# MadrMan/gpgpuraytrace

Hardware: AMD Instinct MI355X
Metric: Mray/s + ms/frame at 1920×1080, 1/2/4/8 MI355X; % HBM roofline (higher is better)
Workload: dtype f32

## Files before the change

gpgpuraytrace_amd/_native.py:

```python
import ctypes as C
import os

HERE = os.path.dirname(os.path.abspath(__file__))
LIB_PATH = os.path.join(HERE, "_build", "librt_hip.so")
ROOT = os.path.dirname(HERE)
HEADER = os.path.join(ROOT, "include", "frosttrace.h")

RT_OK = 0
RT_DEVICE_FLOAT_OUTPUT = 1
RT_DEVICE_STATS = 2
RT_DEVICE_GRAPH = 4
RT_DEVICE_DEBUG_SMALL_RINGS = 32
RT_DEVICE_DEBUG_WITHHOLD_FUSE = 64
RT_DEVICE_GATED = 128
RT_DEVICE_DEBUG_GATE_STRESS = 512
RT_DEVICE_DEFERRED = 1024
RT_DEVICE_DEBUG_DEFER_SMALL = 2048
ABI_VERSION = 9
RT_READBACK_RGBA8 = 0
RT_READBACK_BGRX = 1
RT_TEXTURE_2D = 1
RT_FORMAT_R8G8B8A8_UINT = 3


class RtStats(C.Structure):
    _fields_ = [("primary_steps", C.c_ulonglong), ("shadow_steps", C.c_ulonglong),
                ("prepass_steps", C.c_ulonglong), ("hits", C.c_ulonglong), ("noise_calls", C.c_ulonglong),
                ("ao_steps", C.c_ulonglong), ("noise_wave_iters", C.c_ulonglong)]


RT_RAYS_EYE = 1
RT_RAYS_FORCE_SEGMENTS = 2
RT_RAYS_FORCE_LANES = 4
RT_MAX_RAYS = 1 << 26


class RtRayOptions(C.Structure):
    _fields_ = [("size", C.c_uint32), ("flags", C.c_uint32), ("eye", C.c_float * 3), ("max_blocks", C.c_uint32)]


RT_SURFACE_PARAMS = 8
RT_SURFACE_RAY_RANGE = 16


class RtSurfaceOptions(C.Structure):
    _fields_ = [("size", C.c_uint32), ("flags", C.c_uint32), ("eye", C.c_float * 3), ("max_blocks", C.c_uint32),
                ("t_min", C.c_float), ("t_max", C.c_float), ("stepmod", C.c_float), ("max_steps", C.c_uint32)]


RT_POINT_MAX_AO = 16


class RtPointOptions(C.Structure):
    _fields_ = [("size", C.c_uint32), ("flags", C.c_uint32), ("eye", C.c_float * 3), ("max_blocks", C.c_uint32),
                ("ao_samples", C.c_uint32), ("seed", C.c_uint32)]


RT_FIELD_NORMAL = 32
RT_MAX_LATTICE_DIM = 4096


class RtFieldOptions(C.Structure):
    _fields_ = [("size", C.c_uint32), ("flags", C.c_uint32), ("eye", C.c_float * 3), ("max_blocks", C.c_uint32)]


class RtLattice(C.Structure):
    _fields_ = [("origin", C.c_float * 3), ("spacing", C.c_float * 3), ("dims", C.c_uint32 * 3)]


RT_DIST_FAR = 0xFFFFFFFF


class RtDistanceOptions(C.Structure):
    _fields_ = [("size", C.c_uint32), ("flags", C.c_uint32), ("eye", C.c_float * 3), ("max_blocks", C.c_uint32),
                ("max_cells", C.c_uint32)]


class NativeError(RuntimeError):
    pass


_lib = None

_vp, _i, _u, _sz, _cp = C.c_void_p, C.c_int, C.c_uint, C.c_size_t, C.c_char_p
SIGNATURES = {
    "rt_last_error": (_cp, []),
    "rt_abi_version": (_i, []),
    "rt_vfs_add_path": (_i, [_cp]),
    "rt_vfs_clear": (_i, []),
    "rt_device_create": (_i, [_i, _i, _i, _u, C.POINTER(_vp)]),
    "rt_device_destroy": (None, [_vp]),
    "rt_device_present": (_i, [_vp]),
    "rt_device_flush": (_i, [_vp]),
    "rt_device_synchronize": (_i, [_vp]),
    "rt_device_readback": (_i, [_vp, _vp, _sz]),
    "rt_device_readback_float": (_i, [_vp, _vp]),
    "rt_device_readback_bgrx": (_i, [_vp, _vp, _sz]),
    "rt_device_size": (_i, [_vp, C.POINTER(_i), C.POINTER(_i)]),
    "rt_device_framebuffer": (_vp, [_vp]),
    "rt_device_stream": (_vp, [_vp]),
    "rt_device_set_stream": (_i, [_vp, _vp]),
    "rt_device_stats": (_i, [_vp, C.POINTER(RtStats), _i]),
    "rt_device_stats_sized": (_i, [_vp, C.POINTER(RtStats), _sz, _i]),
    "rt_stream_refs": (_i, [_vp]),
    "rt_device_set_profiling": (_i, [_vp, _i]),
    "rt_device_kernel_time": (_i, [_vp, C.POINTER(C.c_double), C.POINTER(_i)]),
    "rt_device_graph_info": (_i, [_vp, C.POINTER(C.c_ulonglong), C.POINTER(C.c_ulonglong)]),
    "rt_device_info": (_i, [_vp, _i, C.POINTER(C.c_ulonglong)]),
    "rt_device_reserve_cus": (_i, [_vp, _i]),
    "rt_device_defer_batch": (_i, [_vp, _i]),
    "rt_debug_spin": (_i, [_vp, _vp, C.c_ulonglong, C.c_ulonglong, _vp]),
    "rt_debug_defer_slot": (_i, [_vp, _i, _vp, _vp, _vp]),
    "rt_device_wait_event": (_i, [_vp, _vp]),
    "rt_device_record_event": (_i, [_vp, _vp]),
    "rt_device_check": (_i, [_vp]),
    "rt_texture_create": (_i, [_vp, C.POINTER(_vp)]),
    "rt_texture_init": (_i, [_vp, _i, _i, _i, _i, _vp, _i, _i]),
    "rt_texture_destroy": (None, [_vp]),
    "rt_compute_create": (_i, [_vp, C.POINTER(_vp)]),
    "rt_compute_destroy": (None, [_vp]),
    "rt_compute_load": (_i, [_vp, _cp, _cp, _cp, _i, _i, _i, C.POINTER(_cp), C.POINTER(_cp), _i]),
    "rt_compute_swap": (_i, [_vp]),
    "rt_compute_run": (_i, [_vp, _u, _u, _u]),
    "rt_compute_set_texture": (_i, [_vp, _i, _vp]),
    "rt_compute_thread_size": (_i, [_vp, C.POINTER(_i), C.POINTER(_i), C.POINTER(_i)]),
    "rt_compute_get_variable": (_vp, [_vp, _cp]),
    "rt_compute_get_array": (_vp, [_vp, _cp]),
    "rt_compute_get_buffer": (_vp, [_vp, _cp]),
    "rt_variable_write": (_i, [_vp, _vp]),
    "rt_variable_size": (_sz, [_vp]),
    "rt_variable_name": (_cp, [_vp]),
    "rt_array_create": (_i, [_vp, _u]),
    "rt_array_map": (_vp, [_vp]),
    "rt_array_unmap": (_i, [_vp]),
    "rt_array_write": (_i, [_vp, _vp]),
    "rt_array_stride": (_sz, [_vp]),
    "rt_array_device_pointer": (_vp, [_vp]),
    "rt_terrain_render": (_i, [_vp, _vp, _i, _i]),
    "rt_terrain_render_feed": (_i, [_vp, _vp, _i, _i]),
    "rt_terrain_render_batch": (_i, [C.POINTER(_vp), C.POINTER(_vp), _i, _i, _i]),
    "rt_terrain_render_batch_packed": (_i, [C.POINTER(_vp), C.POINTER(_vp), _i, _i, _i, _vp, _sz]),
    "rt_terrain_prepass_batch": (_i, [C.POINTER(_vp), C.POINTER(_vp), _i, _i, _i, _vp]),
    "rt_terrain_trace_batch": (_i, [C.POINTER(_vp), C.POINTER(_vp), _i, _i, _i, _vp]),
    "rt_terrain_prepass_ahead": (_i, [C.POINTER(_vp), C.POINTER(_vp), _i]),
    "rt_terrain_trace_ahead": (_i, [C.POINTER(_vp), C.POINTER(_vp), _i, _i, _i]),
    "rt_terrain_feed_wait": (_i, [_vp, _vp]),
    "rt_shard_bytes": (_sz, [_vp, _i, _i]),
    "rt_shard_pack": (_i, [_vp, _i, _i, _vp]),
    "rt_shard_unpack": (_i, [_vp, _i, _i, _vp]),
    "rt_shard_pack_batch": (_i, [C.POINTER(_vp), C.POINTER(_i), _i, C.POINTER(_vp), _i]),
    "rt_shard_unpack_batch": (_i, [C.POINTER(_vp), C.POINTER(_i), _i, C.POINTER(_vp), _i]),
    "rt_terrain_trace_rays": (_i, [_vp, _vp, _vp, _i, C.POINTER(RtRayOptions), _vp, _vp]),
    "rt_terrain_trace_rays_device": (_i, [_vp, _vp, _i, C.POINTER(RtRayOptions), _vp, _vp]),
    "rt_terrain_trace_surface": (_i, [_vp, _vp, _vp, _vp, _i, C.POINTER(RtSurfaceOptions), _vp, _vp]),
    "rt_terrain_trace_surface_device": (_i, [_vp, _vp, _i, C.POINTER(RtSurfaceOptions), _vp, _vp]),
    "rt_terrain_shade_rays": (_i, [_vp, _vp, _vp, _vp, _i, C.POINTER(RtSurfaceOptions), _vp, _vp, _vp]),
    "rt_terrain_shade_rays_device": (_i, [_vp, _vp, _i, C.POINTER(RtSurfaceOptions), _vp, _vp, _vp]),
    "rt_terrain_shade_points": (_i, [_vp, _vp, _vp, _i, C.POINTER(RtPointOptions), _vp, _vp, _vp]),
    "rt_terrain_shade_points_device": (_i, [_vp, _vp, _vp, _i, C.POINTER(RtPointOptions), _vp, _vp, _vp]),
    "rt_terrain_sample_field": (_i, [_vp, _vp, _i, C.POINTER(RtFieldOptions), _vp]),
    "rt_terrain_sample_field_device": (_i, [_vp, _vp, _i, C.POINTER(RtFieldOptions), _vp]),
    "rt_terrain_sample_lattice": (_i, [_vp, C.POINTER(RtLattice), C.POINTER(RtFieldOptions), _vp, _vp]),
    "rt_terrain_sample_lattice_device": (_i, [_vp, C.POINTER(RtLattice), C.POINTER(RtFieldOptions), _vp, _vp]),
    "rt_terrain_mesh_scratch_bytes": (_sz, [C.POINTER(RtLattice)]),
    "rt_terrain_extract_mesh": (_i, [_vp, C.POINTER(RtLattice), C.POINTER(RtFieldOptions), _vp, _vp, C.c_uint32, _vp,
                                     C.c_uint32, _vp]),
    "rt_terrain_extract_mesh_device": (_i, [_vp, C.POINTER(RtLattice), C.POINTER(RtFieldOptions), _vp, _sz, _vp, _vp,
                                            C.c_uint32, _vp, C.c_uint32, _vp]),
    "rt_terrain_distance_scratch_bytes": (_sz, [C.POINTER(RtLattice)]),
    "rt_terrain_distance_field": (_i, [_vp, C.POINTER(RtLattice), C.POINTER(RtDistanceOptions), _vp, _vp, _vp]),
    "rt_terrain_distance_field_device": (_i, [_vp, C.POINTER(RtLattice), C.POINTER(RtDistanceOptions), _vp, _vp, _sz,
                                              _vp, _vp]),
    "rt_noise_generate": (_i, [C.c_uint32, _i, _vp, _vp]),
    "rt_terrain_set_target_depths": (_i, [_vp, _vp]),
    "rt_recorder_create": (_i, [_vp, _i, _i, _cp, C.POINTER(_vp)]),
    "rt_recorder_start": (_i, [_vp]),
    "rt_recorder_stop": (_i, [_vp]),
    "rt_recorder_is_recording": (_i, [_vp]),
    "rt_recorder_set_frame_time": (_i, [_vp, C.c_float]),
    "rt_recorder_write": (_i, [_vp, _vp, _i]),
    "rt_recorder_info": (_i, [_vp, C.POINTER(C.c_ulonglong), C.POINTER(C.c_ulonglong), C.POINTER(C.c_ulonglong)]),
    "rt_recorder_destroy": (None, [_vp]),
    "rt_recorder_set_async": (_i, [_vp, _i]),
    "rt_readback_create": (_i, [_vp, _i, _i, C.POINTER(_vp)]),
    "rt_readback_submit": (_i, [_vp, C.POINTER(C.c_ulonglong)]),
    "rt_readback_ready": (_i, [_vp, C.c_ulonglong]),
    "rt_readback_wait": (_i, [_vp, C.c_ulonglong, C.POINTER(_vp)]),
    "rt_readback_release": (_i, [_vp, C.c_ulonglong]),
    "rt_readback_destroy": (None, [_vp]),
    "rt_varmgr_start": (_i, [_i, _cp]),
    "rt_varmgr_stop": (_i, []),
    "rt_varmgr_count": (_i, []),
    "rt_varmgr_register_compute": (_i, [_vp]),
    "rt_debug_math": (_i, [_vp, _i, _vp, _vp, _vp, _i]),
    "rt_debug_sky_ceiling": (_i, [_vp, _i, C.c_float, _vp, _i, C.POINTER(C.c_double)]),
    "rt_debug_noise": (_i, [_vp, _vp, _vp, _i, _i]),
    "rt_debug_sky": (_i, [_vp, _vp, _vp, _i]),
}


def lib():
    global _lib
    if _lib is None:
        if not os.path.exists(LIB_PATH):
            raise ImportError(
                f"gpgpuraytrace_amd: native library missing at {LIB_PATH}; build it with "
                "`python -c 'import __graft_entry__ as g; g.build()'` (make -C gpgpuraytrace_amd/csrc)")
        L = C.CDLL(LIB_PATH)
        L.rt_abi_version.restype, L.rt_abi_version.argtypes = _i, []
        if L.rt_abi_version() < ABI_VERSION:
            raise ImportError(f"gpgpuraytrace_amd: {LIB_PATH} has ABI {L.rt_abi_version()}, this binding "
                              f"needs >= {ABI_VERSION}; rebuild it (make -C gpgpuraytrace_amd/csrc)")
        for name, (res, args) in SIGNATURES.items():
            try:
                f = getattr(L, name)
            except AttributeError:
                raise ImportError(f"gpgpuraytrace_amd: {LIB_PATH} does not export {name}; rebuild it "
                                  "(make -C gpgpuraytrace_amd/csrc)") from None
            f.restype = res
            f.argtypes = args
        _lib = L
    return _lib


def check(rc, what=""):
    if rc != RT_OK:
        msg = lib().rt_last_error().decode(errors="replace")
        raise NativeError(f"{what}: rc={rc}: {msg}")
    return rc
```

gpgpuraytrace_amd/csrc/rt_kernels.hip:

```cpp
#include <hip/hip_runtime.h>

#include <cstdio>
#include <cstdlib>
#include <type_traits>

#include "rt_kernels.h"
#include "rt_rayquery.h"
#include "rt_shader.h"
#include "rt_variants.h"

using namespace rts;
using rtm::f3;

namespace {

constexpr int kPermWords = 128 * 128;
constexpr int kNpOct = RT_NP_OCTAVES + 3;
constexpr int kOctWords = kNpOct * 4;
constexpr int kOctBase = (int)kLdsGz / 4 + (int)(kLdsGz - kLdsGxy) / 4;
constexpr int kNoiseLdsWords = kOctBase + kOctWords;
static_assert(kNoiseLdsWords % 4 == 0, "LDS carved after the noise image stays 16-byte aligned");
static_assert(kLdsGxy == (uint32_t)kPermWords * 4u, "gxy follows the perm2D texels");

__device__ __forceinline__ void load_noise_lds(uint32_t* lds, const uint32_t* __restrict__ perm2d,
                                               const float4* __restrict__ grad, const RtConsts* __restrict__ k)
{
    {
        float4* oct = reinterpret_cast<float4*>(lds + kOctBase);
        const int i = threadIdx.x;
        if (i < kNpOct) {
            const int n = i <= RT_NP_OCTAVES ? i : RT_NP_OCTAVES;
            oct[i] = make_float4(k->np_scale[n], k->np_scale_y[n], k->np_rcp[n], 0.0f);
        }
    }
    float4* gxy = reinterpret_cast<float4*>(lds + kLdsGxy / 4);
    float4* gz = reinterpret_cast<float4*>(lds + kLdsGz / 4);
    for (int i = threadIdx.x; i < 128 * 16; i += blockDim.x) {
        int e = i >> 4;
        float4 g0 = grad[e], g1 = grad[(e + 1) & 127];
        gxy[i] = make_float4(g0.x, g1.x, g0.y, g1.y);
        gz[i] = make_float4(g0.z, g1.z, 0.0f, 0.0f);
    }
    uint4* p = reinterpret_cast<uint4*>(lds);
    const uint4* src = reinterpret_cast<const uint4*>(perm2d);
    for (int i = threadIdx.x; i < kPermWords / 4; i += blockDim.x) p[i] = src[i];
    __syncthreads();
}

template <class T>
__device__ __forceinline__ T __attribute__((address_space(1)))* gptr(T* p)
{
    return (T __attribute__((address_space(1)))*)p;
}
__device__ __forceinline__ void gstore(float4* p, float4 v)
{
    typedef float v4f __attribute__((ext_vector_type(4)));
    *(v4f __attribute__((address_space(1)))*)p = v4f{v.x, v.y, v.z, v.w};
}

__device__ __forceinline__ Ctx make_ctx(const RtConsts* k, const uint32_t* lds)
{
    Ctx c;
    c.nz.img = reinterpret_cast<const char*>(lds);
    c.nz.oct = reinterpret_cast<const float4*>(lds + kOctBase);
    c.nz.so16 = kLdsGxy | ((threadIdx.x & (RT_LDS_SLOTS - 1u)) * 16u);
    c.nz.calls = 0;
    c.nz.lds_calls = nullptr;
    c.nz.phase = RT_PHASE_OTHER;
    c.k = k;
    c.kf = (KPtr)k;
    c.eye = rtm::mk(k->eye[0], k->eye[1], k->eye[2]);
    c.sun = rtm::mk(k->sun[0], k->sun[1], k->sun[2]);
    return c;
}

struct QueryEye {
    float x, y, z;
};
__device__ __forceinline__ Ctx make_ctx(const RtConsts* k, const uint32_t* lds, QueryEye e)
{
    Ctx c = make_ctx(k, lds);
    c.eye = rtm::mk(e.x, e.y, e.z);
    return c;
}

__device__ __forceinline__ void stats_noise(RtStats* stats, uint64_t calls)
{
    atomicAdd(&stats->noise_calls, (unsigned long long)(calls & 0xffffffffull));
    if (calls >> 32) atomicAdd(&stats->noise_waves, (unsigned long long)(calls >> 32));
}

__device__ __forceinline__ float uniform_f(float x)
{
    return __int_as_float(__builtin_amdgcn_readfirstlane(__float_as_int(x)));
}

__device__ __forceinline__ Ctx frame_ctx_cam(const Ctx& c, const FrameTable* __restrict__ ft, uint32_t f)
{
    Ctx cf = c;
    cf.kf = (KPtr)ft->kcam[f];
    cf.eye = rtm::mk(uniform_f(cf.kf->eye[0]), uniform_f(cf.kf->eye[1]), uniform_f(cf.kf->eye[2]));
    cf.sun = rtm::mk(uniform_f(cf.kf->sun[0]), uniform_f(cf.kf->sun[1]), uniform_f(cf.kf->sun[2]));
    return cf;
}

template <int L, bool STATS>
__global__ void __launch_bounds__(64) k_camerarays(const RtConsts* __restrict__ k, const uint32_t* __restrict__ perm2d,
                                                   const float4* __restrict__ grad, float4* __restrict__ out,
                                                   RtStats* stats, const FrameTable* __restrict__ ft)
{
    if (ft) out = ft->cam[blockIdx.y];
    __shared__ __attribute__((aligned(16))) uint32_t lds[kNoiseLdsWords];
    load_noise_lds(lds, perm2d, grad, k);
    int i = blockIdx.x * blockDim.x + threadIdx.x;
    if (i >= RT_CAMERA_RES * RT_CAMERA_RES) return;
    Ctx c = make_ctx(k, lds);
    if (ft) c = frame_ctx_cam(c, ft, blockIdx.y);
    int tx = i % RT_CAMERA_RES, ty = i / RT_CAMERA_RES;
    const float r31 = rtm::rcp(31.0f);
    uint32_t pxs = (uint32_t)(((float)tx * r31) * k->screen[0]);
    uint32_t pys = (uint32_t)(((float)ty * r31) * k->screen[1]);
    f3 p, dir;
    get_pixel_ray(c, (float)pxs, (float)pys, &p, &dir);
    RayResult rr = trace_ray<L, false, true>(c, p, RT_CAMERA_NEAR, RT_CAMERA_FAR, 2.0f, dir, 0);
    if (rr.density < 0.0f) rr.pd.w = RT_CAMERA_FAR;
    out[i] = make_float4(rr.pd.x, rr.pd.y, rr.pd.z, rr.pd.w);
    if constexpr (STATS) {
        atomicAdd(&stats->prepass_steps, (unsigned long long)rr.steps);
        stats_noise(stats, c.nz.calls);
    }
}

template <bool STATS, int BS, int LPR>
__global__ void __launch_bounds__(BS) k_camerarays_group(const RtConsts* __restrict__ k,
                                                          const uint32_t* __restrict__ perm2d,
                                                          const float4* __restrict__ grad, float4* __restrict__ out,
                                                          RtStats* stats, const FrameTable* __restrict__ ft)
{
    constexpr int L = RT_NOMADPLAINS;
    if (ft) out = ft->cam[blockIdx.y];
    __shared__ __attribute__((aligned(16))) uint32_t lds[kNoiseLdsWords];
    load_noise_lds(lds, perm2d, grad, k);
    const int i = blockIdx.x * (BS / LPR) + (int)(threadIdx.x / LPR);
    if (i >= RT_CAMERA_RES * RT_CAMERA_RES) return;
    Ctx c = make_ctx(k, lds);
    if (ft) c = frame_ctx_cam(c, ft, blockIdx.y);
    const uint32_t j = threadIdx.x & (LPR - 1u), base = threadIdx.x & 63u & ~(LPR - 1u);
    const SegOctaves<LPR> g = seg_octaves<LPR>(c, j);
    int tx = i % RT_CAMERA_RES, ty = i / RT_CAMERA_RES;
    const float r31 = rtm::rcp(31.0f);
    uint32_t pxs = (uint32_t)(((float)tx * r31) * k->screen[0]);
    uint32_t pys = (uint32_t)(((float)ty * r31) * k->screen[1]);
    f3 p, dir;
    get_pixel_ray(c, (float)pxs, (float)pys, &p, &dir);
    March<L, false> st;
    march_begin(c, st, p, RT_CAMERA_NEAR, 2.0f, dir);
    uint32_t noise = 0;
    while (march_live<L, false, true>(c, st, RT_CAMERA_FAR, 0)) {
        auto dens = [&](f3 q) {
            uint32_t used;
            float d = density_nomadplains_seg<LPR>(c, g, q, j, base, &used);
            noise += used + 1u;
            return d;
        };
        march_step_with<L, false, true>(c, st, dens);
    }
    RayResult rr = march_result(st);
    if (rr.density < 0.0f) rr.pd.w = RT_CAMERA_FAR;
    if (j == 0) {
        out[i] = make_float4(rr.pd.x, rr.pd.y, rr.pd.z, rr.pd.w);
        if constexpr (STATS) {
            atomicAdd(&stats->prepass_steps, (unsigned long long)rr.steps);
            atomicAdd(&stats->noise_calls, (unsigned long long)noise);
        }
    }
}

template <class Depth>
__device__ __forceinline__ float cd_get_depth(Depth depth, int x, int y)
{
    x = x < 0 ? 0 : (x >= RT_CAMERA_RES ? RT_CAMERA_RES - 1 : x);
    y = y < 0 ? 0 : (y >= RT_CAMERA_RES ? RT_CAMERA_RES - 1 : y);
    return depth(x, y);
}
template <class Depth>
__device__ __forceinline__ float cd_interp(Depth d, int x, int y)
{
    if (x < 0) {
        float m = cd_get_depth(d, x + 1, y);
        float dd = cd_get_depth(d, x + 2, y) - m;
        return m - dd;
    }
    if (x >= RT_CAMERA_RES) {
        float m = cd_get_depth(d, x - 1, y);
        float dd = cd_get_depth(d, x - 2, y) - m;
        return m - dd;
    }
    if (y < 0) {
        float m = cd_get_depth(d, x, y + 1);
        float dd = cd_get_depth(d, x, y + 2) - m;
        return m - dd;
    }
    if (y >= RT_CAMERA_RES) {
        float m = cd_get_depth(d, x, y - 1);
        float dd = cd_get_depth(d, x, y - 2) - m;
        return m - dd;
    }
    return cd_get_depth(d, x, y);
}

template <class Depth>
__device__ __forceinline__ float2 cell_bracket(Depth depth, int xpos, int ypos)
{
    float dmin = cd_interp(depth, xpos, ypos);
    float dmax = dmin;
    for (int xp = -2; xp <= 2; ++xp) {
        for (int yp = -2; yp <= 2; ++yp) {
            float d = cd_interp(depth, xpos + xp, ypos + yp);
            dmin = (dmin < d) ? dmin : d;
            dmax = (d < dmax) ? dmax : d;
        }
    }
    dmin = dmin * 0.96f - 0.01f;
    dmax = dmax * 1.22f + 0.4f;
    dmin = (RT_CAMERA_NEAR < dmin) ? dmin : RT_CAMERA_NEAR;
    dmax = (dmax < RT_CAMERA_FAR) ? dmax : RT_CAMERA_FAR;
    return make_float2(dmin, dmax);
}

__device__ __forceinline__ float cam_depth_sc1(const float4* cam, int x, int y)
{
    typedef const float __attribute__((address_space(1))) gfloat;
    return __hip_atomic_load((gfloat*)(reinterpret_cast<const float*>(cam + y * RT_CAMERA_RES + x) + 3),
                             __ATOMIC_RELAXED, __HIP_MEMORY_SCOPE_AGENT);
}

__device__ __forceinline__ void cell_depths_frame(const float4* __restrict__ cam, float2* __restrict__ cells,
                                                  float* s_d)
{
    const int i = threadIdx.x;
    __syncthreads();
    s_d[i] = cam_depth_sc1(cam, i % RT_CAMERA_RES, i / RT_CAMERA_RES);
    __syncthreads();
    cells[i] = cell_bracket([&](int x, int y) { return s_d[y * RT_CAMERA_RES + x]; }, i % RT_CAMERA_RES,
                            i / RT_CAMERA_RES);
}

struct UnitMap {
    uint32_t off_x, off_y, ext_x, ext_y, tiles32_x, tile_first, tile_stride, n_units;
    uint32_t n_frames, frame_samples;
    uint32_t frame_rot;
    uint32_t order_batch;
    uint32_t cells_from_cam;
    uint32_t fit;
    uint32_t fitm;
    uint32_t packed;
};

__device__ __forceinline__ uint32_t out_index(const UnitMap& m, uint32_t u, uint32_t lane, uint32_t px, uint32_t py,
                                              uint32_t W)
{
    if (m.packed)
        return (u >> 4) * 1024u + ((u & 15u) >> 2) * 256u + (lane >> 3) * 32u + (u & 3u) * 8u + (lane & 7u);
    return py * W + px;
}
__device__ __forceinline__ uint32_t packed_index(uint32_t tl)
{
    return (tl & ~0xf8u) | ((tl >> 3) & 0x18u) | ((tl << 2) & 0xe0u);
}

__device__ __forceinline__ bool unit_pixel(const UnitMap& m, uint32_t f, uint32_t u, uint32_t lane, uint32_t W,
                                           uint32_t H, uint32_t* px, uint32_t* py)
{
    const uint32_t first = m.frame_rot ? (m.tile_first + f) % m.tile_stride : m.tile_first;
    uint32_t T = (u >> 4) * m.tile_stride + first, sub = u & 15u;
    uint32_t gx = (T % m.tiles32_x) * 32u + (sub & 3u) * 8u + (lane & 7u);
    uint32_t gy = (T / m.tiles32_x) * 32u + (sub >> 2) * 8u + (lane >> 3);
    *px = gx + m.off_x;
    *py = gy + m.off_y;
    return gx < m.ext_x && gy < m.ext_y && *px < W && *py < H;
}

__device__ __forceinline__ bool sample_pixel(const UnitMap& m, uint32_t f, uint32_t t, uint32_t aa, uint32_t W,
                                             uint32_t H, uint32_t* px, uint32_t* py, uint32_t* a)
{
    uint32_t pix = t / aa;
    *a = t - pix * aa;
    return unit_pixel(m, f, pix >> 6, pix & 63u, W, H, px, py);
}

__device__ __forceinline__ uint32_t wave_fetch(uint32_t* counter, uint32_t lane, uint32_t n = 1u)
{
    uint32_t u = 0;
    if (lane == 0) u = atomicAdd(counter, n);
    return __builtin_amdgcn_readfirstlane(u);
}

__device__ __forceinline__ uint32_t lane_rank(uint64_t mask)
{
    return __builtin_amdgcn_mbcnt_hi((uint32_t)(mask >> 32), __builtin_amdgcn_mbcnt_lo((uint32_t)mask, 0u));
}

__device__ __forceinline__ uint32_t first_unit_index(uint32_t* __restrict__ counters, uint32_t lane)
{
    const uint32_t w = (uint32_t)__builtin_amdgcn_readfirstlane((int)(threadIdx.x >> 6));
    return w * gridDim.x + wave_fetch(&counters[RT_CTR_FIRST + w], lane);
}

template <int L>
struct HitRec {
    static constexpr uint32_t N = FogLive<L>::value ? 3u : (RT_DIAG_HITPAD ? 2u : 1u);
};
template <int L>
__device__ __forceinline__ void hit_store(float4* __restrict__ r, uint32_t t, const RayResult& rr)
{
    if constexpr (FogLive<L>::value) {
        r[0] = make_float4(rr.pd.x, rr.pd.y, rr.pd.z, rr.pd.w);
        r[1] = make_float4(rr.fc.x, rr.fc.y, rr.fc.z, rr.fc.w);
        r[2] = make_float4(rr.density, rr.steps, 0.0f, __uint_as_float(t));
    } else {
        r[0] = make_float4(rr.sd, rr.pd.w, rr.density, __uint_as_float(t));
        if constexpr (RT_DIAG_HITPAD) r[1] = make_float4(0.0f, 0.0f, 0.0f, 0.0f);
    }
}

constexpr uint32_t kOrderLdsBuckets = 144u * 1024u;
constexpr uint32_t kOrderBatchUnitsPerWave = 4u;
__global__ void __launch_bounds__(1024) k_order(const FrameTable* __restrict__ ft, UnitMap m,
                                                uint32_t* __restrict__ order, uint32_t* __restrict__ counters,
                                                const uint32_t* wait_ctl, uint32_t wait_total, uint32_t* zero_ctl,
                                                uint32_t* host_flag, uint32_t* gate, uint32_t* claims)
{
    __shared__ float s_key[RT_CAMERA_RES * RT_CAMERA_RES];
    __shared__ uint32_t s_hist[64];
    __shared__ uint8_t s_b[kOrderLdsBuckets];
    if (blockIdx.x == 0 && threadIdx.x < RT_CTR_BYTES / 4) counters[threadIdx.x] = 0u;
    if (zero_ctl && blockIdx.x == 0 && threadIdx.x < 2) zero_ctl[threadIdx.x] = 0u;
    if (gate) {
        const uint32_t g0 = m.order_batch ? 0u : blockIdx.x, g1 = m.order_batch ? m.n_frames : blockIdx.x + 1u;
        for (uint32_t i = g0 * RT_GATE_WORDS + threadIdx.x; i < g1 * RT_GATE_WORDS; i += blockDim.x) gate[i] = 0u;
        const uint32_t nt = m.n_units >> 4;
        for (uint32_t i = g0 * nt + threadIdx.x; i < g1 * nt; i += blockDim.x) claims[i] = 0u;
    }
    if (wait_ctl) {
        if (threadIdx.x == 0) {
            const uint64_t t0 = __builtin_amdgcn_s_memrealtime();
            while (__hip_atomic_load(wait_ctl + 1, __ATOMIC_RELAXED, __HIP_MEMORY_SCOPE_AGENT) < wait_total) {
                __builtin_amdgcn_s_sleep(8);
                if (__builtin_amdgcn_s_memrealtime() - t0 > 50000000ull) {
                    atomicOr(counters + RT_CTR_BYTES / 4, RT_FLAG_PREPASS_TIMEOUT);
                    if (host_flag) __hip_atomic_store(host_flag, RT_FLAG_PREPASS_TIMEOUT, __ATOMIC_RELAXED,
                                                      __HIP_MEMORY_SCOPE_SYSTEM);
                    break;
                }
            }
        }
        __syncthreads();
    }
    if (m.cells_from_cam) {
        const uint32_t c0 = m.order_batch ? 0u : blockIdx.x, c1 = m.order_batch ? m.n_frames : blockIdx.x + 1u;
        for (uint32_t f = c0; f < c1; ++f) cell_depths_frame(ft->cam[f], ft->cells[f], s_key);
        __syncthreads();
    }
    if (threadIdx.x < 64) s_hist[threadIdx.x] = 0;
    const uint32_t n_tiles = m.n_units >> 4;
    const bool cached = n_tiles * m.n_frames <= kOrderLdsBuckets;
    uint32_t f = 0;
    auto load_keys = [&]() {
        __syncthreads();
        const float2* cells = ft->cells[f];
        for (int i = threadIdx.x; i < RT_CAMERA_RES * RT_CAMERA_RES; i += blockDim.x) {
            float2 cd = cells[i];
            s_key[i] = __log2f(cd.y / cd.x);
        }
        __syncthreads();
    };
    auto bucket = [&](uint32_t tile) -> uint32_t {
        const RtConsts* k = ft->k[f];
        const uint32_t W = (uint32_t)k->width, H = (uint32_t)k->height;
        float key = 0.0f;
        for (uint32_t corner = 0; corner < 4; ++corner) {
            uint32_t px, py;
            uint32_t u = tile * 16u + (corner & 1u) * 3u + (corner >> 1) * 12u;
            uint32_t lane = (corner & 1u) * 7u + (corner >> 1) * 56u;
            if (!unit_pixel(m, f, u, lane, W, H, &px, &py)) {
                if (!unit_pixel(m, f, tile * 16u, 0u, W, H, &px, &py)) continue;
                px = px + (corner & 1u) * 31u < W ? px + (corner & 1u) * 31u : W - 1u;
                py = py + (corner >> 1) * 31u < H ? py + (corner >> 1) * 31u : H - 1u;
            }
            float spx = (float)px * k->rcp_w, spy = (float)py * k->rcp_h;
            uint32_t cell = (uint32_t)rtm::fma(rtm::floor(spy * 32.0f), 32.0f, rtm::floor(spx * 32.0f));
            key = fmaxf(key, s_key[cell]);
        }
        int b = (int)(key * 3.3f);
        return (uint32_t)(b < 0 ? 0 : (b > 63 ? 63 : b));
    };
    {
        const uint32_t g0 = m.order_batch ? 0u : blockIdx.x, g1 = m.order_batch ? m.n_frames : blockIdx.x + 1u;
        for (f = g0; f < g1; ++f) {
            load_keys();
            for (uint32_t t = threadIdx.x; t < n_tiles; t += blockDim.x) {
                const uint32_t b = bucket(t);
                if (cached) s_b[f * n_tiles + t] = (uint8_t)b;
                atomicAdd(&s_hist[b], 1u);
            }
        }
        __syncthreads();
        if (threadIdx.x == 0) {
            uint32_t run = g0 * n_tiles;
            for (int b = 63; b >= 0; --b) {
                uint32_t c = s_hist[b];
                s_hist[b] = run;
                run += c;
            }
        }
        for (f = g0; f < g1; ++f) {
            if (cached) __syncthreads();
            else load_keys();
            for (uint32_t t = threadIdx.x; t < n_tiles; t += blockDim.x) {
                const uint32_t b = cached ? (uint32_t)s_b[f * n_tiles + t] : bucket(t);
                order[atomicAdd(&s_hist[b], 1u)] = (f << 24) | t;
            }
        }
    }
}

constexpr uint32_t kShadowRec = 3;

constexpr uint32_t kRefillIdle = RT_REFILL_IDLE;

__device__ __forceinline__ float4 shade_finish(const RtConsts* k, float4 cb, float4 fog, float4 ray,
                                               float shadow_density, float shadow_fog_w)
{
    float b = cb.w;
    if (shadow_density > 0.0f) b = b * 0.1f;
    else b = rtm::sat(b - shadow_fog_w);
    f3 col = rtm::mk(cb.x * fma(b, k->one_minus_shadow[0], k->shadow_color[0]),
                     cb.y * fma(b, k->one_minus_shadow[1], k->shadow_color[1]),
                     cb.z * fma(b, k->one_minus_shadow[2], k->shadow_color[2]));
    col = rtm::mk(rtm::lerp(col.x, fog.x, fog.w), rtm::lerp(col.y, fog.y, fog.w), rtm::lerp(col.z, fog.z, fog.w));
    col = rtm::mk(rtm::lerp(col.x, ray.x, ray.w), rtm::lerp(col.y, ray.y, ray.w), rtm::lerp(col.z, ray.z, ray.w));
    return make_float4(rtm::sat(col.x), rtm::sat(col.y), rtm::sat(col.z), 1.0f);
}

__device__ __forceinline__ float4 miss_sample(const Ctx& c, float px, float py, float dist, f4 fog)
{
    f3 p, dir;
    get_pixel_ray(c, px, py, &p, &dir);
    f3 pdn = rtm::normalize(dir);
    float skyAmount = dist * 0.0005f;
    skyAmount = rtm::sat(skyAmount * skyAmount);
    SkyColor scat = get_rayleigh_mie(c, pdn);
    float space = get_space_color(c, pdn);
    f3 sky = rtm::mk((scat.mie.x + scat.rayleigh.x) + space, (scat.mie.y + scat.rayleigh.y) + space,
                     (scat.mie.z + scat.rayleigh.z) + space);
    f3 col = rtm::mk(rtm::lerp(sky.x, fog.x, fog.w), rtm::lerp(sky.y, fog.y, fog.w), rtm::lerp(sky.z, fog.z, fog.w));
    col = rtm::mk(rtm::lerp(col.x, sky.x, skyAmount), rtm::lerp(col.y, sky.y, skyAmount),
                  rtm::lerp(col.z, sky.z, skyAmount));
    return make_float4(rtm::sat(col.x), rtm::sat(col.y), rtm::sat(col.z), 0.0f);
}

typedef float v4f_t __attribute__((ext_vector_type(4)));
__device__ __forceinline__ float4 ld_rec(const float4* base, uint32_t i)
{
    const __amdgpu_buffer_rsrc_t r =
        __builtin_amdgcn_make_buffer_rsrc(const_cast<float4*>(base), (short)0, 0x7fffffff, 0x00020000);
    const v4f_t v = __builtin_amdgcn_raw_buffer_load_b128(r, (int)(i * 16u), 0, 16 );
    return make_float4(v.x, v.y, v.z, v.w);
}
__device__ __forceinline__ uint32_t ld_u32(const uint32_t* base, uint32_t i, bool sc1 = true)
{
    const __amdgpu_buffer_rsrc_t r =
        __builtin_amdgcn_make_buffer_rsrc(const_cast<uint32_t*>(base), (short)0, 0x7fffffff, 0x00020000);
    return sc1 ? __builtin_amdgcn_raw_buffer_load_b32(r, (int)(i * 4u), 0, 16 )
               : __builtin_amdgcn_raw_buffer_load_b32(r, (int)(i * 4u), 0, 0);
}
__device__ __forceinline__ float4 ld_fresh(const float4* p)
{
    v4f_t v;
    asm volatile("global_load_dwordx4 %0, %1, off sc1\n\ts_waitcnt vmcnt(0)" : "=v"(v) : "v"(p) : "memory");
    return make_float4(v.x, v.y, v.z, v.w);
}

__device__ __forceinline__ uint32_t late(uint32_t x)
{
    asm volatile("" : "+v"(x));
    return x;
}

__device__ __forceinline__ void sample_store(const RtConsts* k, float4* __restrict__ samples, uint32_t t, float4 v)
{
    t = late(t);
    if (k->aa_samples == 1) {
        float* c = reinterpret_cast<float*>(samples) + 3u * t;
        c[0] = v.x;
        c[1] = v.y;
        c[2] = v.z;
    } else {
        samples[t] = v;
    }
}

__device__ __forceinline__ void ao_count(uint32_t* __restrict__ aocc, uint32_t t)
{
    atomicAdd(&aocc[t >> 2], 1u << ((t & 3u) * 8u));
}
constexpr uint32_t kFinFlag = 0x80u;
__device__ __forceinline__ uint32_t ao_occluded(const uint32_t* __restrict__ aocc, uint32_t t)
{
    return (aocc[t >> 2] >> ((t & 3u) * 8u)) & 0x7fu;
}

struct ShadeHit {
    float4 cb, fog, ray;
    bool more;
    f3 hp, n;
    float prec;
    uint32_t px, py, a;
};


__device__ __forceinline__ Ctx frame_ctx(const Ctx& c, const FrameTable* __restrict__ ft, uint32_t f)
{
    Ctx cf = c;
    cf.kf = (KPtr)ft->k[f];
    cf.eye = rtm::mk(uniform_f(cf.kf->eye[0]), uniform_f(cf.kf->eye[1]), uniform_f(cf.kf->eye[2]));
    cf.sun = rtm::mk(uniform_f(cf.kf->sun[0]), uniform_f(cf.kf->sun[1]), uniform_f(cf.kf->sun[2]));
    return cf;
}

__device__ __forceinline__ uint32_t frame_of(const UnitMap& m, uint32_t t)
{
    return m.n_frames == 1u ? 0u : t / m.frame_samples;
}

template <class Body>
__device__ __forceinline__ void per_frame(bool valid, uint32_t f_lane, Body body)
{
    uint64_t pend = __ballot(valid);
    while (pend) {
        const uint32_t f = (uint32_t)__builtin_amdgcn_readlane((int)f_lane, (int)__builtin_ctzll(pend));
        const bool mine = valid && f_lane == f;
        pend &= ~__ballot(mine);
        if (mine) body(f);
    }
}

struct FrameRays {
    float v[RT_MAX_BATCH][6];
    uint32_t* out8[RT_MAX_BATCH];
};
__device__ __forceinline__ void frame_rays_load(FrameRays& s, const FrameTable* __restrict__ ft, uint32_t n_frames)
{
    if (threadIdx.x < n_frames) {
        const RtConsts* k = ft->k[threadIdx.x];
        const f3 sun = rtm::mk(k->sun[0], k->sun[1], k->sun[2]);
        const f3 sd = rtm::scale(sun, rtm::rcp(rtm::length(sun)));
        s.v[threadIdx.x][0] = k->eye[0];
        s.v[threadIdx.x][1] = k->eye[1];
        s.v[threadIdx.x][2] = k->eye[2];
        s.v[threadIdx.x][3] = sd.x;
        s.v[threadIdx.x][4] = sd.y;
        s.v[threadIdx.x][5] = sd.z;
        s.out8[threadIdx.x] = ft->out8[threadIdx.x];
    }
}

template <int L>
__device__ __forceinline__ ShadeHit shade_hit(const Ctx& c, const UnitMap& m, float4 r0, float4 r1, float4 r2,
                                              uint32_t t, uint32_t tl, March<L, true>& st)
{
    const RtConsts* k = c.k;
    const uint32_t W = (uint32_t)k->width, H = (uint32_t)k->height, aa = (uint32_t)k->aa_samples;
    ShadeHit h;
    float4 pdw, dn;
    if constexpr (FogLive<L>::value) {
        pdw = r0;
        h.fog = r1;
        dn = r2;
    } else {
        (void)r1;
        (void)r2;
        pdw = make_float4(r0.x, 0.0f, 0.0f, r0.y);
        dn = make_float4(r0.z, 0.0f, 0.0f, 0.0f);
        h.fog = make_float4(0.0f, 0.0f, 0.0f, 0.0f);
    }
    uint32_t px, py, a;
    sample_pixel(m, m.frame_rot ? (t - tl) / m.frame_samples : 0u, tl, aa, W, H, &px, &py, &a);
    h.px = px;
    h.py = py;
    h.a = a;
    f3 p, dir;
    get_pixel_ray(c, (float)px + k->aa_off[a][0], (float)py + k->aa_off[a][1], &p, &dir);
    if constexpr (!FogLive<L>::value) {
        const f3 md = rtm::scale(dir, rtm::rcp(rtm::length(dir)));
        const float sd = pdw.x;
        pdw = make_float4(fma(md.x, sd, p.x), fma(md.y, sd, p.y), fma(md.z, sd, p.z), pdw.w);
    }
    f3 hp = rtm::mk(pdw.x, pdw.y, pdw.z);
    h.hp = hp;
    h.prec = shade_precision(pdw.w);
    march_begin(c, st, hp, 0.4f, h.prec, c.sun);
    if (march_live<L, true, true>(c, st, 100.0f, 0)) march_step<L, true, true>(c, st);
    h.more = march_live<L, true, true>(c, st, 100.0f, 0);
    f3 pdn = rtm::normalize(dir);
    float skyAmount = pdw.w * 0.0005f;
    skyAmount = rtm::sat(skyAmount * skyAmount);
    f4 pd = {pdw.x, pdw.y, pdw.z, dn.x};
    f3 n = get_normal<L>(c, pd);
    h.n = n;
    ShadePre sp = shade_pre<L>(c, hp, n, pdn, pdw.w);
    float specular = rtm::sat(rtm::pow_nonneg(rtm::max(sp.spec_dot, 0.0f), 40.0f)) * sp.spec_k;
    SkyColor scat = get_rayleigh_mie(c, pdn);
    h.cb = make_float4(sp.col[0] + specular, sp.col[1] + specular, sp.col[2] + specular, sp.brightness);
    h.ray = make_float4(scat.rayleigh.x, scat.rayleigh.y, scat.rayleigh.z, skyAmount);
    return h;
}

constexpr uint32_t kAuxAO = 0xffffffffu, kAuxAOCand = 0x80000000u, kAuxFinT = 0x7ffffffeu;
__device__ __forceinline__ bool aux_ao(uint32_t aux) { return (int32_t)aux < 0; }
constexpr uint32_t kAuxAOSlot = 0xc0000000u, kAuxSlotFree = 0x60000000u;
__device__ __forceinline__ bool aux_ao_slot(uint32_t aux) { return (aux & 0xff000000u) == kAuxAOSlot; }
__device__ __forceinline__ bool aux_slot_free(uint32_t aux) { return (aux & 0xff000000u) == kAuxSlotFree; }

template <int L>
__device__ __forceinline__ void long_pack(const March<L, true>& st, uint32_t t, uint32_t aux, float4* r)
{
    r[0] = make_float4(st.p.x, st.p.y, st.p.z, st.dist);
    r[1] = make_float4(st.step, __uint_as_float(aux), __uint_as_float((uint32_t)st.iters), __uint_as_float(t));
    if (aux_ao(aux)) r[2] = make_float4(st.dir.x, st.dir.y, st.dir.z, 0.0f);
    else if constexpr (March<L, true>::FOG) r[2] = make_float4(st.f.x, st.f.y, st.f.z, st.f.w);
}

template <int L>
__device__ __forceinline__ uint32_t long_unpack(const float4 r0, const float4 r1, const float4 r2, f3 sun_dir,
                                                March<L, true>& st, uint32_t* aux)
{
    *aux = __float_as_uint(r1.y);
    st.p = rtm::mk(r0.x, r0.y, r0.z);
    st.dist = r0.w;
    st.step = r1.x;
    st.lastStep = 0.0f;
    st.d = 0.0f;
    st.iters = (int)__float_as_uint(r1.z);
    if (aux_ao(*aux)) {
        st.dir = rtm::mk(r2.x, r2.y, r2.z);
        st.f = {0.0f, 0.0f, 0.0f, 0.0f};
        st.fog = false;
    } else {
        st.dir = sun_dir;
        if constexpr (March<L, true>::FOG) st.f = {r2.x, r2.y, r2.z, r2.w};
        else st.f = {0.0f, 0.0f, 0.0f, 0.0f};
        st.fog = true;
    }
    return __float_as_uint(r1.w);
}

template <int L>
__device__ __forceinline__ void ao_begin(const Ctx& c, const ShadeHit& h, uint32_t kk, March<L, true>& st)
{
    march_begin(c, st, h.hp, 0.4f, h.prec, ao_dir(h.n, h.px, h.py, h.a, kk), false);
}

template <int L>
struct FinRec {
    static constexpr uint32_t N = FogLive<L>::value ? 3u : 2u;
};
template <int L>
__device__ __forceinline__ void fin_store(float4* __restrict__ f, const ShadeHit& h)
{
    if constexpr (FogLive<L>::value) {
        f[0] = h.cb;
        f[1] = h.fog;
        f[2] = h.ray;
    } else {
        f[0] = h.cb;
        f[1] = h.ray;
    }
}

__device__ __forceinline__ uint32_t fit_pixel(float4 v, float ao)
{
    const float ia = rtm::rcp(1.0f);
    return unorm8((0.0f + v.x * ao) * ia) | (unorm8((0.0f + v.y * ao) * ia) << 8) |
           (unorm8((0.0f + v.z * ao) * ia) << 16) | 0xff000000u;
}

__device__ __forceinline__ void fit_store(const RtConsts* k, const UnitMap& m, const FrameRays& fr, uint32_t t,
                                          uint32_t px8)
{
    const uint32_t f = frame_of(m, t), W = (uint32_t)k->width;
    const uint32_t tl = t - f * m.frame_samples;
    if (m.packed) {
        gptr(fr.out8[f])[late(packed_index(tl))] = px8;
        return;
    }
    uint32_t px, py;
    unit_pixel(m, f, tl >> 6, t & 63u, W, (uint32_t)k->height, &px, &py);
    gptr(fr.out8[f])[(size_t)late(py) * W + px] = px8;
}

template <int L>
__device__ __forceinline__ void long_finish(const RtConsts* k, const UnitMap& m, const FrameRays& fr,
                                            const float4* __restrict__ fin, const float4* __restrict__ finp,
                                            float4* __restrict__ samples, uint32_t* __restrict__ aocc, uint32_t t,
                                            uint32_t aux, const March<L, true>& st)
{
    if (aux_ao(aux)) {
        if (st.d > 0.0f) {
            if (aux == kAuxAO) {
                if (m.fit) reinterpret_cast<uint8_t*>(aocc)[late(t)] = (uint8_t)(kFinFlag | 1u);
                else if (k->ao_samples == 1) reinterpret_cast<uint8_t*>(aocc)[late(t)] = 1u;
                else if (!(RT_DIAG_SKIP & 8)) ao_count(aocc, t);
            } else if (!(RT_DIAG_SKIP & 2)) {
                fit_store(k, m, fr, t, aux | 0xff000000u);
            }
        }
    } else {
        constexpr uint32_t FR = FinRec<L>::N;
        float4 f0, f1, fog = make_float4(0.0f, 0.0f, 0.0f, 0.0f);
        if (aux == kAuxFinT) {
            const float4* f = fin + (size_t)FR * t;
            f0 = ld_fresh(f);
            if constexpr (FogLive<L>::value) fog = ld_fresh(f + 1);
            f1 = ld_fresh(f + FR - 1u);
        } else {
            f0 = ld_rec(finp, FR * aux);
            if constexpr (FogLive<L>::value) fog = ld_rec(finp, FR * aux + 1u);
            f1 = ld_rec(finp, FR * aux + FR - 1u);
        }
        const float4 v = shade_finish(k, f0, fog, f1, st.d, st.f.w);
        if (m.fit && k->ao_samples == 0) {
            if (!(RT_DIAG_SKIP & 2)) fit_store(k, m, fr, t, fit_pixel(v, 1.0f));
        } else if (!(RT_DIAG_SKIP & 4)) {
            sample_store(k, samples, t, v);
        }
    }
}

constexpr uint32_t kLongRing = 570;
constexpr uint32_t kFinSlots = RT_FIN_SLOTS;
constexpr uint32_t kAoSlots = RT_AO_SLOTS;
static_assert(kAoSlots % 2u == 0u && kAoSlots <= 256u && kAoSlots <= RT_AO_POOL_SLOTS,
              "AO slots: pairs of u16 counters, u8 indices, a colour each in the pool");
constexpr uint32_t kLongBatch = RT_LONG_BATCH;
constexpr uint32_t kCompactLive = RT_COMPACT_LIVE;
constexpr uint32_t kSegLanes = RT_SEG_LANES, kSegHandBack = RT_SEG_HANDBACK, kSegQueue = RT_SEG_QUEUE;
constexpr uint32_t kPrepassSplit = RT_FUSE_RAYS_PER_TASK / (64u / RT_PREPASS_LPR);
static_assert(kPrepassSplit >= 1u && RT_PREPASS_LPR >= RT_FUSE_RAYS_PER_TASK && RT_PREPASS_LPR <= 32, "prepass lanes per ray");
constexpr uint32_t kPrimarySeg = RT_PRIMARY_SEG;
static_assert(kPrimarySeg == 0u || kPrimarySeg == 4u || kPrimarySeg == 8u || kPrimarySeg == 16u, "lanes per ray");
constexpr bool kStatsPrimarySeg = RT_STATS_PRIMARY_SEG != 0;

struct BlockStats {
    enum { PRIMARY = 0, SHADOW = 1, AO = 2, HITS = 3, NOISE = 4, NOISE_WAVES = 5 };
    unsigned long long v[6];
    uint32_t done, pad;
};

struct TraceQueues {
    uint32_t lock;
    uint32_t h_top, pad0;
    uint32_t l_head, l_tail;
    uint32_t active;
    uint32_t drained;
    uint32_t pad;
    uint32_t ls_top;
    uint32_t pad1;
    uint32_t f_top;
    uint32_t overflow;
    uint32_t gscan, gate_all, gate_cells;
    uint32_t near_end;

    float4 longs[kLongRing * kShadowRec];
    uint16_t fin_free[kFinSlots];
    uint32_t ao_ctr[kAoSlots / 2];
    uint8_t ao_free[kAoSlots];
    uint32_t ao_top;
};

template <class T>
__device__ __forceinline__ T vload(const T& x)
{
    return __hip_atomic_load(&x, __ATOMIC_RELAXED, __HIP_MEMORY_SCOPE_WORKGROUP);
}

__device__ __forceinline__ void q_lock(uint32_t* lock, uint32_t lane)
{
    if (lane == 0) {
        while (atomicCAS(lock, 0u, 1u) != 0u) __builtin_amdgcn_s_sleep(1);
    }
    __builtin_amdgcn_wave_barrier();
    __builtin_amdgcn_fence(__ATOMIC_ACQUIRE, "workgroup");
}

__device__ __forceinline__ void q_unlock(uint32_t* lock, uint32_t lane)
{
    __builtin_amdgcn_fence(__ATOMIC_RELEASE, "workgroup");
    __builtin_amdgcn_wave_barrier();
    if (lane == 0) atomicExch(lock, 0u);
}

RT_DIAG_LIVE_HIST(__device__ unsigned long long g_live_hist[65];)
WT(__device__ unsigned long long g_wave_trace[RT_WT_MAX_WAVES * RT_WT_FIELDS];)

template <int L>
struct TraceThreads {
    static constexpr uint32_t value = 64u * ((L == RT_GREENROCKS || L == RT_SIMPLE) ? RT_TRACE_WAVES_WIDE : RT_TRACE_WAVES_FAST);
};
static_assert(RT_CTR_FIRST + RT_TRACE_WAVES_FAST <= RT_CTR_BYTES / 4 && RT_CTR_FIRST + RT_TRACE_WAVES_WIDE <= RT_CTR_BYTES / 4,
              "a first-unit counter per wave slot inside the zeroed work counters");

template <int L, bool STATS, bool GATED = false>
__global__ void __launch_bounds__(TraceThreads<L>::value) k_trace(const RtConsts* __restrict__ k, const FrameTable* __restrict__ ft,
                                                const uint32_t* __restrict__ perm2d,
                                                const float4* __restrict__ grad,
                                                UnitMap m, const uint32_t* __restrict__ order,
                                                uint64_t* __restrict__ hitmask, float4* __restrict__ samples,
                                                float4* __restrict__ fin, float4* __restrict__ finpool,
                                                float4* __restrict__ cpool,
                                                float4* __restrict__ hitq,
                                                float4* __restrict__ spill_long, uint32_t hit_cap,
                                                uint32_t long_spill_cap,
                                                uint32_t* __restrict__ aocc, uint32_t* __restrict__ counters,
                                                RtStats* stats, uint32_t long_batch, uint32_t refill_idle,
                                                uint32_t compact_live, uint32_t long_ring_cap, uint32_t fin_slots,
                                                FusedPrepass np, GatedPrepass gp)
{
    __shared__ __attribute__((aligned(16))) uint32_t
        lds[kNoiseLdsWords + (sizeof(FrameRays) + sizeof(TraceQueues) + sizeof(BlockStats)) / 4];
    FrameRays& s_fr = *reinterpret_cast<FrameRays*>(lds + kNoiseLdsWords);
    TraceQueues& q = *reinterpret_cast<TraceQueues*>(lds + kNoiseLdsWords + sizeof(FrameRays) / 4);
    BlockStats& s_st =
        *reinterpret_cast<BlockStats*>(lds + kNoiseLdsWords + (sizeof(FrameRays) + sizeof(TraceQueues)) / 4);
    frame_rays_load(s_fr, ft, m.n_frames);
    if (threadIdx.x == 0) {
        q.lock = 0;
        q.h_top = 0;
        q.l_head = q.l_tail = 0;
        q.active = 0;
        q.drained = 0;
        q.ls_top = 0;
        q.f_top = fin_slots;
        q.overflow = 0;
        q.gscan = q.gate_all = q.gate_cells = 0;
        q.near_end = 0;
        if constexpr (STATS) s_st = BlockStats{};
    }
    for (uint32_t i = threadIdx.x; i < fin_slots; i += blockDim.x) q.fin_free[i] = (uint16_t)i;
    for (uint32_t i = threadIdx.x; i < kAoSlots; i += blockDim.x) {
        q.ao_free[i] = (uint8_t)i;
        if (i < kAoSlots / 2u) q.ao_ctr[i] = 0u;
    }
    if (threadIdx.x == 0) q.ao_top = kAoSlots;
    load_noise_lds(lds, perm2d, grad, k);
    const uint32_t lane = __lane_id();
    Ctx c = make_ctx(k, lds);
    if constexpr (STATS) c.nz.lds_calls = (__attribute__((address_space(3))) unsigned long long*)&s_st.v[BlockStats::NOISE];
    const uint32_t W = (uint32_t)k->width, H = (uint32_t)k->height, aa = (uint32_t)k->aa_samples;
    const int max_steps = k->max_steps;
    constexpr bool kSky = RT_SKY_EXIT && L == RT_NOMADPLAINS && (!STATS || RT_SKY_EXIT_STATS);
    const uint32_t n_total = (uint32_t)__builtin_amdgcn_readfirstlane(m.n_units * m.n_frames);
    constexpr uint32_t HR = HitRec<L>::N;
    float4* const hq = hitq + (size_t)blockIdx.x * hit_cap * HR;
    float4* const finp = finpool + (size_t)blockIdx.x * kFinSlots * FinRec<L>::N;
    float4* const cpl = cpool + (size_t)blockIdx.x * RT_AO_POOL_SLOTS;
    float4* const lspill = spill_long + (size_t)blockIdx.x * long_spill_cap * kShadowRec;
    auto queued_long = [&]() { return vload(q.l_tail) - vload(q.l_head) + vload(q.ls_top); };
    auto queued_hits = [&]() { return vload(q.h_top); };
    auto stat = [&](int i, uint32_t v) {
        if constexpr (STATS) atomicAdd(&s_st.v[i], (unsigned long long)v);
    };

    WT(unsigned long long wt[RT_WT_FIELDS] = {}; wt[10] = __builtin_amdgcn_s_getreg((31 << 11) | 4);
       wt[11] = __builtin_amdgcn_s_getreg((31 << 11) | 20); uint32_t wl_rays = 0, wl_maxit = 0, wp_maxit = 0;)
    auto push_recs = [&](bool want, auto pack) {
        const uint64_t lb = __ballot(want);
        if (!lb) return;
        const uint32_t n = (uint32_t)__popcll(lb), rank = lane_rank(lb);
        q_lock(&q.lock, lane);
        const uint32_t lh = vload(q.l_head), lt = vload(q.l_tail);
        if (lt - lh + n <= long_ring_cap) {
            if (want) pack(&q.longs[((lt + rank) % kLongRing) * kShadowRec]);
            if (lane == 0) q.l_tail = lt + n;
        } else {
            const uint32_t stl = (uint32_t)__builtin_amdgcn_readfirstlane(vload(q.ls_top));
            const bool fits = stl + n <= long_spill_cap;
            if (want && fits) pack(lspill + (size_t)(stl + rank) * kShadowRec);
            __builtin_amdgcn_s_waitcnt(0);
            if (lane == 0) {
                q.ls_top = fits ? stl + n : stl;
                q.overflow |= fits ? 0u : RT_FLAG_SPILL_OVERFLOW;
            }
        }
        q_unlock(&q.lock, lane);
    };
    auto push_long = [&](bool want, const March<L, true>& st, uint32_t t, uint32_t aux) {
        push_recs(want, [&](float4* r) { long_pack(st, t, aux, r); });
    };

    auto free_fin_locked = [&](bool live, uint32_t& aux) {
        const bool pend = !live && aux < kFinSlots;
        const uint64_t pb = __ballot(pend);
        if (pb) {
            const uint32_t top = vload(q.f_top);
            if (pend) {
                q.fin_free[top + lane_rank(pb)] = (uint16_t)aux;
                aux = kAuxAO;
            }
            if (lane == 0) q.f_top = top + (uint32_t)__popcll(pb);
        }
        if constexpr (kAoSlots > 0u) {
            const bool pa = !live && aux_slot_free(aux);
            const uint64_t ab = __ballot(pa);
            if (ab) {
                const uint32_t top = vload(q.ao_top);
                if (pa) {
                    q.ao_free[top + lane_rank(ab)] = (uint8_t)(aux & 255u);
                    aux = kAuxAO;
                }
                if (lane == 0) q.ao_top = top + (uint32_t)__popcll(ab);
            }
        }
    };
    auto ao_slot_finish = [&](const March<L, true>& st, uint32_t t, uint32_t& aux) {
        const uint32_t sl = aux & 255u, sh = (sl & 1u) * 16u;
        const uint32_t occ1 = st.d > 0.0f ? 1u : 0u;
        const uint32_t old = atomicAdd(&q.ao_ctr[sl >> 1], (1u | (occ1 << 5)) << sh) >> sh;
        if ((old & 31u) + 1u == (uint32_t)k->ao_samples) {
            const uint32_t occ = ((old >> 5) & 31u) + occ1;
            if (m.fitm && !(old & (1u << 10))) {
                const float4 v = ld_rec(cpl, sl);
                const uint32_t at = __float_as_uint(v.w);
                if (!(RT_DIAG_SKIP & 2)) gptr(s_fr.out8[at >> 23])[at & 0x7fffffu] = fit_pixel(v, ao_factor(occ, k->ao_samples));
            } else if (occ != 0u) {
                reinterpret_cast<uint8_t*>(aocc)[late(t)] = (uint8_t)((m.fitm ? kFinFlag : 0u) | occ);
            }
            atomicAnd(&q.ao_ctr[sl >> 1], ~(0xffffu << sh));
            aux = kAuxSlotFree | sl;
        } else {
            aux = kAuxAO;
        }
    };

    auto do_shadow = [&]() {
        March<L, true> st;
        st.d = 0.0f;
        st.iters = 0;
        bool live = false;
        uint32_t t = 0, aux = kAuxAO;
        Ctx cl = c;
        cl.nz.phase = RT_PHASE_LONG;
        for (;;) {
            if (live && !march_live<L, true, true>(cl, st, aux_ao(aux) ? RT_AO_END : 100.0f, 0)) {
                WT(wl_rays++; wl_maxit = max(wl_maxit, (uint32_t)st.iters);)
                stat(aux_ao(aux) ? BlockStats::AO : BlockStats::SHADOW, (uint32_t)st.iters);
                if (kAoSlots > 0u && aux_ao_slot(aux)) ao_slot_finish(st, t, aux);
                else long_finish<L>(k, m, s_fr, fin, finp, samples, aocc, t, aux, st);
                live = false;
            }
            const uint64_t idle = __ballot(!live);
            const uint32_t nidle = (uint32_t)__popcll(idle);
            if (nidle >= refill_idle && queued_long() != 0u) {
                q_lock(&q.lock, lane);
                free_fin_locked(live, aux);
                const uint32_t head = vload(q.l_head), tail = vload(q.l_tail);
                const uint32_t take = (tail - head) < nidle ? (tail - head) : nidle;
                const uint32_t sl = vload(q.ls_top);
                const uint32_t more = sl < nidle - take ? sl : nidle - take;
                const uint32_t rank = lane_rank(idle);
                const bool mine = ((idle >> lane) & 1ull) && rank < take + more;
                auto take_ray = [&](float4 r0, float4 r1, float4 r2) {
                    t = long_unpack(r0, r1, r2, rtm::mk(0.0f, 0.0f, 0.0f), st, &aux);
                    const float* fr = s_fr.v[frame_of(m, t)];
                    cl.eye = rtm::mk(fr[0], fr[1], fr[2]);
                    if (!aux_ao(aux)) st.dir = rtm::mk(fr[3], fr[4], fr[5]);
                    live = true;
                };
                if (mine && rank < take) {
                    const float4* r = &q.longs[((head + rank) % kLongRing) * kShadowRec];
                    take_ray(r[0], r[1], r[2]);
                } else if (mine) {
                    const uint32_t ri = (sl - more + rank - take) * kShadowRec;
                    take_ray(ld_rec(lspill, ri), ld_rec(lspill, ri + 1u), ld_rec(lspill, ri + 2u));
                }
                if (more) __builtin_amdgcn_s_waitcnt(0);
                if (lane == 0) {
                    q.l_head = head + take;
                    q.ls_top = sl - more;
                }
                q_unlock(&q.lock, lane);
            }
            const uint64_t lv = __ballot(live);
            const bool drained_now = vload(q.drained) != 0u;
            bool hand_back = lv != 0ull && (uint32_t)__popcll(lv) < compact_live && queued_long() == 0u && !drained_now;
            if constexpr (L == RT_NOMADPLAINS && kSegLanes > 0u)
                hand_back = hand_back || (drained_now && lv != 0ull && (uint32_t)__popcll(lv) <= kSegHandBack &&
                                          queued_long() == 0u);
            if (lv == 0ull || hand_back) {
                if (__ballot(!live && (aux < kFinSlots || aux_slot_free(aux)))) {
                    q_lock(&q.lock, lane);
                    free_fin_locked(live, aux);
                    q_unlock(&q.lock, lane);
                }
                if (hand_back) push_long(live, st, t, aux);
                c.nz.calls = cl.nz.calls;
                return;
            }
            RT_DIAG_LONG_STEPS(if (live && (RT_COUNT_LONG_STEPS == 1 || (RT_COUNT_LONG_STEPS == 2) == (vload(q.drained) != 0u))) {
                cl.nz.phase = RT_COUNT_PHASE;
                count_noise(cl.nz);
                cl.nz.phase = RT_PHASE_LONG;
            })
            WT(wt[26]++;)
            if (live) march_step<L, true, true>(cl, st);
        }
    };

    auto do_shadow_seg = [&]() {
        if constexpr (L == RT_NOMADPLAINS && kSegLanes > 0u) {
            constexpr uint32_t LPR = kSegLanes ? kSegLanes : 8u, RPW = 64u / LPR;
            March<L, true> st;
            st.d = 0.0f;
            st.iters = 0;
            uint32_t t = 0, aux = kAuxAO;
            bool live = false;
            Ctx cl = c;
            cl.nz.phase = RT_PHASE_LONG;
            q_lock(&q.lock, lane);
            const uint32_t head = vload(q.l_head), tail = vload(q.l_tail);
            const uint32_t take = (tail - head) < RPW ? (tail - head) : RPW;
            const uint32_t sl = vload(q.ls_top);
            const uint32_t more = sl < RPW - take ? sl : RPW - take;
            if (const uint32_t grp = late(lane) / LPR; grp < take + more) {
                float4 r0, r1, r2;
                if (grp < take) {
                    const float4* r = &q.longs[((head + grp) % kLongRing) * kShadowRec];
                    r0 = r[0];
                    r1 = r[1];
                    r2 = r[2];
                } else {
                    const uint32_t ri = (sl - more + grp - take) * kShadowRec;
                    r0 = ld_rec(lspill, ri);
                    r1 = ld_rec(lspill, ri + 1u);
                    r2 = ld_rec(lspill, ri + 2u);
                }
                t = long_unpack(r0, r1, r2, rtm::mk(0.0f, 0.0f, 0.0f), st, &aux);
                const float* fr = s_fr.v[frame_of(m, t)];
                cl.eye = rtm::mk(fr[0], fr[1], fr[2]);
                if (!aux_ao(aux)) st.dir = rtm::mk(fr[3], fr[4], fr[5]);
                live = true;
            }
            __builtin_amdgcn_s_waitcnt(0);
            if (lane == 0) {
                q.l_head = head + take;
                q.ls_top = sl - more;
            }
            q_unlock(&q.lock, lane);
            const uint32_t lid = late(lane);
            const uint32_t j = lid & (LPR - 1u), base = lid & ~(LPR - 1u);
            const SegOctaves<LPR> g = seg_octaves<LPR>(c, j);
            for (;;) {
                if (live && !march_live<L, true, true>(cl, st, aux_ao(aux) ? RT_AO_END : 100.0f, 0)) {
                    if (j == 0u) {
                        stat(aux_ao(aux) ? BlockStats::AO : BlockStats::SHADOW, (uint32_t)st.iters);
                        if (kAoSlots > 0u && aux_ao_slot(aux)) ao_slot_finish(st, t, aux);
                        else long_finish<L>(k, m, s_fr, fin, finp, samples, aocc, t, aux, st);
                    }
                    live = false;
                }
                if (!__ballot(live)) break;
                WT(wt[25]++;)
                if (live) {
                    auto dens = [&](f3 q0) {
                        uint32_t used;
                        const float d = density_nomadplains_seg<LPR>(cl, g, q0, j, base, &used);
                        if constexpr (STATS) {
                            if (j == 0u) atomicAdd(&s_st.v[BlockStats::NOISE], (unsigned long long)(used + 1u));
                            if (lane == (uint32_t)__builtin_ctzll(__ballot(1)))
                                atomicAdd(&s_st.v[BlockStats::NOISE_WAVES], (unsigned long long)SegOctaves<LPR>::R);
                        }
                        return d;
                    };
                    march_step_with<L, true, true>(cl, st, dens);
                }
            }
            uint32_t fa = j == 0u ? aux : kAuxAO;
            if (__ballot(fa < kFinSlots || aux_slot_free(fa))) {
                q_lock(&q.lock, lane);
                free_fin_locked(false, fa);
                q_unlock(&q.lock, lane);
            }
        }
    };

    auto primary_seg = [&](const Ctx& cf, March<L, true>& st, bool lv, uint64_t lb, float spx, float spy, bool sky) {
        if constexpr (L == RT_NOMADPLAINS && kPrimarySeg > 0u && (!STATS || kStatsPrimarySeg)) {
            constexpr uint32_t LPR = 64u / (kPrimarySeg ? kPrimarySeg : 8u);
            const uint32_t lid = late(lane);
            const uint32_t j = lid & (LPR - 1u), grp = lid / LPR, base = lid & ~(LPR - 1u);
            const uint32_t n = (uint32_t)__popcll(lb);
            uint32_t src = lid;
            uint64_t rem = lb;
            for (uint32_t r = 0; r < n; ++r) {
                const uint32_t sl = (uint32_t)__builtin_ctzll(rem);
                rem &= rem - 1ull;
                src = grp == r ? sl : src;
            }
            March<L, true> sg;
            sg.p = rtm::mk(__shfl(st.p.x, (int)src), __shfl(st.p.y, (int)src), __shfl(st.p.z, (int)src));
            sg.dir = rtm::mk(__shfl(st.dir.x, (int)src), __shfl(st.dir.y, (int)src), __shfl(st.dir.z, (int)src));
            sg.sd = __shfl(st.sd, (int)src);
            sg.dist = __shfl(st.dist, (int)src);
            sg.step = __shfl(st.step, (int)src);
            sg.lastStep = __shfl(st.lastStep, (int)src);
            sg.d = __shfl(st.d, (int)src);
            sg.iters = __shfl(st.iters, (int)src);
            sg.f = {0.0f, 0.0f, 0.0f, 0.0f};
            sg.fog = false;
            bool live = grp < n;
            const SegOctaves<LPR> g = seg_octaves<LPR>(cf, j);
            for (;;) {
                if (live && !march_live<L, true, false>(cf, sg, RT_CAMERA_FAR, max_steps)) live = false;
                if constexpr (kSky) {
                    if (live && sky && sky_exit(sg.p.y, sg.dir.y, sg.dist)) live = false;
                }
                if (!__ballot(live)) break;
                if (live) {
                    auto dens = [&](f3 q0) {
                        uint32_t used;
                        const float d = density_nomadplains_seg<LPR, true>(cf, g, q0, j, base, &used);
                        if constexpr (STATS) {
                            if (j == 0u) atomicAdd(&s_st.v[BlockStats::NOISE], (unsigned long long)(used + 1u));
                            if (lane == (uint32_t)__builtin_ctzll(__ballot(1)))
                                atomicAdd(&s_st.v[BlockStats::NOISE_WAVES], (unsigned long long)SegOctaves<LPR>::R);
                        }
                        return d;
                    };
                    march_step_with<L, true, false>(cf, sg, dens);
                }
            }
            const int back = (int)(lane_rank(lb) * LPR);
            const float sd = __shfl(sg.sd, back), dist = __shfl(sg.dist, back), step = __shfl(sg.step, back);
            const float last = __shfl(sg.lastStep, back), d = __shfl(sg.d, back);
            const int iters = __shfl(sg.iters, back);
            if (lv) {
                st.sd = sd;
                st.dist = dist;
                st.step = step;
                st.lastStep = last;
                st.d = d;
                st.iters = iters;
            }
            f3 p, dir;
            get_pixel_ray(cf, spx, spy, &p, &dir);
            st.p = p;
            st.dir = rtm::scale(dir, rtm::rcp(rtm::length(dir)));
        }
    };

    auto do_shade = [&]() {
        q_lock(&q.lock, lane);
        const uint32_t top = vload(q.h_top);
        const uint32_t take = top < 64u ? top : 64u;
        float4 r0 = make_float4(0.0f, 0.0f, 0.0f, 0.0f), r1 = r0, r2 = r0;
        if (lane < take) {
            const uint32_t ri = (top - take + lane) * HR;
            r0 = ld_rec(hq, ri);
            if constexpr (HR == 3u) {
                r1 = ld_rec(hq, ri + 1u);
                r2 = ld_rec(hq, ri + 2u);
            }
        }
        __builtin_amdgcn_s_waitcnt(0);
        if (lane == 0) q.h_top = top - take;
        q_unlock(&q.lock, lane);
        const uint32_t t = __float_as_uint(HR == 3u ? r2.w : r0.w);
        March<L, true> st;
        bool more = false;
        uint32_t aux = kAuxAO;
        uint32_t ao_aux = kAuxAO;
        const bool valid = lane < take;
        if (kAoSlots > 0u && k->ao_samples >= 2) {
            const uint64_t vb = __ballot(valid);
            if (vb) {
                q_lock(&q.lock, lane);
                const uint32_t top = vload(q.ao_top), n = (uint32_t)__popcll(vb), rank = lane_rank(vb);
                const uint32_t got = n < top ? n : top;
                if (valid && rank < got) ao_aux = kAuxAOSlot | (uint32_t)q.ao_free[top - 1u - rank];
                if (lane == 0) q.ao_top = top - got;
                q_unlock(&q.lock, lane);
            }
        }
        ShadeHit h;
        per_frame(valid, valid ? frame_of(m, t) : 0u, [&](uint32_t f) {
            Ctx cf = frame_ctx(c, ft, f);
            cf.nz.phase = RT_PHASE_SHADE;
            h = shade_hit<L>(cf, m, r0, r1, r2, t, t - f * m.frame_samples, st);
            c.nz.calls = cf.nz.calls;
            more = h.more;
            if (!more) {
                const float4 v = shade_finish(k, h.cb, h.fog, h.ray, st.d, st.f.w);
                if (m.fit) {
                    if (!(RT_DIAG_SKIP & 2)) {
                        const uint32_t tl = t - f * m.frame_samples;
                        gptr(ft->out8[f])[m.packed ? late(packed_index(tl)) : late(h.py) * W + h.px] = fit_pixel(v, 1.0f);
                    }
                    if (k->ao_samples) ao_aux = kAuxAOCand | (fit_pixel(v, ao_factor(1u, 1)) & 0xffffffu);
                } else if (m.fitm && aux_ao_slot(ao_aux)) {
                    const uint32_t tl = t - f * m.frame_samples;
                    cpl[late(ao_aux & 255u)] =
                        make_float4(v.x, v.y, v.z, __uint_as_float((f << 23) | (m.packed ? packed_index(tl) : h.py * W + h.px)));
                } else if (!(RT_DIAG_SKIP & 4)) {
                    sample_store(k, samples, t, v);
                }
                stat(BlockStats::SHADOW, (uint32_t)st.iters);
            }
            const uint64_t mb = __ballot(more);
            if (mb) {
                const uint32_t lead = (uint32_t)__builtin_ctzll(__ballot(1));
                q_lock(&q.lock, lane - lead);
                const uint32_t top = vload(q.f_top), n = (uint32_t)__popcll(mb), rank = lane_rank(mb);
                const uint32_t got = n < top ? n : top;
                if (more) aux = rank < got ? (uint32_t)q.fin_free[top - 1u - rank] : kAuxFinT;
                if (lane == lead) q.f_top = top - got;
                q_unlock(&q.lock, lane - lead);
                if (more && !(RT_DIAG_SKIP & 16)) fin_store<L>(aux == kAuxFinT ? fin + (size_t)FinRec<L>::N * t : finp + (size_t)FinRec<L>::N * aux, h);
            }
        });
        const bool kfin = valid && ((m.fit && k->ao_samples && more) || (m.fitm && (more || !aux_ao_slot(ao_aux))));
        if (kfin) {
            reinterpret_cast<uint8_t*>(aocc)[late(t)] = (uint8_t)kFinFlag;
            hitmask[t >> 6] = 1ull;
        }
        if (m.fitm && more && aux_ao_slot(ao_aux))
            atomicOr(&q.ao_ctr[(ao_aux & 255u) >> 1], (1u << 10) << ((ao_aux & 1u) * 16u));
        if (__ballot(more)) {
            __builtin_amdgcn_s_waitcnt(0);
            push_long(more, st, t, aux);
        }
        if (m.fit || m.fitm) __builtin_amdgcn_s_waitcnt(0);
        for (int kk = 0; kk < k->ao_samples; ++kk) {
            March<L, true> ao;
            if (valid) ao_begin(c, h, (uint32_t)kk, ao);
            push_long(valid, ao, t, ao_aux);
        }
    };

    auto do_prepass = [&](const FrameTable* __restrict__ pft, uint32_t qt, bool own) {
        if constexpr (L == RT_NOMADPLAINS) {
            constexpr uint32_t LPR = RT_PREPASS_LPR, RPW = 64u / LPR;
            constexpr uint32_t WPF = RT_CAMERA_RES * RT_CAMERA_RES / RPW;
            const uint32_t f = qt / WPF;
            const uint32_t ray0 = (qt - f * WPF) * RPW;
            const uint32_t ray = ray0 + late(lane) / LPR;
            const uint32_t lid = late(lane);
            const uint32_t j = lid & (LPR - 1u), base = lid & ~(LPR - 1u);
            Ctx cp = c;
            cp.k = pft->kcam[0];
            cp.kf = (KPtr)pft->kcam[f];
            cp.eye = rtm::mk(uniform_f(cp.kf->eye[0]), uniform_f(cp.kf->eye[1]), uniform_f(cp.kf->eye[2]));
            cp.sun = rtm::mk(uniform_f(cp.kf->sun[0]), uniform_f(cp.kf->sun[1]), uniform_f(cp.kf->sun[2]));
            const uint32_t tx = ray % RT_CAMERA_RES, ty = ray / RT_CAMERA_RES;
            const float r31 = rtm::rcp(31.0f);
            const uint32_t pxs = (uint32_t)(((float)tx * r31) * cp.k->screen[0]);
            const uint32_t pys = (uint32_t)(((float)ty * r31) * cp.k->screen[1]);
            f3 p, dir;
            get_pixel_ray(cp, (float)pxs, (float)pys, &p, &dir);
            March<L, false> st;
            march_begin(cp, st, p, RT_CAMERA_NEAR, 2.0f, dir);
            const SegOctaves<LPR> g = seg_octaves<LPR>(cp, j);
            __builtin_amdgcn_s_setprio(RT_FUSE_PRIO);
            while (march_live<L, false, true>(cp, st, RT_CAMERA_FAR, 0)) {
                auto dens = [&](f3 q0) {
                    uint32_t used;
                    return density_nomadplains_seg<LPR, false>(cp, g, q0, j, base, &used);
                };
                march_step_with<L, false, true>(cp, st, dens);
            }
            __builtin_amdgcn_s_setprio(0);
            RayResult rr = march_result(st);
            if (rr.density < 0.0f) rr.pd.w = RT_CAMERA_FAR;
            if (j == 0u) {
                typedef float v4f __attribute__((ext_vector_type(4)));
                const v4f v = {rr.pd.x, rr.pd.y, rr.pd.z, rr.pd.w};
                float4* dst = pft->cam[f] + ray;
                asm volatile("global_store_dwordx4 %0, %1, off sc1" : : "v"(dst), "v"(v) : "memory");
            }
            asm volatile("s_waitcnt vmcnt(0)" : : : "memory");
            if (!own) {
                if (lane == 0) __hip_atomic_fetch_add(np.ctl + 1, RPW, __ATOMIC_RELAXED, __HIP_MEMORY_SCOPE_AGENT);
                return;
            }
            typedef uint32_t __attribute__((address_space(1))) guint;
            guint* gf = (guint*)(gp.gate + f * RT_GATE_WORDS);
            uint32_t old = 0;
            if (lane == 0) {
                const uint32_t task = ray0 / RT_FUSE_RAYS_PER_TASK;
                bool whole = true;
                if constexpr (RPW < RT_FUSE_RAYS_PER_TASK)
                    whole = __hip_atomic_fetch_add(gf + RT_GATE_TASKS + task, RPW, __ATOMIC_RELAXED,
                                                   __HIP_MEMORY_SCOPE_AGENT) == RT_FUSE_RAYS_PER_TASK - RPW;
                if (whole) {
                    __hip_atomic_fetch_or(gf + (task >> 5), 1u << (task & 31u), __ATOMIC_RELAXED, __HIP_MEMORY_SCOPE_AGENT);
                    old = __hip_atomic_fetch_add(gf + RT_GATE_CTR, (uint32_t)RT_FUSE_RAYS_PER_TASK, __ATOMIC_RELAXED,
                                                 __HIP_MEMORY_SCOPE_AGENT);
                }
            }
            if ((uint32_t)__builtin_amdgcn_readfirstlane(old) == RT_CAMERA_RES * RT_CAMERA_RES - RT_FUSE_RAYS_PER_TASK) {
                if (gp.debug & 2u) {
                    const uint64_t t0 = __builtin_amdgcn_s_memrealtime();
                    while (__builtin_amdgcn_s_memrealtime() - t0 < 20000ull) __builtin_amdgcn_s_sleep(8);
                }
                const float4* cam = pft->cam[f];
                typedef unsigned long long __attribute__((address_space(1))) gu64;
                gu64* cells = (gu64*)pft->cells[f];
                for (uint32_t c = late(lane); c < RT_CAMERA_RES * RT_CAMERA_RES; c += 64u) {
                    const float2 b = cell_bracket([&](int x, int y) { return cam_depth_sc1(cam, x, y); },
                                                  (int)(c % RT_CAMERA_RES), (int)(c / RT_CAMERA_RES));
                    __hip_atomic_store(cells + c, (unsigned long long)__float_as_uint(b.x) |
                                                      ((unsigned long long)__float_as_uint(b.y) << 32),
                                       __ATOMIC_RELAXED, __HIP_MEMORY_SCOPE_AGENT);
                }
                asm volatile("s_waitcnt vmcnt(0)" : : : "memory");
                if (lane == 0) __hip_atomic_store(gf + RT_GATE_CTR + 1, 1u, __ATOMIC_RELAXED, __HIP_MEMORY_SCOPE_AGENT);
            }
        }
    };

    typedef const uint32_t __attribute__((address_space(1))) gcuint;
    auto ld_sc1 = [&](const uint32_t* p) {
        return __hip_atomic_load((gcuint*)p, __ATOMIC_RELAXED, __HIP_MEMORY_SCOPE_AGENT);
    };
    auto tile_ready = [&](uint32_t e, uint32_t w0, uint32_t w1, uint32_t w2, uint32_t w3) -> bool {
        const uint32_t f = e >> 24, first = m.frame_rot ? (m.tile_first + f) % m.tile_stride : m.tile_first;
        const uint32_t T = (e & 0xffffffu) * m.tile_stride + first;
        const uint32_t gx = (T % m.tiles32_x) * 32u, gy = (T / m.tiles32_x) * 32u;
        const uint32_t px0 = gx + m.off_x, py0 = gy + m.off_y;
        if (gx >= m.ext_x || gy >= m.ext_y || px0 >= W || py0 >= H) return true;
        const uint32_t xe = m.off_x + m.ext_x < W ? m.off_x + m.ext_x : W, ye = m.off_y + m.ext_y < H ? m.off_y + m.ext_y : H;
        const uint32_t px1 = px0 + 31u < xe ? px0 + 31u : xe - 1u, py1 = py0 + 31u < ye ? py0 + 31u : ye - 1u;
        auto cell_of = [&](uint32_t p, float r) { return (int)rtm::floor(((float)p * r) * 32.0f); };
        const int cx0 = cell_of(px0, k->rcp_w) - 2, cx1 = cell_of(px1, k->rcp_w) + 2;
        const int cy0 = cell_of(py0, k->rcp_h) - 2, cy1 = cell_of(py1, k->rcp_h) + 2;
        const int xlo = cx0 < 0 ? 0 : cx0, xhi = cx1 > RT_CAMERA_RES - 1 ? RT_CAMERA_RES - 1 : cx1;
        const int ylo = cy0 < 0 ? 0 : cy0, yhi = cy1 > RT_CAMERA_RES - 1 ? RT_CAMERA_RES - 1 : cy1;
        const uint32_t g = ((2u << (xhi / RT_FUSE_RAYS_PER_TASK)) - 1u) & ~((1u << (xlo / RT_FUSE_RAYS_PER_TASK)) - 1u);
        bool ok = true;
        for (int r = ylo; r <= yhi; ++r) {
            const uint32_t w = (r >> 3) == 0 ? w0 : (r >> 3) == 1 ? w1 : (r >> 3) == 2 ? w2 : w3;
            ok = ok && ((w >> ((r & 7) * 4)) & g) == g;
        }
        return ok;
    };
    auto gated_fetch = [&](uint32_t* pf, uint32_t* pu) -> int {
        const uint32_t nt = n_total >> 4;
        bool gate_all = vload(q.gate_all) != 0u;
        if (!gate_all) {
            const uint32_t gw = lane < m.n_frames ? ld_u32(gp.gate, late(lane * RT_GATE_WORDS + RT_GATE_CTR))
                                                  : (uint32_t)(RT_CAMERA_RES * RT_CAMERA_RES);
            gate_all = __ballot(gw < (uint32_t)(RT_CAMERA_RES * RT_CAMERA_RES)) == 0ull;
            if (gate_all && lane == 0) q.gate_all = 1u;
        }
        if (gate_all) {
            for (int tries = 0; tries < 16; ++tries) {
                const uint32_t qi = wave_fetch(&counters[RT_CTR_PRIMARY], lane);
                if (qi >= n_total) return -1;
                uint32_t old = 0u;
                if (lane == 0) old = atomicOr(gp.claims + late(qi >> 4), 1u << (qi & 15u));
                if (!((__builtin_amdgcn_readfirstlane(old) >> (qi & 15u)) & 1u)) {
                    const uint32_t e = __builtin_amdgcn_readfirstlane(order[qi >> 4]);
                    *pf = e >> 24;
                    *pu = (e & 0xffffffu) * 16u + (qi & 15u);
                    return 1;
                }
            }
            return 0;
        }
        const uint32_t h = (uint32_t)__builtin_amdgcn_readfirstlane(ld_sc1(counters + RT_CTR_SCAN));
        if (h >= nt) return -1;
        const uint32_t gs = vload(q.gscan);
        const uint32_t base = gs > h && gs < nt ? gs : h;
        const uint32_t i = late(base + lane);
        uint32_t e = 0u, c = 0xffffu;
        if (i < nt) {
            e = ld_u32(order, i, false);
            c = ld_u32(gp.claims, i);
        }
        const bool left = (c & 0xffffu) != 0xffffu;
        const uint64_t lb = __ballot(left);
        if (base == h) {
            const uint32_t nh = lb ? base + (uint32_t)__builtin_ctzll(lb) : base + 64u;
            if (nh > h && lane == 0) atomicMax(counters + RT_CTR_SCAN, nh);
        }
        if (lane == 0) q.gscan = base + 64u;
        bool ready = left;
        if (left) {
            const uint32_t gw = (e >> 24) * RT_GATE_WORDS;
            ready = tile_ready(e, ld_u32(gp.gate, gw), ld_u32(gp.gate, gw + 1u), ld_u32(gp.gate, gw + 2u),
                               ld_u32(gp.gate, gw + 3u));
        }
        const uint64_t rdy = __ballot(ready);
        const uint32_t hw = __builtin_amdgcn_s_getreg((31 << 11) | 4);
        const uint64_t from = rdy & (~0ull << ((hw ^ (hw >> 6) ^ (hw >> 12)) & 63u));
        for (uint64_t rb = from ? from : rdy; rb; rb &= rb - 1ull) {
            const uint32_t l = (uint32_t)__builtin_ctzll(rb);
            uint32_t cl = (uint32_t)__builtin_amdgcn_readlane((int)c, (int)l) | 0xffff0000u;
            while (cl != 0xffffffffu) {
                const uint32_t kk = (uint32_t)__builtin_ctz(~cl);
                uint32_t old = 0u;
                if (lane == 0) old = atomicOr(gp.claims + late(base + l), 1u << kk);
                old = (uint32_t)__builtin_amdgcn_readfirstlane(old);
                if (!((old >> kk) & 1u)) {
                    const uint32_t el = (uint32_t)__builtin_amdgcn_readlane((int)e, (int)l);
                    *pf = el >> 24;
                    *pu = (el & 0xffffffu) * 16u + kk;
                    if (lane == 0) q.gscan = base;
                    return 1;
                }
                cl |= old;
            }
        }
        return 0;
    };

    auto do_unit = [&](uint32_t f, uint32_t u) {
        bool cells_in = true;
        if constexpr (GATED) {
            cells_in = (vload(q.gate_cells) >> f) & 1u;
            if (!cells_in && ld_sc1(gp.gate + f * RT_GATE_WORDS + RT_GATE_CTR + 1) != 0u) {
                cells_in = true;
                if (lane == 0) atomicOr(&q.gate_cells, 1u << f);
            }
        }
        Ctx cf = frame_ctx(c, ft, f);
        cf.nz.phase = RT_PHASE_PRIMARY;
        uint32_t px, py;
        const bool valid = unit_pixel(m, f, u, lane, W, H, &px, &py);
        const float pxf = (float)px, pyf = (float)py;
        float plane_x = 0.0f;
        if (valid) {
            float spx = pxf * k->rcp_w, spy = pyf * k->rcp_h;
            const uint32_t cell = (uint32_t)rtm::fma(rtm::floor(spy * 32.0f), 32.0f, rtm::floor(spx * 32.0f));
            if (GATED && !cells_in) {
                const float4* cam = ft->cam[f];
                plane_x = cell_bracket([&](int x, int y) { return cam_depth_sc1(cam, x, y); }, (int)(cell % RT_CAMERA_RES),
                                       (int)(cell / RT_CAMERA_RES)).x;
            } else if (GATED) {
                typedef const float __attribute__((address_space(1))) gcfloat;
                plane_x = __hip_atomic_load((gcfloat*)(ft->cells[f] + cell), __ATOMIC_RELAXED, __HIP_MEMORY_SCOPE_AGENT);
            } else {
                plane_x = gptr(ft->cells[f])[cell].x;
            }
        }
        [[maybe_unused]] const bool sky = kSky && k->sky_exit != 0;
        for (uint32_t a = 0; a < aa; ++a) {
            const uint32_t t = f * m.frame_samples + (u * 64u + lane) * aa + a;
            March<L, true> st;
            st.d = 0.0f;
            bool lv = false;
            if (valid) {
                f3 p, dir;
                get_pixel_ray(cf, pxf + k->aa_off[a][0], pyf + k->aa_off[a][1], &p, &dir);
                march_begin(cf, st, p, plane_x, 1.0f, dir);
                lv = true;
            }
            __builtin_amdgcn_s_setprio(0);
            uint32_t it = 0;
            while (lv) {
                lv = march_live<L, true, false>(cf, st, RT_CAMERA_FAR, max_steps);
                if (!lv) break;
                if constexpr (kSky) {
                    if (sky && sky_exit(st.p.y, st.dir.y, st.dist)) {
                        lv = false;
                        break;
                    }
                }
                [[maybe_unused]] const uint64_t lb = __ballot(1);
                RT_DIAG_LIVE_HIST(if (lane == (uint32_t)__builtin_ctzll(lb)) atomicAdd(&g_live_hist[__popcll(lb)], 1ull);)
                RT_DIAG_PRIMARY_STEPS({
                    cf.nz.phase = RT_COUNT_PHASE;
                    count_noise(cf.nz);
                    cf.nz.phase = RT_PHASE_PRIMARY;
                })
                if constexpr (L == RT_NOMADPLAINS && kPrimarySeg > 0u && (!STATS || kStatsPrimarySeg)) {
                    if ((uint32_t)__popcll(lb) <= kPrimarySeg) break;
                }
                march_step<L, true, false>(cf, st);
                if (it == 96u) __builtin_amdgcn_s_setprio(1);
                else if (it == 224u) __builtin_amdgcn_s_setprio(2);
                else if (it == 384u) __builtin_amdgcn_s_setprio(3);
                ++it;
            }
            if constexpr (L == RT_NOMADPLAINS && kPrimarySeg > 0u && (!STATS || kStatsPrimarySeg)) {
                if (const uint64_t lb = __ballot(lv)) primary_seg(cf, st, lv, lb, pxf + k->aa_off[a][0], pyf + k->aa_off[a][1], sky);
            }
            __builtin_amdgcn_s_setprio(0);
            const bool hit = valid && st.d > 0.0f;
            WT(if (valid) wp_maxit = max(wp_maxit, (uint32_t)st.iters);)
            RayResult rr;
            if (valid) {
                rr = march_result(st);
                stat(BlockStats::PRIMARY, (uint32_t)st.iters);
                if (!hit) {
                    const float4 v = miss_sample(cf, pxf + k->aa_off[a][0], pyf + k->aa_off[a][1], rr.pd.w, rr.fc);
                    if (aa == 1u) {
                        const uint32_t px8 = unorm8(v.x) | (unorm8(v.y) << 8) | (unorm8(v.z) << 16) | 0xff000000u;
                        if (m.packed) {
                            if (!(RT_DIAG_SKIP & 1)) gptr(ft->out8[f])[packed_index(late(u * 64u + lane))] = px8;
                        } else {
                            const size_t o = (size_t)py * W + px;
                            if (!(RT_DIAG_SKIP & 1)) gptr(ft->out8[f])[o] = px8;
                            if (float4* o32 = ft->out32[f]) gstore(o32 + o, make_float4(v.x, v.y, v.z, 1.0f));
                        }
                    } else {
                        samples[t] = v;
                    }
                }
            }
            const uint64_t hb = __ballot(hit);
            if (lane == 0) hitmask[(f * m.n_units + u) * aa + a] = (m.fit || m.fitm) ? 0ull : hb;
            if (hb) {
                const uint32_t n = (uint32_t)__popcll(hb), rank = lane_rank(hb);
                if (hit) stat(BlockStats::HITS, 1u);
                q_lock(&q.lock, lane);
                const uint32_t top = vload(q.h_top);
                const bool fits = (uint32_t)__builtin_amdgcn_readfirstlane(top) + n <= hit_cap;
                if (hit && fits) hit_store<L>(hq + (size_t)(top + rank) * HR, t, rr);
                __builtin_amdgcn_s_waitcnt(0);
                if (lane == 0) {
                    if (fits) q.h_top = top + n;
                    else q.overflow |= RT_FLAG_HIT_OVERFLOW;
                }
                q_unlock(&q.lock, lane);
            }
        }
        c.nz.calls = cf.nz.calls;
    };

    const uint32_t n_static = gridDim.x * (blockDim.x >> 6);
    const uint32_t first_qi = first_unit_index(counters, lane);
    bool first_unit = true;
    bool np_open = np.tasks != 0u;
    bool gp_open = GATED && gp.tasks != 0u;
    if constexpr (GATED) {
        if (gp.debug & 1u) {
            float acc = 0.0f;
            for (uint32_t f = 0; f < m.n_frames; ++f)
                for (uint32_t i = lane; i < RT_CAMERA_RES * RT_CAMERA_RES; i += 64u) acc += ft->cells[f][i].x;
            asm volatile("" : : "v"(acc));
        }
    }
    WT(wt[0] = __builtin_amdgcn_s_memrealtime();)
    for (;;) {
        if constexpr (L == RT_NOMADPLAINS) {
            if (GATED && gp_open) {
                const uint32_t qt = wave_fetch(&counters[RT_CTR_GATE], lane);
                if (qt < gp.tasks * kPrepassSplit) {
                    WT(const unsigned long long tp = __builtin_amdgcn_s_memrealtime();)
                    do_prepass(ft, qt, true);
                    WT(const unsigned long long tq = __builtin_amdgcn_s_memrealtime(); wt[21] += tq - tp; wt[22] = tq;)
                    continue;
                }
                gp_open = false;
            }
            if (np_open && !first_unit) {
                const uint32_t qt = wave_fetch(np.ctl, lane);
                if (qt < np.tasks * kPrepassSplit) {
                    do_prepass(np.ft, qt, false);
                    continue;
                }
                np_open = false;
            }
        }
        const uint32_t lp = queued_long();
        const uint32_t hp = queued_hits();
        const bool drained = vload(q.drained) != 0u;
        WT(const unsigned long long t0 = __builtin_amdgcn_s_memrealtime(); wt[12]++;
           wt[15] = t0; if (drained && wt[18] == 0) { wt[18] = t0; wt[19] = lp; wt[20] = hp; })
        const uint32_t lb_now = (RT_NEAR_UNITS > 0 && vload(q.near_end) != 0u) ? (uint32_t)RT_NEAR_LONG_BATCH : long_batch;
        if (lp >= lb_now || (drained && lp > 0u)) {
            if constexpr (L == RT_NOMADPLAINS && kSegLanes > 0u) {
                if (drained && lp <= kSegQueue) {
                    do_shadow_seg();
                    WT(const unsigned long long ds = __builtin_amdgcn_s_memrealtime() - t0; wt[4] += ds; wt[7]++;
                       wt[23] += ds; wt[24]++;)
                    continue;
                }
            }
            do_shadow();
            WT(const unsigned long long dl = __builtin_amdgcn_s_memrealtime() - t0; wt[4] += dl; wt[7]++; wt[27] += dl;)
            continue;
        }
        if (hp >= 64u || (drained && hp > 0u)) {
            if (lane == 0) atomicAdd(&q.active, 1u);
            do_shade();
            if (lane == 0) atomicSub(&q.active, 1u);
            WT(wt[3] += __builtin_amdgcn_s_memrealtime() - t0; wt[6]++;)
            continue;
        }
        if (GATED ? !drained : (!drained || first_unit)) {
            if (lane == 0) atomicAdd(&q.active, 1u);
            bool run = false;
            uint32_t f = 0, u = 0;
            if constexpr (GATED) {
                const int got = __builtin_amdgcn_readfirstlane(gated_fetch(&f, &u));
                run = got > 0;
                if (got < 0) {
                    if (lane == 0) q.drained = 1u;
                }
            } else {
                const uint32_t qi = first_unit ? first_qi : n_static + wave_fetch(&counters[RT_CTR_PRIMARY], lane);
                first_unit = false;
                if (RT_NEAR_UNITS > 0 && qi + (uint32_t)RT_NEAR_UNITS * n_static >= n_total && lane == 0) q.near_end = 1u;
                if (qi < n_total) {
                    const uint32_t e = __builtin_amdgcn_readfirstlane(order[qi >> 4]);
                    f = e >> 24;
                    u = (e & 0xffffffu) * 16u + (qi & 15u);
                    run = true;
                } else if (lane == 0) {
                    q.drained = 1u;
                }
            }
            WT(if (!run) wt[9] += __builtin_amdgcn_s_memrealtime() - t0;)
            if (run) {
                do_unit((uint32_t)__builtin_amdgcn_readfirstlane(f), (uint32_t)__builtin_amdgcn_readfirstlane(u));
                WT(const unsigned long long t1 = __builtin_amdgcn_s_memrealtime(); wt[2] += t1 - t0; wt[5]++; wt[8] = t1;)
            }
            if (lane == 0) atomicSub(&q.active, 1u);
            continue;
        }
        if (vload(q.active) == 0u && queued_long() == 0u && queued_hits() == 0u) break;
        __builtin_amdgcn_s_sleep(2);
        WT(wt[9] += __builtin_amdgcn_s_memrealtime() - t0;)
    }
    if (lane == 0) {
        const uint32_t ov = vload(q.overflow);
        if (ov) atomicOr(counters + RT_CTR_BYTES / 4, ov);
    }
    WT(wt[1] = __builtin_amdgcn_s_memrealtime();
       for (int o = 32; o >= 1; o >>= 1) {
           wl_rays += __shfl_xor(wl_rays, o, 64);
           wl_maxit = max(wl_maxit, (uint32_t)__shfl_xor(wl_maxit, o, 64));
           wp_maxit = max(wp_maxit, (uint32_t)__shfl_xor(wp_maxit, o, 64));
       }
       wt[13] = wl_rays; wt[14] = wl_maxit; wt[16] = wp_maxit;
       const uint32_t slot = blockIdx.x * (blockDim.x >> 6) + (threadIdx.x >> 6);
       if (lane < RT_WT_FIELDS && slot < RT_WT_MAX_WAVES) {
           unsigned long long v = 0;
           for (int f = 0; f < RT_WT_FIELDS; ++f) v = (lane == (uint32_t)f) ? wt[f] : v;
           g_wave_trace[slot * RT_WT_FIELDS + lane] = v;
       })
    if constexpr (STATS) {
        uint32_t done = 0;
        if (lane == 0) done = atomicAdd(&s_st.done, 1u);
        if (__builtin_amdgcn_readfirstlane(done) == (blockDim.x >> 6) - 1u && lane == 0) {
            atomicAdd(&stats->primary_steps, vload(s_st.v[BlockStats::PRIMARY]));
            atomicAdd(&stats->shadow_steps, vload(s_st.v[BlockStats::SHADOW]));
            atomicAdd(&stats->ao_steps, vload(s_st.v[BlockStats::AO]));
            atomicAdd(&stats->hits, vload(s_st.v[BlockStats::HITS]));
            atomicAdd(&stats->noise_calls, vload(s_st.v[BlockStats::NOISE]));
            atomicAdd(&stats->noise_waves, vload(s_st.v[BlockStats::NOISE_WAVES]));
        }
    }
}

__global__ void __launch_bounds__(1024) k_finish(const RtConsts* __restrict__ k, const FrameTable* __restrict__ ft,
                                                 UnitMap m, const uint64_t* __restrict__ hitmask,
                                                 const float4* __restrict__ samples, uint32_t* __restrict__ aocc)
{
    const uint32_t lane = threadIdx.x & 63u;
    const uint32_t W = (uint32_t)k->width, H = (uint32_t)k->height, aa = (uint32_t)k->aa_samples;
    const uint32_t n_waves = gridDim.x * (blockDim.x >> 6);
    const uint32_t total = m.n_units * m.n_frames;
    for (uint32_t g = blockIdx.x * (blockDim.x >> 6) + (threadIdx.x >> 6); g < total; g += n_waves) {
        const uint32_t f = __builtin_amdgcn_readfirstlane(g / m.n_units), u = g - f * m.n_units;
        auto* out8 = gptr(ft->out8[f]);
        float4* out32 = ft->out32[f];
        uint32_t px, py;
        if (!unit_pixel(m, f, u, lane, W, H, &px, &py)) continue;
        if (m.fit || m.fitm) {
            if (hitmask[f * m.n_units + u] == 0ull) continue;
            const uint32_t t = f * m.frame_samples + u * 64u + lane;
            if (!((aocc[t >> 2] >> ((t & 3u) * 8u)) & kFinFlag)) continue;
        } else if (aa == 1u && !((hitmask[f * m.n_units + u] >> lane) & 1ull)) {
            continue;
        }
        float c0 = 0.0f, c1 = 0.0f, c2 = 0.0f;
        for (uint32_t a = 0; a < aa; ++a) {
            const uint32_t t = f * m.frame_samples + (u * 64u + lane) * aa + a;
            float4 v;
            if (aa == 1u) {
                const float* c = reinterpret_cast<const float*>(samples) + 3u * t;
                v = make_float4(c[0], c[1], c[2], 1.0f);
            } else {
                v = samples[t];
            }
            if (v.w > 0.0f && k->ao_samples > 0) {
                const float ao = ao_factor(ao_occluded(aocc, t), k->ao_samples);
                v = make_float4(v.x * ao, v.y * ao, v.z * ao, v.w);
            }

            c0 = c0 + v.x;
            c1 = c1 + v.y;
            c2 = c2 + v.z;
        }
        if (k->ao_samples > 0) {
            const uint32_t t0 = f * m.frame_samples + (u * 64u + lane) * aa;
            for (uint32_t w = t0 >> 2; w <= (t0 + aa - 1u) >> 2; ++w) aocc[w] = 0u;
        }
        float ia = rtm::rcp((float)aa);
        c0 = c0 * ia;
        c1 = c1 * ia;
        c2 = c2 * ia;
        size_t o = out_index(m, u, lane, px, py, (uint32_t)k->width);
        if (!(RT_DIAG_SKIP & 64)) out8[o] = unorm8(c0) | (unorm8(c1) << 8) | (unorm8(c2) << 16) | 0xff000000u;
        if (out32) gstore(out32 + o, make_float4(c0, c1, c2, 1.0f));
    }
}

__global__ void __launch_bounds__(256) k_bgrx(const uint32_t* __restrict__ fb, uint32_t* __restrict__ dst, int w,
                                              int h, int pitch_words)
{
    const int quads = (w + 3) >> 2;
    const int y = blockIdx.y;
    for (int qx = blockIdx.x * blockDim.x + threadIdx.x; qx < quads; qx += gridDim.x * blockDim.x) {
        const int x = qx << 2;
        const uint32_t* src = fb + (size_t)y * w + x;
        uint32_t* out = dst + (size_t)y * pitch_words + x;
        constexpr uint32_t sel = 0x0c000102u;
        if (x + 4 <= w && ((w & 3) == 0) && ((pitch_words & 3) == 0)) {
            const uint4 v = *reinterpret_cast<const uint4*>(src);
            uint4 o;
            o.x = __builtin_amdgcn_perm(0u, v.x, sel);
            o.y = __builtin_amdgcn_perm(0u, v.y, sel);
            o.z = __builtin_amdgcn_perm(0u, v.z, sel);
            o.w = __builtin_amdgcn_perm(0u, v.w, sel);
            *reinterpret_cast<uint4*>(out) = o;
        } else {
            for (int i = 0; i < 4 && x + i < w; ++i) out[i] = __builtin_amdgcn_perm(0u, src[i], sel);
        }
    }
}

template <bool BGRX>
__global__ void __launch_bounds__(256) k_snapshot(const uint32_t* __restrict__ fb, uint32_t* __restrict__ dst,
                                                  uint32_t words)
{
    constexpr uint32_t sel = 0x0c000102u;
    const uint32_t quads = words >> 2;
    const uint32_t q = blockIdx.x * 256u + threadIdx.x;
    if (q < quads) {
        uint4 v = reinterpret_cast<const uint4*>(fb)[q];
        if (BGRX) {
            v.x = __builtin_amdgcn_perm(0u, v.x, sel);
            v.y = __builtin_amdgcn_perm(0u, v.y, sel);
            v.z = __builtin_amdgcn_perm(0u, v.z, sel);
            v.w = __builtin_amdgcn_perm(0u, v.w, sel);
        }
        reinterpret_cast<uint4*>(dst)[q] = v;
    } else if (q == quads) {
        for (uint32_t i = quads << 2; i < words; ++i) dst[i] = BGRX ? __builtin_amdgcn_perm(0u, fb[i], sel) : fb[i];
    }
}

__global__ void __launch_bounds__(256) k_shard_copy(ShardJobs jobs, int w, int h, int count, int pack)
{
    const int job = blockIdx.y;
    const int tiles_x = (w + 31) / 32, total = tiles_x * ((h + 31) / 32);
    const int tile = (int)blockIdx.x * count + jobs.shard[job];
    if (tile >= total) return;
    const int r = (int)threadIdx.x >> 3, c = ((int)threadIdx.x & 7) * 4;
    const int x = (tile % tiles_x) * 32 + c, y = (tile / tiles_x) * 32 + r;
    if (y >= h || x >= w) return;
    uint32_t* fb = jobs.fb[job] + (size_t)y * w + x;
    uint32_t* pk = jobs.packed[job] + (size_t)blockIdx.x * 1024 + r * 32 + c;
    if (x + 3 < w && (((uintptr_t)fb | (uintptr_t)pk) & 15u) == 0) {
        if (pack) *reinterpret_cast<uint4*>(pk) = *reinterpret_cast<const uint4*>(fb);
        else *reinterpret_cast<uint4*>(fb) = *reinterpret_cast<const uint4*>(pk);
    } else {
        for (int i = 0; i < 4 && x + i < w; ++i) {
            if (pack) pk[i] = fb[i];
            else fb[i] = pk[i];
        }
    }
}

template <int L>
void launch_camerarays_l(const RtLaunch& a, float4* out, const FrameTable* ft, uint32_t n)
{
    if constexpr (L == RT_NOMADPLAINS) {
        auto go = [&](auto bs_tag, auto lpr_tag) {
            constexpr int BS = decltype(bs_tag)::value, LPR = decltype(lpr_tag)::value;
            dim3 grid(RT_CAMERA_RES * RT_CAMERA_RES / (BS / LPR), n), block(BS);
            if (a.stats)
                hipLaunchKernelGGL((k_camerarays_group<true, BS, LPR>), grid, block, 0, a.stream, a.consts, a.perm2d,
                                   a.grad, out, a.stats, ft);
            else
                hipLaunchKernelGGL((k_camerarays_group<false, BS, LPR>), grid, block, 0, a.stream, a.consts,
                                   a.perm2d, a.grad, out, a.stats, ft);
        };
        using C512 = std::integral_constant<int, 512>;
        using L32 = std::integral_constant<int, 32>;
        if (n <= 2) go(std::integral_constant<int, RT_PREPASS_BS1>{}, std::integral_constant<int, RT_PREPASS_LPR1>{});
        else if (n <= 4) go(C512{}, L32{});
        else if (n <= 16) go(C512{}, std::integral_constant<int, 8>{});
        else go(C512{}, std::integral_constant<int, 4>{});
        return;
    }
    dim3 grid(RT_CAMERA_RES * RT_CAMERA_RES / 64, n), block(64);
    if (a.stats)
        hipLaunchKernelGGL((k_camerarays<L, true>), grid, block, 0, a.stream, a.consts, a.perm2d, a.grad, out, a.stats,
                           ft);
    else
        hipLaunchKernelGGL((k_camerarays<L, false>), grid, block, 0, a.stream, a.consts, a.perm2d, a.grad, out, a.stats,
                           ft);
}

template <int L>
void launch_split_l(const RtLaunch& a, uint32_t ox, uint32_t oy, uint32_t ex, uint32_t ey, uint32_t first,
                    uint32_t stride)
{
    UnitMap m;
    uint32_t tiles_x = (ex + 31) / 32, tiles_y = (ey + 31) / 32, total = tiles_x * tiles_y;
    const uint32_t rot = a.n_frames > 1u && stride > 1u ? 1u : 0u;
    if (!rot && first >= total) return;
    m.off_x = ox;
    m.off_y = oy;
    m.ext_x = ex;
    m.ext_y = ey;
    m.tiles32_x = tiles_x;
    m.tile_first = first;
    m.tile_stride = stride;
    m.n_units = ((total - (rot ? 0u : first) + stride - 1) / stride) * 16u;
    m.frame_rot = rot;
    m.n_frames = a.n_frames;
    m.frame_samples = m.n_units * 64u * (uint32_t)a.aa;
    uint32_t blocks = (uint32_t)(a.num_cus > 0 ? a.num_cus : 256);
    uint32_t need = (m.n_units * m.n_frames + 15u) / 16u;
    uint32_t pblocks = need < blocks ? need : blocks;
    m.order_batch = RT_ORDER_BATCH >= 0 ? (uint32_t)RT_ORDER_BATCH
                                        : (uint32_t)(m.n_frames > 1u && m.n_units < kOrderBatchUnitsPerWave * pblocks * 16u);
    uint32_t fblocks = need < 2u * blocks ? need : 2u * blocks;
    dim3 blk(1024);
    m.cells_from_cam = (uint32_t)a.cells_from_cam;
    m.fit = (uint32_t)a.fit;
    m.fitm = kAoSlots > 0u ? (uint32_t)a.fitm : 0u;
    m.packed = (uint32_t)a.packed;
    hipLaunchKernelGGL(k_order, dim3(m.order_batch ? 1u : m.n_frames), blk, 0, a.stream, a.frames, m, a.order, a.queue,
                       a.wait_ctl, a.wait_total, a.fuse_next.ctl, a.host_flag, a.gated.tasks ? a.gated.gate : nullptr,
                       a.gated.claims);
    if (a.after_order) (void)hipEventRecord(a.after_order, a.stream);
    if (a.after_order_fuse) (void)hipEventRecord(a.after_order_fuse, a.stream);
    auto primary = [&](auto stats_tag) {
        constexpr bool S = decltype(stats_tag)::value;
        const RtConsts* k0 = a.frames_host.k[0];
        constexpr bool kCanGate = L == RT_NOMADPLAINS && !S;
        auto* kern = (kCanGate && a.gated.tasks) ? k_trace<L, S, kCanGate> : k_trace<L, S, false>;
        hipLaunchKernelGGL(kern, dim3(pblocks), dim3(TraceThreads<L>::value), 0, a.stream, k0, a.frames,
                           a.perm2d, a.grad, m,
                           a.order, a.hitmask, a.samples, a.fin, a.finpool, a.cpool, a.hitq, a.spill_long, a.hit_cap,
                           a.long_spill_cap, a.aocc, a.queue, a.stats, kLongBatch, kRefillIdle, kCompactLive,
                           a.small_rings ? 64u : kLongRing, a.small_rings ? 8u : kFinSlots, a.fuse_next, a.gated);
        if (!(m.fit && a.ao_samples == 0))
            hipLaunchKernelGGL(k_finish, dim3(fblocks), blk, 0, a.stream, k0, a.frames, m, a.hitmask, a.samples, a.aocc);
    };
    if (a.stats) primary(std::true_type{});
    else primary(std::false_type{});
}

}

void rt_launch_camerarays(const RtLaunch& a, float4* out)
{
    switch (a.landscape) {
    case RT_TESTING: launch_camerarays_l<RT_TESTING>(a, out, nullptr, 1u); break;
    case RT_SIMPLE: launch_camerarays_l<RT_SIMPLE>(a, out, nullptr, 1u); break;
    case RT_GREENROCKS: launch_camerarays_l<RT_GREENROCKS>(a, out, nullptr, 1u); break;
    default: launch_camerarays_l<RT_NOMADPLAINS>(a, out, nullptr, 1u); break;
    }
}

void rt_launch_camerarays_batch(const RtLaunch& a)
{
    switch (a.landscape) {
    case RT_TESTING: launch_camerarays_l<RT_TESTING>(a, nullptr, a.frames, a.n_frames); break;
    case RT_SIMPLE: launch_camerarays_l<RT_SIMPLE>(a, nullptr, a.frames, a.n_frames); break;
    case RT_GREENROCKS: launch_camerarays_l<RT_GREENROCKS>(a, nullptr, a.frames, a.n_frames); break;
    default: launch_camerarays_l<RT_NOMADPLAINS>(a, nullptr, a.frames, a.n_frames); break;
    }
}

void rt_launch_tracescreen(const RtLaunch& a, uint32_t ox, uint32_t oy, uint32_t ex, uint32_t ey, uint32_t first,
                           uint32_t stride)
{
    if (ex == 0 || ey == 0 || stride == 0) return;
    switch (a.landscape) {
    case RT_TESTING: launch_split_l<RT_TESTING>(a, ox, oy, ex, ey, first, stride); break;
    case RT_SIMPLE: launch_split_l<RT_SIMPLE>(a, ox, oy, ex, ey, first, stride); break;
    case RT_GREENROCKS: launch_split_l<RT_GREENROCKS>(a, ox, oy, ex, ey, first, stride); break;
    default: launch_split_l<RT_NOMADPLAINS>(a, ox, oy, ex, ey, first, stride); break;
    }
}

void rt_launch_bgrx(hipStream_t s, const uint32_t* fb, uint32_t* dst, int w, int h, int pitch_words)
{
    const int quads = (w + 3) / 4;
    const int bx = (quads + 255) / 256;
    hipLaunchKernelGGL(k_bgrx, dim3(bx, h), dim3(256), 0, s, fb, dst, w, h, pitch_words);
}

void rt_launch_snapshot(hipStream_t s, const uint32_t* fb, uint32_t* dst, size_t words, int bgrx)
{
    if (words == 0 || words > 0xffffffffull) return;
    const uint32_t n = (uint32_t)words;
    const uint32_t threads = (n >> 2) + ((n & 3u) ? 1u : 0u);
    const uint32_t blocks = (threads + 255u) / 256u;
    if (bgrx) hipLaunchKernelGGL(k_snapshot<true>, dim3(blocks), dim3(256), 0, s, fb, dst, n);
    else hipLaunchKernelGGL(k_snapshot<false>, dim3(blocks), dim3(256), 0, s, fb, dst, n);
}

void rt_launch_shard_copy(hipStream_t s, const ShardJobs& jobs, int n, int w, int h, int count, int pack)
{
    if (n <= 0 || n > RT_SHARD_JOBS) return;
    const size_t tiles = rt_shard_tiles(w, h, 0, count);
    if (tiles == 0) return;
    hipLaunchKernelGGL(k_shard_copy, dim3((unsigned)tiles, (unsigned)n), dim3(256), 0, s, jobs, w, h, count, pack);
}

namespace {

template <int V>
using Int = std::integral_constant<int, V>;

template <class F>
void with_landscape(const RtLaunch& a, F f)
{
    switch (a.landscape) {
    case RT_TESTING: f(Int<RT_TESTING>{}); break;
    case RT_SIMPLE: f(Int<RT_SIMPLE>{}); break;
    case RT_GREENROCKS: f(Int<RT_GREENROCKS>{}); break;
    default: f(Int<RT_NOMADPLAINS>{}); break;
    }
}

template <class F>
void with_bool(bool b, F f)
{
    if (b) f(std::true_type{});
    else f(std::false_type{});
}

template <class F>
bool with_segment(int bs, int lpr, F f)
{
    if (bs == RT_PREPASS_BS1 && lpr == RT_PREPASS_LPR1) f(Int<RT_PREPASS_BS1>{}, Int<RT_PREPASS_LPR1>{});
    else if (bs == 512 && lpr == 32) f(Int<512>{}, Int<32>{});
    else if (bs == 512 && lpr == 8) f(Int<512>{}, Int<8>{});
    else if (bs == 512 && lpr == 4) f(Int<512>{}, Int<4>{});
    else return false;
    return true;
}

}

namespace {

#ifdef RT_QUERY_UTIL
__device__ unsigned long long g_query_util[4];
#endif

struct QueryRay {
    f3 p, dir;
    float t0, endd;
};

struct RayArgs {
    QueryEye eye;
};
template <bool STEPS>
struct RayPolicy {
    using Args = RayArgs;
    static constexpr bool SKIPREFINE = true, NORMAL = false, kSteps = STEPS;
    static __device__ __forceinline__ QueryRay ray(const Args&, float4 o, float4 d)
    {
        return QueryRay{rtm::mk(o.x, o.y, o.z), rtm::mk(d.x, d.y, d.z), RT_CAMERA_NEAR, RT_CAMERA_FAR};
    }
    static __device__ __forceinline__ float t_max(const Args&) { return RT_CAMERA_FAR; }
    static __device__ __forceinline__ float stepmod(const Args&) { return 2.0f; }
    static __device__ __forceinline__ int max_steps(const Args&) { return 0; }
    template <class M, class Normal>
    static __device__ __forceinline__ void store(const M& st, float4* __restrict__ out, uint32_t* __restrict__ steps,
                                                 uint32_t i, Normal)
    {
        RayResult rr = march_result(st);
        if (rr.density < 0.0f) rr.pd.w = RT_CAMERA_FAR;
        gstore(out + i, make_float4(rr.pd.x, rr.pd.y, rr.pd.z, rr.pd.w));
        if constexpr (STEPS) steps[i] = (uint32_t)st.iters;
    }
};

struct SurfArgs {
    QueryEye eye;
    float t_min, t_max, stepmod;
    int max_steps;
};
template <bool STEPS, bool RANGE>
struct SurfPolicy {
    using Args = SurfArgs;
    static constexpr bool SKIPREFINE = false, NORMAL = true, kSteps = STEPS;
    static __device__ __forceinline__ QueryRay ray(const Args& a, float4 o, float4 d)
    {
        return QueryRay{rtm::mk(o.x, o.y, o.z), rtm::mk(d.x, d.y, d.z), RANGE ? o.w : a.t_min, RANGE ? d.w : a.t_max};
    }
    static __device__ __forceinline__ float t_max(const Args& a) { return a.t_max; }
    static __device__ __forceinline__ float stepmod(const Args& a) { return a.stepmod; }
    static __device__ __forceinline__ int max_steps(const Args& a) { return a.max_steps; }
    template <class M, class Normal>
    static __device__ __forceinline__ void store(const M& st, float4* __restrict__ out, uint32_t* __restrict__ steps,
                                                 uint32_t i, Normal normal)
    {
        const RayResult rr = march_result(st);
        f3 nrm = rtm::mk(0.0f, 0.0f, 0.0f);
        if (rr.density > 0.0f) nrm = normal(f4{rr.pd.x, rr.pd.y, rr.pd.z, rr.density});
        gstore(out + 2 * (size_t)i, make_float4(rr.pd.x, rr.pd.y, rr.pd.z, rr.pd.w));
        gstore(out + 2 * (size_t)i + 1, make_float4(nrm.x, nrm.y, nrm.z, rr.density));
        if constexpr (STEPS) steps[i] = (uint32_t)st.iters;
    }
};

template <class P, int BS, int LPR>
__global__ void __launch_bounds__(BS) k_query_seg(const RtConsts* __restrict__ k, const uint32_t* __restrict__ perm2d,
                                                  const float4* __restrict__ grad, const float4* __restrict__ rays,
                                                  float4* __restrict__ out, uint32_t* __restrict__ steps, uint32_t n,
                                                  typename P::Args a)
{
    constexpr int L = RT_NOMADPLAINS;
    __shared__ __attribute__((aligned(16))) uint32_t lds[kNoiseLdsWords];
    load_noise_lds(lds, perm2d, grad, k);
    const uint32_t i = blockIdx.x * (uint32_t)(BS / LPR) + threadIdx.x / (uint32_t)LPR;
    if (i >= n) return;
    Ctx c = make_ctx(k, lds, a.eye);
    const uint32_t j = threadIdx.x & (LPR - 1u), base = threadIdx.x & 63u & ~(LPR - 1u);
    const SegOctaves<LPR> g = seg_octaves<LPR>(c, j);
    const QueryRay r = P::ray(a, rays[2 * (size_t)i], rays[2 * (size_t)i + 1]);
    auto dens = [&](f3 q) {
        uint32_t used;
        return density_nomadplains_seg<LPR>(c, g, q, j, base, &used);
    };
    March<L, false> st;
    march_begin(c, st, r.p, r.t0, P::stepmod(a), r.dir);
    while (march_live<L, false, P::SKIPREFINE>(c, st, r.endd, P::max_steps(a)))
        march_step_with<L, false, P::SKIPREFINE>(c, st, dens);
    if constexpr (P::NORMAL) {
        const RayResult rr = march_result(st);
        f3 nrm = rtm::mk(0.0f, 0.0f, 0.0f);
        if (rr.density > 0.0f) nrm = get_normal_with(c, f4{rr.pd.x, rr.pd.y, rr.pd.z, rr.density}, dens);
        if (j == 0) {
            gstore(out + 2 * (size_t)i, make_float4(rr.pd.x, rr.pd.y, rr.pd.z, rr.pd.w));
            gstore(out + 2 * (size_t)i + 1, make_float4(nrm.x, nrm.y, nrm.z, rr.density));
            if constexpr (P::kSteps) steps[i] = (uint32_t)st.iters;
        }
    } else {
        if (j == 0) P::store(st, out, steps, i, 0);
    }
}

template <int L, class P>
__global__ void __launch_bounds__(1024) k_query_lanes(const RtConsts* __restrict__ k, const uint32_t* __restrict__ perm2d,
                                                      const float4* __restrict__ grad, const float4* __restrict__ rays,
                                                      float4* __restrict__ out, uint32_t* __restrict__ steps, uint32_t n,
                                                      typename P::Args a, uint32_t* __restrict__ counter,
                                                      uint32_t refill_live)
{
    RT_DIAG_QUERY_UTIL(uint32_t util_wave = 0, util_lane = 0, util_nwave = 0, util_nlane = 0;)
    __shared__ __attribute__((aligned(16))) uint32_t lds[kNoiseLdsWords];
    load_noise_lds(lds, perm2d, grad, k);
    Ctx c = make_ctx(k, lds, a.eye);
    const uint32_t lane = threadIdx.x & 63u;
    auto normal = [&](f4 pd) { return get_normal<L>(c, pd); };
    March<L, false> st{};
    float endd = P::t_max(a);
    uint32_t idx = 0;
    bool has = false, live = false;
    bool more = true;
    for (;;) {
        uint64_t lv = __ballot(live);
        if (more && (uint32_t)__popcll(lv) <= refill_live) {
            const uint32_t cnt = 64u - (uint32_t)__popcll(lv);
            const uint32_t first = wave_fetch(counter, lane, cnt);
            RT_DIAG_QUERY_UTIL(if (const uint64_t nm = __ballot(!live && has && st.d > 0.0f); P::NORMAL && nm) {
                ++util_nwave;
                util_nlane += (uint32_t)__popcll(nm);
            })
            if (!live) {
                if (has) P::store(st, out, steps, idx, normal);
                idx = first + lane_rank(~lv);
                has = idx < n;
                if (has) {
                    const QueryRay r = P::ray(a, rays[2 * (size_t)idx], rays[2 * (size_t)idx + 1]);
                    endd = r.endd;
                    march_begin(c, st, r.p, r.t0, P::stepmod(a), r.dir);
                    live = march_live<L, false, P::SKIPREFINE>(c, st, endd, P::max_steps(a));
                }
            }
            more = first + cnt < n;
            lv = __ballot(live);
        }
        if (!lv) {
            if (!more) break;
            continue;
        }
        RT_DIAG_QUERY_UTIL(++util_wave; util_lane += (uint32_t)__popcll(lv);)
        if (live) {
            march_step<L, false, P::SKIPREFINE>(c, st);
            live = march_live<L, false, P::SKIPREFINE>(c, st, endd, P::max_steps(a));
        }
    }
    RT_DIAG_QUERY_UTIL(if (const uint64_t nm = __ballot(has && st.d > 0.0f); P::NORMAL && nm) {
        ++util_nwave;
        util_nlane += (uint32_t)__popcll(nm);
    })
    if (has) P::store(st, out, steps, idx, normal);
    RT_DIAG_QUERY_UTIL(if (lane == 0) {
        atomicAdd(&g_query_util[0], (unsigned long long)util_wave);
        atomicAdd(&g_query_util[1], (unsigned long long)util_lane);
        atomicAdd(&g_query_util[2], (unsigned long long)util_nwave);
        atomicAdd(&g_query_util[3], (unsigned long long)util_nlane);
    })
}

SurfArgs surf_args(const float eye[3], const RtMarchParams& m)
{
    return SurfArgs{{eye[0], eye[1], eye[2]}, m.t_min, m.t_max, m.stepmod, m.max_steps};
}

template <class F>
void with_steps_range(bool steps, bool range, F f)
{
    with_bool(steps, [&](auto steps_tag) { with_bool(range, [&](auto range_tag) { f(steps_tag, range_tag); }); });
}

template <class F>
void with_policy(const RtTraceQuery& q, F f)
{
    with_steps_range(q.steps != nullptr, q.surface && q.march.ray_range, [&](auto steps_tag, auto range_tag) {
        constexpr bool STEPS = decltype(steps_tag)::value, RANGE = decltype(range_tag)::value;
        if (q.surface) f((SurfPolicy<STEPS, RANGE>*)nullptr, surf_args(q.eye, q.march));
        else if constexpr (!RANGE) f((RayPolicy<STEPS>*)nullptr, RayArgs{{q.eye[0], q.eye[1], q.eye[2]}});
    });
}

}

bool rt_launch_tracequery(const RtLaunch& a, const RtTraceQuery& q)
{
    if (q.n == 0 || q.blocks == 0) return true;
    if (q.lpr > 1 && a.landscape != RT_NOMADPLAINS) return false;
    constexpr uint32_t thr = RT_RAYQ_REFILL < 63 ? RT_RAYQ_REFILL : 63;
    bool found = true;
    with_policy(q, [&](auto* policy, auto args) {
        using P = std::remove_pointer_t<decltype(policy)>;
        if (q.lpr > 1) {
            found = with_segment(q.bs, q.lpr, [&](auto bs_tag, auto lpr_tag) {
                constexpr int BS = decltype(bs_tag)::value, LPR = decltype(lpr_tag)::value;
                hipLaunchKernelGGL((k_query_seg<P, BS, LPR>), dim3(q.blocks), dim3(BS), 0, a.stream, a.consts, a.perm2d,
// ... 878 lines not shown
```

gpgpuraytrace_amd/csrc/rt_runtime.cpp:

```cpp
#include <hip/hip_runtime.h>

#include <arpa/inet.h>
#include <netinet/in.h>
#include <sys/socket.h>
#include <unistd.h>

#include <algorithm>
#include <atomic>
#include <cmath>
#include <cstdarg>
#include <cstdio>
#include <cstring>
#include <deque>
#include <map>
#include <memory>
#include <mutex>
#include <string>
#include <thread>
#include <vector>

#include "../../include/frosttrace.h"
#include "rt_kernels.h"
#include "rt_math.h"
#include "rt_noise.h"
// ... 2128 lines not shown

int rt_terrain_render_batch_packed(const rt_compute* cams, const rt_compute* scrs, int n, int shard_rank,
                                   int shard_count, void* dst_device, size_t frame_stride)
{
    if (!dst_device || shard_count < 2) return fail(RT_ERR_INVALID, "packed output: a device buffer and shard_count >= 2");
    if (cams && scrs && n >= 1 && scrs[0] && scrs[0]->dev) {
        const rt_device d = scrs[0]->dev;
        size_t need = 0;
        for (int f = 0; f < n; ++f) {
            const int sh = n > 1 ? (shard_rank + f) % shard_count : shard_rank;
            need = std::max(need, rt_shard_tiles(d->width, d->height, sh, shard_count) * RT_TILE * RT_TILE * 4);
        }
        if (frame_stride < need || frame_stride % 16) return fail(RT_ERR_INVALID, "packed output: frame_stride %zu < %zu bytes "
                                                                   "or not 16-byte aligned", frame_stride, need);
    }
    TraceOpts o;
    o.prepass = true;
    o.packed_dst = (uint8_t*)dst_device;
    o.packed_stride = frame_stride;
    o.shard = Shard{shard_rank, shard_count};
    return batch_trace(Frames{cams, scrs, n}, o);
}

int rt_terrain_prepass_batch(const rt_compute* cams, const rt_compute* scrs, int n, int first, int count,
                             void* camera_out)
{
    PrepassOpts o;
    o.first = first;
    o.count = count;
    o.camera_out = (float4*)camera_out;
    return batch_prepass(Frames{cams, scrs, n}, o);
}

int rt_terrain_trace_batch(const rt_compute* cams, const rt_compute* scrs, int n, int shard_rank, int shard_count,
                           const void* camera_in)
{
    if (!camera_in) return fail(RT_ERR_INVALID, "camera_in: the batch's gathered CameraResults");
    TraceOpts o;
    o.camera_in = (const float4*)camera_in;
    o.shard = Shard{shard_rank, shard_count};
    return batch_trace(Frames{cams, scrs, n}, o);
}

int rt_terrain_prepass_ahead(const rt_compute* cams, const rt_compute* scrs, int n)
{
    if (!cams || !scrs || n < 1 || n > RT_MAX_BATCH) return fail(RT_ERR_INVALID, "a batch holds 1..%d frames", RT_MAX_BATCH);
    for (int f = 0; f < n; ++f)
        if (!cams[f] || !scrs[f] || cams[f]->dev != scrs[f]->dev) return fail(RT_ERR_INVALID, "computes must share a device");
    rt_device lead = scrs[0]->dev;
    const Frames fr{cams, scrs, n};
    if (int rc0 = devices_enter(fr)) return rc0;
    if (lead->flags & RT_DEVICE_GRAPH) return fail(RT_ERR_STATE, "the ahead prepass runs on a side stream: not with RT_DEVICE_GRAPH");
    if (lead->ahead_pending) return fail(RT_ERR_STATE, "a prepass is already ahead for this device's batch: trace it first");
    if (lead->fuse_state == rt_device_s::FUSE_FUSED && lead->ev_fuser_done) {
        HIP_TRY(hipStreamWaitEvent(lead->stream, lead->ev_fuser_done, 0));
    }
    fuse_forget(lead);
    lead->fuse_state = rt_device_s::FUSE_NONE;
    HIP_TRY(hipSetDevice(lead->ordinal));
    hipStream_t side = ahead_stream(lead->ordinal, true);
    if (!side) return fail(RT_ERR_HIP, "side stream");
    if (int rc = ensure_event(lead->ev_order)) return rc;
    if (int rc = ensure_event(lead->ev_ahead)) return rc;
    if (!lead->order_recorded) {
        HIP_TRY(hipEventRecord(lead->ev_order, lead->stream));
        lead->order_recorded = true;
    }
    HIP_TRY(hipStreamWaitEvent(side, lead->ev_order, 0));
    const Shader* s0 = scrs[0]->shader;
    const bool fuse = s0 && s0->landscape == RT_NOMADPLAINS && !(lead->flags & RT_DEVICE_STATS);
    rt_device devs[RT_MAX_BATCH];
    int n_devs = 0;
    for (int f = 0; f < n; ++f)
        if (std::find(devs, devs + n_devs, scrs[f]->dev) == devs + n_devs) devs[n_devs++] = scrs[f]->dev;
    int rc;
    {
        StreamRedirect on_side(devs, n_devs, side);
        rc = fuse ? batch_stage(fr) : batch_prepass(fr, PrepassOpts{});
    }
    if (rc) return rc;
    HIP_TRY(hipEventRecord(lead->ev_ahead, side));
    lead->ahead_pending = true;
    lead->ahead_cams.assign(cams, cams + n);
    lead->fuse_devs.clear();
    for (int i = 0; i < n_devs; ++i) {
        rt_device d = devs[i];
        if (int rc = ensure_event(d->ev_ahead_in)) return rc;
        HIP_TRY(hipEventRecord(d->ev_ahead_in, side));
        d->ahead_in_pending = true;
        lead->fuse_devs.push_back(d);
    }
    if (fuse) {
        lead->fuse_state = rt_device_s::FUSE_STAGED;
        lead->fuse_n = n;
        std::lock_guard<std::mutex> lk(g_stream_mu);
        g_fuse_staged[lead->ordinal].push_back(lead);
    }
    return RT_OK;
}

int rt_terrain_trace_ahead(const rt_compute* cams, const rt_compute* scrs, int n, int shard_rank, int shard_count)
{
    if (!cams || !scrs || n < 1 || n > RT_MAX_BATCH || !scrs[0] || !scrs[0]->shader) return fail(RT_ERR_INVALID, "a batch holds 1..%d frames", RT_MAX_BATCH);
    rt_device lead = scrs[0]->dev;
    const Frames fr{cams, scrs, n};
    if (int rc0 = devices_enter(fr)) return rc0;
    HIP_TRY(hipSetDevice(lead->ordinal));
    bool ahead = lead->ahead_pending && (size_t)n <= lead->ahead_cams.size();
    for (int f = 0; ahead && f < n; ++f)
        ahead = cams[f] == lead->ahead_cams[f] && cams[f]->shader && !cams[f]->shader->cb_dirty;
    TraceOpts o;
    TraceFuse& tf = o.fuse;
    o.prepass = true;
    o.shard = Shard{shard_rank, shard_count};
    const int state = lead->fuse_state;
    if (ahead && state == rt_device_s::FUSE_FUSED) {
        HIP_TRY(hipStreamWaitEvent(lead->stream, lead->ev_fuse_order, 0));
        tf.wait_ctl = lead->fctl;
        tf.wait_total = (uint32_t)lead->fuse_n * (uint32_t)(RT_CAMERA_RES * RT_CAMERA_RES);
        for (rt_device d : lead->fuse_devs) d->ahead_in_pending = false;
        o.prepass = false;
    } else if (ahead && state == rt_device_s::FUSE_NONE) {
        HIP_TRY(hipStreamWaitEvent(lead->stream, lead->ev_ahead, 0));
        o.prepass = false;
    }
    fuse_forget(lead);
    lead->fuse_state = rt_device_s::FUSE_NONE;
    lead->ahead_pending = false;
    rt_device z = nullptr;
    const Shader* s0 = scrs[0]->shader;
    const size_t frame_tiles = rt_shard_tiles(lead->width, lead->height, 0, 1);
    const bool runs_trace = (n > 1 && shard_count > 1) || (size_t)shard_rank < frame_tiles;
    if (runs_trace && s0->landscape == RT_NOMADPLAINS && !(lead->flags & (RT_DEVICE_STATS | RT_DEVICE_GRAPH))) {
        std::lock_guard<std::mutex> lk(g_stream_mu);
        auto& v = g_fuse_staged[lead->ordinal];
        for (auto it = v.begin(); it != v.end(); ++it) {
            rt_device c = *it;
            const rt_compute cz = c->ahead_cams.empty() ? nullptr : (rt_compute)c->ahead_cams[0];
            if (c == lead || c->width != lead->width || c->height != lead->height || !cz || !cz->shader ||
                cz->shader->landscape != RT_NOMADPLAINS || !same_tables(cz->shader, s0))
                continue;
            z = c;
            v.erase(it);
            break;
        }
    }
    if (z) {
        HIP_TRY(hipStreamWaitEvent(lead->stream, z->ev_ahead, 0));
        const uint32_t tasks = (lead->flags & RT_DEVICE_DEBUG_WITHHOLD_FUSE)
                                   ? 0u : (uint32_t)z->fuse_n * (uint32_t)RT_FUSE_TASKS_PER_FRAME;
        tf.next = FusedPrepass{z->fuse_table.d, z->fctl, tasks};
        if (int rc = ensure_event(z->ev_fuse_order)) return rc;
        tf.next_after_order = z->ev_fuse_order;
    }
    int rc = batch_trace(fr, o);
    if (z) {
        if (rc) {
            std::lock_guard<std::mutex> lk(g_stream_mu);
            g_fuse_staged[z->ordinal].insert(g_fuse_staged[z->ordinal].begin(), z);
            return rc;
        }
        if (int rc = ensure_event(z->ev_fuser_done)) return rc;
        HIP_TRY(hipEventRecord(z->ev_fuser_done, lead->stream));
        z->fuse_state = rt_device_s::FUSE_FUSED;
        for (rt_device d : z->fuse_devs) {
            HIP_TRY(hipEventRecord(d->ev_ahead_in, lead->stream));
            d->ahead_in_pending = true;
        }
    }
    return rc;
}

size_t rt_shard_bytes(rt_device d, int rank, int count)
{
    if (!d || count < 1 || rank < 0 || rank >= count) return 0;
    size_t tiles = rt_shard_tiles(d->width, d->height, rank, count);
    return tiles * RT_TILE * RT_TILE * 4;
}

static int shard_copy(const rt_device* devs, const int* shards, int count, void* const* bufs, int n, int pack)
{
    if (!devs || !shards || !bufs || n < 0 || count < 1) return fail(RT_ERR_INVALID, "bad arguments");
    if (n == 0) return RT_OK;
    rt_device d0 = devs[0];
    if (d0 && host_flag_check(d0)) return RT_ERR_STATE;
    for (int i = 0; i < n; ++i) {
        if (!devs[i] || !bufs[i] || shards[i] < 0 || shards[i] >= count) return fail(RT_ERR_INVALID, "bad arguments");
        if (int rc = defer_flush(devs[i])) return rc;
        if (devs[i]->width != d0->width || devs[i]->height != d0->height)
            return fail(RT_ERR_INVALID, "shard batch: devices differ in size");
    }
    auto order = [&](rt_device from, rt_device to) -> int {
        if (int rc = ensure_event(from->sync_ev)) return rc;
        HIP_TRY(hipEventRecord(from->sync_ev, from->stream));
        HIP_TRY(hipStreamWaitEvent(to->stream, from->sync_ev, 0));
        return RT_OK;
    };
    int rc;
    for (int i = 1; i < n; ++i)
        if (devs[i]->stream != d0->stream && (rc = order(devs[i], d0))) return rc;
    ShardJobs jobs;
    for (int b = 0; b < n; b += RT_SHARD_JOBS) {
        const int m = n - b < RT_SHARD_JOBS ? n - b : RT_SHARD_JOBS;
        for (int j = 0; j < m; ++j) {
            jobs.fb[j] = devs[b + j]->fb8;
            jobs.packed[j] = (uint32_t*)bufs[b + j];
            jobs.shard[j] = shards[b + j];
        }
        rt_launch_shard_copy(d0->stream, jobs, m, d0->width, d0->height, count, pack);
    }
    HIP_TRY(hipGetLastError());
    bool others = false;
    for (int i = 1; i < n; ++i) others |= devs[i]->stream != d0->stream;
    if (others) {
        if (int rc = ensure_event(d0->sync_ev)) return rc;
        HIP_TRY(hipEventRecord(d0->sync_ev, d0->stream));
        for (int i = 1; i < n; ++i)
            if (devs[i]->stream != d0->stream) HIP_TRY(hipStreamWaitEvent(devs[i]->stream, d0->sync_ev, 0));
    }
    return RT_OK;
}

int rt_shard_pack(rt_device d, int rank, int count, void* dst)
{
    return shard_copy(&d, &rank, count, &dst, 1, 1);
}

int rt_shard_unpack(rt_device d, int rank, int count, const void* src)
{
    void* p = const_cast<void*>(src);
    return shard_copy(&d, &rank, count, &p, 1, 0);
}

int rt_shard_pack_batch(const rt_device* devs, const int* shard_ranks, int shard_count, void* const* dst_device, int n)
{
    return shard_copy(devs, shard_ranks, shard_count, dst_device, n, 1);
}

int rt_shard_unpack_batch(const rt_device* devs, const int* shard_ranks, int shard_count,
                          const void* const* src_device, int n)
{
    return shard_copy(devs, shard_ranks, shard_count, const_cast<void* const*>(src_device), n, 0);
}

int rt_noise_generate(uint32_t seed, int rand_kind, uint8_t* perm2d, float* grad)
{
    if (!perm2d || !grad) return fail(RT_ERR_INVALID, "null output");
    if (rand_kind != 0 && rand_kind != 1) return fail(RT_ERR_INVALID, "rand_kind must be 0 (MSVC) or 1 (glibc)");
    rt_noise::generate(seed, rand_kind, perm2d, grad);
    return RT_OK;
}

}

namespace {
float host_depth(const float* cr, int x, int y)
{
    if (x < 0) x = 0;
    if (x >= RT_CAMERA_RES) x = RT_CAMERA_RES - 1;
    if (y < 0) y = 0;
    if (y >= RT_CAMERA_RES) y = RT_CAMERA_RES - 1;
    return cr[(y * RT_CAMERA_RES + x) * 4 + 3];
}
float host_depth_interp(const float* cr, int x, int y)
{
    if (x < 0) { float m = host_depth(cr, x + 1, y); float d = host_depth(cr, x + 2, y) - m; return m - d; }
    if (x >= RT_CAMERA_RES) { float m = host_depth(cr, x - 1, y); float d = host_depth(cr, x - 2, y) - m; return m - d; }
    if (y < 0) { float m = host_depth(cr, x, y + 1); float d = host_depth(cr, x, y + 2) - m; return m - d; }
    if (y >= RT_CAMERA_RES) { float m = host_depth(cr, x, y - 1); float d = host_depth(cr, x, y - 2) - m; return m - d; }
    return host_depth(cr, x, y);
}
}

extern "C" int rt_terrain_set_target_depths(const float* cr, float* cells)
{
    if (!cr || !cells) return fail(RT_ERR_INVALID, "null arguments");
    for (int x = 0; x < RT_CAMERA_RES * RT_CAMERA_RES; ++x) {
        int xpos = x % RT_CAMERA_RES, ypos = x / RT_CAMERA_RES;
        float dmin = host_depth_interp(cr, xpos, ypos);
        float dmax = dmin;
        for (int xp = -2; xp <= 2; ++xp)
            for (int yp = -2; yp <= 2; ++yp) {
                float d = host_depth_interp(cr, xpos + xp, ypos + yp);
                dmin = std::min(d, dmin);
                dmax = std::max(d, dmax);
            }
        dmin = dmin * 0.96f - 0.01f;
        dmax = dmax * 1.22f + 0.4f;
        dmin = std::max(RT_CAMERA_NEAR, dmin);
        dmax = std::min(RT_CAMERA_FAR, dmax);
        cells[2 * x] = dmin;
        cells[2 * x + 1] = dmax;
    }
    return RT_OK;
}

extern "C" int rt_debug_sky_ceiling(const float* np_rcp, int n_oct, float expo, const float* grad, int n_grad,
                                    double* ceiling)
{
    if (!np_rcp || n_oct < 0 || (grad && n_grad < 0)) return fail(RT_ERR_INVALID, "bad arguments");
    return sky_ceiling(np_rcp, n_oct, expo, grad, n_grad, ceiling);
}

extern "C" int rt_debug_math(rt_device d, int op, const float* a, const float* b, float* y, int n)
{
    if (!d || !a || !y || n <= 0) return fail(RT_ERR_INVALID, "bad arguments");
    float *da = nullptr, *db = nullptr, *dy = nullptr;
    if (op == 12) {
        HIP_TRY(hipMalloc(&da, 4));
        HIP_TRY(hipMalloc(&dy, 12));
        HIP_TRY(hipMemcpy(da, a, 4, hipMemcpyHostToDevice));
        HIP_TRY(hipMemsetAsync(dy, 0, 12, d->stream));
        rt_launch_debug_math(d->stream, op, da, da, dy, n);
        HIP_TRY(hipGetLastError());
        HIP_TRY(hipStreamSynchronize(d->stream));
        HIP_TRY(hipMemcpy(y, dy, 12, hipMemcpyDeviceToHost));
        HIP_TRY(hipFree(da));
        HIP_TRY(hipFree(dy));
        return RT_OK;
    }
    if (op == 14) {
        const size_t in = (size_t)n * 12, out = (size_t)n * 4;
        HIP_TRY(hipMalloc(&da, in));
        HIP_TRY(hipMalloc(&dy, out));
        HIP_TRY(hipMemcpy(da, a, in, hipMemcpyHostToDevice));
        rt_launch_debug_math(d->stream, op, da, da, dy, n);
        HIP_TRY(hipGetLastError());
        HIP_TRY(hipStreamSynchronize(d->stream));
        HIP_TRY(hipMemcpy(y, dy, out, hipMemcpyDeviceToHost));
        HIP_TRY(hipFree(da));
        HIP_TRY(hipFree(dy));
        RtConsts k;
        consts_np_octaves(k);
        double C;
        sky_ceiling(k.np_rcp + 1, RT_NP_OCTAVES, k.np_expo, nullptr, 0, &C);
        y[n] = std::nextafter((float)C, INFINITY);
        return RT_OK;
    }
    size_t bytes = (size_t)n * 4;
    HIP_TRY(hipMalloc(&da, bytes));
    HIP_TRY(hipMalloc(&db, bytes));
    HIP_TRY(hipMalloc(&dy, bytes));
    HIP_TRY(hipMemcpy(da, a, bytes, hipMemcpyHostToDevice));
    HIP_TRY(hipMemcpy(db, b ? b : a, bytes, hipMemcpyHostToDevice));
    rt_launch_debug_math(d->stream, op, da, db, dy, n);
    HIP_TRY(hipGetLastError());
    HIP_TRY(hipStreamSynchronize(d->stream));
    HIP_TRY(hipMemcpy(y, dy, bytes, hipMemcpyDeviceToHost));
    HIP_TRY(hipFree(da));
    HIP_TRY(hipFree(db));
    HIP_TRY(hipFree(dy));
    return RT_OK;
}

extern "C" int rt_debug_noise(rt_compute c, const float* xyz, float* out, int n, int density)
{
    if (!c || !c->shader || !xyz || !out || n <= 0) return fail(RT_ERR_INVALID, "bad arguments");
    rt_device dev = c->dev;
    int rc;
    if ((rc = check_texture(c->shader)) || (rc = sync_shader(dev, c->shader))) return rc;
    float *dx = nullptr, *dy = nullptr;
    HIP_TRY(hipMalloc(&dx, (size_t)n * 12));
    HIP_TRY(hipMalloc(&dy, (size_t)n * 4));
    HIP_TRY(hipMemcpyAsync(dx, xyz, (size_t)n * 12, hipMemcpyHostToDevice, dev->stream));
    rt_launch_debug_noise(make_launch(dev, c->shader), dx, dy, n, density);
    HIP_TRY(hipGetLastError());
    HIP_TRY(hipMemcpyAsync(out, dy, (size_t)n * 4, hipMemcpyDeviceToHost, dev->stream));
    HIP_TRY(hipStreamSynchronize(dev->stream));
    HIP_TRY(hipFree(dx));
    HIP_TRY(hipFree(dy));
    return RT_OK;
}

extern "C" int rt_debug_sky(rt_compute c, const float* dirs, float* out, int n)
{
    if (!c || !c->shader || !dirs || !out || n <= 0) return fail(RT_ERR_INVALID, "bad arguments");
    rt_device dev = c->dev;
    int rc;
    if ((rc = check_texture(c->shader)) || (rc = sync_shader(dev, c->shader))) return rc;
    float *dx = nullptr, *dy = nullptr;
    HIP_TRY(hipMalloc(&dx, (size_t)n * 12));
    HIP_TRY(hipMalloc(&dy, (size_t)n * 28));
    HIP_TRY(hipMemcpyAsync(dx, dirs, (size_t)n * 12, hipMemcpyHostToDevice, dev->stream));
    rt_launch_debug_sky(make_launch(dev, c->shader), dx, dy, n);
    HIP_TRY(hipGetLastError());
    HIP_TRY(hipMemcpyAsync(out, dy, (size_t)n * 28, hipMemcpyDeviceToHost, dev->stream));
    HIP_TRY(hipStreamSynchronize(dev->stream));
    HIP_TRY(hipFree(dx));
    HIP_TRY(hipFree(dy));
    return RT_OK;
}

namespace {

int sync_query_consts(rt_device dev, Shader* s, float default_eye[3], const float* sky_eye = nullptr)
{
    Shader::QueryConsts& q = s->query;
    if (!q.d_consts) HIP_TRY(hipMalloc(&q.d_consts, sizeof(RtConsts)));
    if (!q.d_grad) HIP_TRY(hipMalloc(&q.d_grad, 128 * sizeof(float4)));
    RtConsts hk;
    std::vector<uint8_t> grad(128 * sizeof(float4), 0);
    {
        std::lock_guard<std::mutex> lk(g_cb_mu);
        build_consts(*s, *dev, hk);
        const auto& nz = s->cb[CB_NOISE];
        memcpy(grad.data(), nz.data(), std::min(grad.size(), nz.size()));
    }
    for (int i = 0; i < 3; ++i) default_eye[i] = hk.eye[i];
    if (sky_eye) {
        for (int i = 0; i < 3; ++i) hk.eye[i] = sky_eye[i];
        consts_sky_eye(hk);
    }
    if (q.valid && !memcmp(&hk, &q.last, sizeof(RtConsts)) && grad == q.grad_last) return RT_OK;
    q.valid = false;
    if (int rc = q.consts_staging.upload(dev->stream, q.d_consts, &hk, sizeof(RtConsts))) return rc;
    if (int rc = q.grad_staging.upload(dev->stream, q.d_grad, grad.data(), grad.size())) return rc;
    q.last = hk;
    q.grad_last = grad;
    q.valid = true;
    return RT_OK;
}

int query_prepare(rt_compute c, const rtq::Options& o, bool sky_eye, RtLaunch* a, float eye[3])
{
    const float* opt_eye = (o.flags & rtq::kEye) ? o.eye : nullptr;
    if (int rc = sync_query_consts(c->dev, c->shader, eye, sky_eye ? opt_eye : nullptr)) return rc;
    if (opt_eye) memcpy(eye, opt_eye, 3 * sizeof(float));
    *a = make_launch(c->dev, c->shader);
    a->consts = c->shader->query.d_consts;
    a->grad = c->shader->query.d_grad;
    return RT_OK;
}

int arm_counter(rt_device dev, uint32_t** counter)
{
    if (!dev->rq_counter) HIP_TRY(hipMalloc(&dev->rq_counter, 64));
    HIP_TRY(hipMemsetAsync(dev->rq_counter, 0, 4, dev->stream));
    *counter = dev->rq_counter;
    return RT_OK;
}

int query_launched(bool launched, const char* no_kernel)
{
    if (!launched) return fail(RT_ERR_UNSUPPORTED, "%s", no_kernel);
    HIP_TRY(hipGetLastError());
    return RT_OK;
}

int cus_of(rt_device dev) { return dev->num_cus - dev->reserve_cus; }

RtMarchParams march_params(const rtq::SurfOptions& o)
{
    return RtMarchParams{o.t_min, o.t_max, o.stepmod, rtq::surface_max_steps(o.max_steps),
                         (o.flags & rtq::kSurfRayRange) != 0};
}

template <class Opt>
struct QueryFamily {
    const char* name;
    const char* counted;
    int (*parse)(const void*, Opt*, const char**);
};

template <class Opt, class Clause, class Run>
int query_entry(rt_compute c, const QueryFamily<Opt>& f, int count, const void* opt, Clause clause, const char* missing,
                Run run)
{
    if (!c) return fail(RT_ERR_INVALID, "null compute");
    const char* why = "";
    if (f.counted && rtq::check_count(count, &why))
        return fail(RT_ERR_INVALID, "%s: the %s count must be 0..2^26", f.name, f.counted);
    Opt o;
    if (int rc = f.parse(opt, &o, &why)) return fail(rc, "%s: %s", f.name, why);
    if (!c->shader) return fail(RT_ERR_STATE, "no current shader");
    uint32_t n = (uint32_t)count;
    if (int rc = clause(o, &n)) return rc;
    if (n > 0 && missing) return fail(RT_ERR_INVALID, "%s", missing);
    if (int rc = check_texture(c->shader)) return rc;
    if (int rc = host_flag_check(c->dev)) return rc;
    if (n == 0) return RT_OK;
    HIP_TRY(hipSetDevice(c->dev->ordinal));
    return run(o, n);
}

template <class Opt>
auto segments_clause(rt_compute c, const char* name)
{
    return [=](const Opt& o, uint32_t*) -> int {
        if ((o.flags & rtq::kForceSegments) && c->shader->landscape != RT_NOMADPLAINS)
            return fail(RT_ERR_UNSUPPORTED, "%s: the segment shape exists for nomadplains only", name);
        return RT_OK;
    };
}

struct HostPart {
    size_t bytes;
    const void* src;
    void* dst;
};

template <int N, class Enqueue>
int host_form(rt_device dev, const HostPart (&parts)[N], Enqueue enqueue)
{
    static_assert(N <= rtq::kBlockParts, "a part more than the layout holds");
    size_t bytes[N];
    for (int i = 0; i < N; ++i) bytes[i] = parts[i].bytes;
    const rtq::BlockLayout lay = rtq::block_layout(bytes, N);
    char* d = nullptr;
    HIP_TRY(hipMalloc(&d, lay.total));
    char* at[N];
    for (int i = 0; i < N; ++i) at[i] = bytes[i] ? d + lay.offset[i] : nullptr;
    auto run = [&]() -> int {
        for (int i = 0; i < N; ++i)
            if (at[i] && parts[i].src)
                HIP_TRY(hipMemcpyAsync(at[i], parts[i].src, bytes[i], hipMemcpyHostToDevice, dev->stream));
        if (int rc = enqueue(at)) return rc;
        for (int i = 0; i < N; ++i)
            if (at[i] && parts[i].dst)
                HIP_TRY(hipMemcpyAsync(parts[i].dst, at[i], bytes[i], hipMemcpyDeviceToHost, dev->stream));
        HIP_TRY(hipStreamSynchronize(dev->stream));
        return RT_OK;
    };
    const int rc = run();
    if (rc) (void)hipStreamSynchronize(dev->stream);
    (void)hipFree(d);
    return rc;
}

std::vector<float> pack_surface_rays(const float* origins, const float* dirs, const float* ranges, uint32_t n,
                                     rtq::SurfOptions* o)
{
    if (ranges) o->flags |= rtq::kSurfRayRange;
    else o->flags &= ~rtq::kSurfRayRange;
    std::vector<float> packed((size_t)n * 8);
    rtq::pack(origins, dirs, (int)n, packed.data());
    if (ranges) rtq::pack_ranges(ranges, (int)n, packed.data());
    return packed;
}

int trace_rays_enqueue(rt_compute c, const void* rays_device, uint32_t n, const rtq::Options& o, void* results_device,
                       void* steps_device)
{
    rt_device dev = c->dev;
    RtLaunch a;
    RtTraceQuery q{};
    if (int rc = query_prepare(c, o, false, &a, q.eye)) return rc;
    rtq::Plan p;
    const char* why = "";
    if (int rc = rtq::plan((int)n, a.landscape == RT_NOMADPLAINS, o.flags, o.max_blocks, cus_of(dev), RT_PREPASS_BS1,
                           RT_PREPASS_LPR1, &p, &why))
        return fail(rc, "rt_terrain_trace_rays: %s", why);
    q.rays = (const float4*)rays_device;
    q.results = (float4*)results_device;
    q.steps = (uint32_t*)steps_device;
    q.n = n;
    q.bs = p.bs;
    q.lpr = p.lpr;
    q.blocks = p.blocks;
    if (p.shape == rtq::LANES)
        if (int rc = arm_counter(dev, &q.counter)) return rc;
    return query_launched(rt_launch_tracequery(a, q), "rt_terrain_trace_rays: no kernel for this shape");
}

const QueryFamily<rtq::Options> kRayFamily{"rt_terrain_trace_rays", "ray", rtq::parse_options};

}

extern "C" int rt_terrain_trace_rays_device(rt_compute c, const void* rays_device, int n, const rt_ray_options* opt,
                                            void* results_device, void* steps_device)
{
    return query_entry(
        c, kRayFamily, n, opt, segments_clause<rtq::Options>(c, kRayFamily.name),
        !rays_device || !results_device ? "rt_terrain_trace_rays_device: null rays or results" : nullptr,
        [&](const rtq::Options& o, uint32_t nr) {
            return trace_rays_enqueue(c, rays_device, nr, o, results_device, steps_device);
        });
}

extern "C" int rt_terrain_trace_rays(rt_compute c, const float* origins, const float* dirs, int n,
                                     const rt_ray_options* opt, float* results, uint32_t* steps)
{
    return query_entry(
        c, kRayFamily, n, opt, segments_clause<rtq::Options>(c, kRayFamily.name),
        !origins || !dirs || !results ? "rt_terrain_trace_rays: null origins, dirs or results" : nullptr,
        [&](const rtq::Options& o, uint32_t nr) {
            std::vector<float> packed((size_t)nr * 8);
            rtq::pack(origins, dirs, n, packed.data());
            const HostPart parts[] = {{nr * rtq::kRayBytes, packed.data(), nullptr},
                                      {nr * rtq::kRayResultBytes, nullptr, results},
                                      {steps ? nr * rtq::kStepsBytes : 0, nullptr, steps}};
            return host_form(c->dev, parts,
                             [&](char* const* at) { return trace_rays_enqueue(c, at[0], nr, o, at[1], at[2]); });
        });
}

namespace {

int trace_surface_enqueue(rt_compute c, const void* rays_device, uint32_t n, const rtq::SurfOptions& o,
                          void* results_device, void* steps_device)
{
    rt_device dev = c->dev;
    RtLaunch a;
    RtTraceQuery q{};
    if (int rc = query_prepare(c, o, false, &a, q.eye)) return rc;
    rtq::Plan p;
    const char* why = "";
// ... 1044 lines not shown
```

gpgpuraytrace_amd/csrc/rt_types.h:

```cpp
#pragma once

#include <stdint.h>

enum { RT_NOMADPLAINS = 0, RT_TESTING = 1, RT_SIMPLE = 2, RT_GREENROCKS = 3, RT_NUM_LANDSCAPES = 4 };

#define RT_CAMERA_RES 32
#define RT_CAMERA_NEAR 0.01f
#define RT_CAMERA_FAR 5000.0f
#define RT_NP_OCTAVES 17
#define RT_NOISE_BOUND 1.05f
#define RT_SKY_CEIL 256.0f
#define RT_COL_OCTAVES 20

struct RtConsts {
    float eye[4];
    float view_inverse[16];
    float screen[2];
    float proj11, proj22;
    float rcp_w, rcp_h;
    float sun[3];
    float step_factor, one_minus_step_factor, density_factor, min_limit;
    float np_scale[RT_NP_OCTAVES + 1];
    float np_scale_y[RT_NP_OCTAVES + 1];
    float np_rcp[RT_NP_OCTAVES + 1];
    float np_expo;
    float col_scale[RT_COL_OCTAVES + 1];
    float col_rcp[RT_COL_OCTAVES + 1];
    float albedo[4];
    float shadow_color[3], one_minus_shadow[3];
    float rcp200;
    float sky_dist_to_top, sky_start[3], sky_start_n[3], sky_depth0, sky_rcp_samples, sky_fscale, sky_sos;
    float sky_att[3], sky_mie_k[3], sky_km_esun, sky_mie_a, sky_two_g, sky_one_plus_g2;
    float aa_off[16][2];
    int32_t aa_samples;
    int32_t landscape;
    int32_t max_steps;
    int32_t ao_samples;
    int32_t width, height;
    int32_t sky_exit;
    int32_t pad[2];
};

struct RtStats {
    unsigned long long primary_steps;
    unsigned long long shadow_steps;
    unsigned long long prepass_steps;
    unsigned long long hits;
    unsigned long long noise_calls;
    unsigned long long ao_steps;
    unsigned long long noise_waves;
};
```

include/frosttrace.h:

```cpp
#ifndef FROSTTRACE_H
#define FROSTTRACE_H

#include <stddef.h>
#include <stdint.h>

#ifdef __cplusplus
extern "C" {
#endif

#define RT_ABI_VERSION 9

enum {
    RT_OK = 0,
    RT_ERR_INVALID = -1,
    RT_ERR_HIP = -2,
    RT_ERR_NOT_FOUND = -3,
    RT_ERR_UNSUPPORTED = -4,
    RT_ERR_STATE = -5
};

enum {
    RT_DEVICE_FLOAT_OUTPUT = 1u,
    RT_DEVICE_STATS = 2u,
    RT_DEVICE_GRAPH = 4u,
    RT_DEVICE_DEBUG_SMALL_RINGS = 32u,
    RT_DEVICE_DEBUG_WITHHOLD_FUSE = 64u,
    RT_DEVICE_GATED = 128u,
    RT_DEVICE_DEBUG_GATE_STRESS = 512u,
    RT_DEVICE_DEFERRED = 1024u,
    RT_DEVICE_DEBUG_DEFER_SMALL = 2048u
};

enum { RT_TEXTURE_1D = 0, RT_TEXTURE_2D = 1, RT_TEXTURE_3D = 2 };
enum { RT_FORMAT_UNKNOWN = 0, RT_FORMAT_R8G8B8A8_SNORM = 1, RT_FORMAT_R8G8B8A8_UNORM = 2, RT_FORMAT_R8G8B8A8_UINT = 3 };

typedef struct rt_device_s* rt_device;
typedef struct rt_compute_s* rt_compute;
typedef struct rt_texture_s* rt_texture;
typedef struct rt_variable_s* rt_variable;
typedef struct rt_array_s* rt_array;
typedef struct rt_recorder_s* rt_recorder;

typedef struct {
    unsigned long long primary_steps;
    unsigned long long shadow_steps;
    unsigned long long prepass_steps;
    unsigned long long hits;
    unsigned long long noise_calls;
    unsigned long long ao_steps;
    unsigned long long noise_wave_iters;
} rt_stats;

const char* rt_last_error(void);
int rt_abi_version(void);

int rt_vfs_add_path(const char* path);
int rt_vfs_clear(void);

int rt_device_create(int ordinal, int width, int height, unsigned flags, rt_device* out);
void rt_device_destroy(rt_device dev);
int rt_device_present(rt_device dev);
int rt_device_flush(rt_device dev);
int rt_device_synchronize(rt_device dev);
int rt_device_readback(rt_device dev, void* dst, size_t row_pitch);
int rt_device_readback_float(rt_device dev, float* dst);
int rt_device_readback_bgrx(rt_device dev, void* dst, size_t row_pitch);
int rt_device_size(rt_device dev, int* width, int* height);
void* rt_device_framebuffer(rt_device dev);
void* rt_device_stream(rt_device dev);
int rt_device_set_stream(rt_device dev, void* hip_stream);
int rt_stream_refs(void* hip_stream);
int rt_device_stats(rt_device dev, rt_stats* out, int reset);
int rt_device_stats_sized(rt_device dev, rt_stats* out, size_t size, int reset);
int rt_device_set_profiling(rt_device dev, int enable);
int rt_device_kernel_time(rt_device dev, double* total_ms, int* launches);
int rt_device_graph_info(rt_device dev, unsigned long long* captures, unsigned long long* launches);
enum { RT_INFO_GATED_LAUNCHES = 0, RT_INFO_PREPASS_LAUNCHES = 1, RT_INFO_PRESTREAM_RENDERS = 2, RT_INFO_DEFERRED_FUSED = 3 };
int rt_device_info(rt_device dev, int key, unsigned long long* out);
int rt_device_reserve_cus(rt_device dev, int n);
int rt_device_defer_batch(rt_device dev, int frames);
int rt_device_wait_event(rt_device dev, void* hip_event);
int rt_device_record_event(rt_device dev, void* hip_event);
int rt_device_check(rt_device dev);

enum { RT_READBACK_RGBA8 = 0, RT_READBACK_BGRX = 1 };
typedef struct rt_readback_s* rt_readback;
int rt_readback_create(rt_device dev, int format, int depth, rt_readback* out);
int rt_readback_submit(rt_readback rb, unsigned long long* ticket);
int rt_readback_ready(rt_readback rb, unsigned long long ticket);
int rt_readback_wait(rt_readback rb, unsigned long long ticket, const void** pixels);
int rt_readback_release(rt_readback rb, unsigned long long ticket);
void rt_readback_destroy(rt_readback rb);

int rt_texture_create(rt_device dev, rt_texture* out);
int rt_texture_init(rt_texture tex, int dimensions, int format, int width, int height, const void* data,
                    int binding, int cpu_access);
void rt_texture_destroy(rt_texture tex);

int rt_compute_create(rt_device dev, rt_compute* out);
void rt_compute_destroy(rt_compute cs);
int rt_compute_load(rt_compute cs, const char* directory, const char* file, const char* entry, int tx, int ty, int tz,
                    const char* const* macro_names, const char* const* macro_values, int n_macros);
int rt_compute_swap(rt_compute cs);
int rt_compute_run(rt_compute cs, unsigned dispatch_x, unsigned dispatch_y, unsigned dispatch_z);
int rt_compute_set_texture(rt_compute cs, int stage, rt_texture tex);
int rt_compute_thread_size(rt_compute cs, int* x, int* y, int* z);
rt_variable rt_compute_get_variable(rt_compute cs, const char* name);
rt_array rt_compute_get_array(rt_compute cs, const char* name);
void* rt_compute_get_buffer(rt_compute cs, const char* name);

int rt_variable_write(rt_variable var, const void* data);
size_t rt_variable_size(rt_variable var);
const char* rt_variable_name(rt_variable var);

int rt_array_create(rt_array arr, unsigned elements);
void* rt_array_map(rt_array arr);
int rt_array_unmap(rt_array arr);
int rt_array_write(rt_array arr, const void* data);
size_t rt_array_stride(rt_array arr);
void* rt_array_device_pointer(rt_array arr);

int rt_terrain_render(rt_compute camera_cs, rt_compute screen_cs, int shard_rank, int shard_count);
int rt_terrain_render_feed(rt_compute camera_cs, rt_compute screen_cs, int shard_rank, int shard_count);
int rt_terrain_feed_wait(rt_compute camera_cs, float* camera_results);
int rt_terrain_render_batch(const rt_compute* camera_cs, const rt_compute* screen_cs, int n, int shard_rank,
                            int shard_count);
int rt_terrain_render_batch_packed(const rt_compute* camera_cs, const rt_compute* screen_cs, int n, int shard_rank,
                                   int shard_count, void* dst_device, size_t frame_stride);
int rt_terrain_prepass_batch(const rt_compute* camera_cs, const rt_compute* screen_cs, int n, int first, int count,
                             void* camera_out);
int rt_terrain_trace_batch(const rt_compute* camera_cs, const rt_compute* screen_cs, int n, int shard_rank,
                           int shard_count, const void* camera_in);
int rt_terrain_prepass_ahead(const rt_compute* camera_cs, const rt_compute* screen_cs, int n);
int rt_terrain_trace_ahead(const rt_compute* camera_cs, const rt_compute* screen_cs, int n, int shard_rank,
                           int shard_count);
size_t rt_shard_bytes(rt_device dev, int shard_rank, int shard_count);
int rt_shard_pack(rt_device dev, int shard_rank, int shard_count, void* dst_device);
int rt_shard_unpack(rt_device dev, int shard_rank, int shard_count, const void* src_device);
int rt_shard_pack_batch(const rt_device* devs, const int* shard_ranks, int shard_count, void* const* dst_device,
                        int n);
int rt_shard_unpack_batch(const rt_device* devs, const int* shard_ranks, int shard_count,
                          const void* const* src_device, int n);

int rt_noise_generate(uint32_t seed, int rand_kind, uint8_t* perm2d, float* grad);
int rt_terrain_set_target_depths(const float* camera_results, float* cell_distance);

enum { RT_RAYS_EYE = 1, RT_RAYS_FORCE_SEGMENTS = 2, RT_RAYS_FORCE_LANES = 4 };
typedef struct {
    uint32_t size;
    uint32_t flags;
    float eye[3];
    uint32_t max_blocks;
} rt_ray_options;
int rt_terrain_trace_rays(rt_compute cs, const float* origins, const float* dirs, int n,
                          const rt_ray_options* opt, float* results, uint32_t* steps);
int rt_terrain_trace_rays_device(rt_compute cs, const void* rays_device, int n,
                                 const rt_ray_options* opt, void* results_device, void* steps_device);

enum { RT_SURFACE_PARAMS = 8, RT_SURFACE_RAY_RANGE = 16 };
typedef struct {
    uint32_t size;
    uint32_t flags;
    float eye[3];
    uint32_t max_blocks;
    float t_min, t_max, stepmod;
    uint32_t max_steps;
} rt_surface_options;
int rt_terrain_trace_surface(rt_compute cs, const float* origins, const float* dirs, const float* ranges, int n,
                             const rt_surface_options* opt, float* results, uint32_t* steps);
int rt_terrain_trace_surface_device(rt_compute cs, const void* rays_device, int n,
                                    const rt_surface_options* opt, void* results_device, void* steps_device);

int rt_terrain_shade_rays(rt_compute screen_cs, const float* origins, const float* dirs, const float* ranges, int n,
                          const rt_surface_options* opt, float* results, uint32_t* rgba8, uint32_t* steps);
int rt_terrain_shade_rays_device(rt_compute screen_cs, const void* rays_device, int n, const rt_surface_options* opt,
                                 void* results_device, void* rgba8_device, void* steps_device);

typedef struct {
    uint32_t size;
    uint32_t flags;
    float eye[3];
    uint32_t max_blocks;
    uint32_t ao_samples;
    uint32_t seed;
} rt_point_options;
int rt_terrain_shade_points(rt_compute screen_cs, const float* points, const float* normals, int n,
                            const rt_point_options* opt, float* results, uint32_t* rgba8, uint32_t* steps);
int rt_terrain_shade_points_device(rt_compute screen_cs, const void* points_device, const void* normals_device, int n,
                                   const rt_point_options* opt, void* results_device, void* rgba8_device,
                                   void* steps_device);

enum { RT_FIELD_NORMAL = 32 };
typedef struct {
    uint32_t size;
    uint32_t flags;
    float eye[3];
    uint32_t max_blocks;
} rt_field_options;
typedef struct {
    float origin[3];
    float spacing[3];
    uint32_t dims[3];
} rt_lattice;
int rt_terrain_sample_field(rt_compute cs, const float* points, int n, const rt_field_options* opt, float* results);
int rt_terrain_sample_field_device(rt_compute cs, const void* points_device, int n, const rt_field_options* opt,
                                   void* results_device);
int rt_terrain_sample_lattice(rt_compute cs, const rt_lattice* lat, const rt_field_options* opt, float* results,
                              uint32_t* occupancy);
int rt_terrain_sample_lattice_device(rt_compute cs, const rt_lattice* lat, const rt_field_options* opt,
                                     void* results_device, void* occupancy_device);

size_t rt_terrain_mesh_scratch_bytes(const rt_lattice* lat);
int rt_terrain_extract_mesh(rt_compute cs, const rt_lattice* lat, const rt_field_options* opt, float* vertices,
                            float* normals, uint32_t max_vertices, uint32_t* triangles, uint32_t max_triangles,
                            uint32_t counts[2]);
int rt_terrain_extract_mesh_device(rt_compute cs, const rt_lattice* lat, const rt_field_options* opt,
                                   void* scratch_device, size_t scratch_bytes, void* vertices_device,
                                   void* normals_device, uint32_t max_vertices, void* triangles_device,
                                   uint32_t max_triangles, void* counts_device);

#define RT_DIST_FAR 0xFFFFFFFFu
typedef struct { uint32_t size, flags; float eye[3]; uint32_t max_blocks; uint32_t max_cells; } rt_distance_options;
size_t rt_terrain_distance_scratch_bytes(const rt_lattice* lat);
int rt_terrain_distance_field(rt_compute cs, const rt_lattice* lat, const rt_distance_options* opt,
                              const uint32_t* occupancy_in, uint32_t* d2, float* distance);
int rt_terrain_distance_field_device(rt_compute cs, const rt_lattice* lat, const rt_distance_options* opt,
                                     const void* occupancy_in_device, void* scratch_device, size_t scratch_bytes,
                                     void* d2_device, void* distance_device);

int rt_debug_math(rt_device dev, int op, const float* a, const float* b, float* out, int n);
int rt_debug_sky_ceiling(const float* np_rcp, int n_oct, float expo, const float* grad, int n_grad, double* ceiling);
int rt_debug_noise(rt_compute cs, const float* xyz, float* out, int n, int density);
int rt_debug_sky(rt_compute cs, const float* dirs, float* out, int n);
int rt_debug_spin(void* hip_stream, const unsigned long long* base_device, unsigned long long until_ticks,
                  unsigned long long ticks, unsigned long long* stamp_device);
int rt_debug_defer_slot(rt_device dev, int slot, void** fb8, void** camera_results, void** cell_distance);

int rt_recorder_create(rt_device dev, int frame_rate, int fixed_speed, const char* path, rt_recorder* out);
int rt_recorder_start(rt_recorder rec);
int rt_recorder_stop(rt_recorder rec);
int rt_recorder_is_recording(rt_recorder rec);
int rt_recorder_set_frame_time(rt_recorder rec, float seconds);
int rt_recorder_write(rt_recorder rec, const void* frame, int stride);
int rt_recorder_info(rt_recorder rec, unsigned long long* frames, unsigned long long* next_sample_time,
                     unsigned long long* frame_duration);
void rt_recorder_destroy(rt_recorder rec);
int rt_recorder_set_async(rt_recorder rec, int depth);

int rt_varmgr_start(int port, const char* bind_address);
int rt_varmgr_stop(void);
int rt_varmgr_count(void);
int rt_varmgr_register_compute(rt_compute cs);

#ifdef __cplusplus
}
#endif
#endif
```

Baseline: 1603.

## Pack trace kernel args into kernarg struct, precompute frame-index reciprocal, specialise fit1 shadow path

Moves most k_trace parameters into a TraceLaunch struct read on demand from the kernarg segment, so values are reloaded from scalar memory instead of held live in registers across the persistent loop. Replaces the integer division by frame_samples with a host-computed multiply-high and shift, and turns refill/compaction/batch thresholds into compile-time constants. Adds a do_shadow specialisation for fit mode with one AO sample that skips the AO-slot bookkeeping. It also adds a debug entry point to check the reciprocal on the host. Repeated kernarg loads add scalar-memory traffic, and the reciprocal falls back to division when it cannot be exact.

```diff
diff --git a/gpgpuraytrace_amd/_native.py b/gpgpuraytrace_amd/_native.py
--- a/gpgpuraytrace_amd/_native.py
+++ b/gpgpuraytrace_amd/_native.py
@@ -195,6 +195,7 @@
     "rt_debug_math": (_i, [_vp, _i, _vp, _vp, _vp, _i]),
     "rt_debug_sky_ceiling": (_i, [_vp, _i, C.c_float, _vp, _i, C.POINTER(C.c_double)]),
     "rt_debug_noise": (_i, [_vp, _vp, _vp, _i, _i]),
+    "rt_debug_frame_index": (_i, [_u, _u, _vp, _vp, _i, C.POINTER(_u), C.POINTER(_u)]),
     "rt_debug_sky": (_i, [_vp, _vp, _vp, _i]),
 }
 
diff --git a/gpgpuraytrace_amd/csrc/rt_kernels.hip b/gpgpuraytrace_amd/csrc/rt_kernels.hip
--- a/gpgpuraytrace_amd/csrc/rt_kernels.hip
+++ b/gpgpuraytrace_amd/csrc/rt_kernels.hip
@@ -249,6 +249,7 @@
 struct UnitMap {
     uint32_t off_x, off_y, ext_x, ext_y, tiles32_x, tile_first, tile_stride, n_units;
     uint32_t n_frames, frame_samples;
+    uint32_t frame_mul, frame_shift;
     uint32_t frame_rot;
     uint32_t order_batch;
     uint32_t cells_from_cam;
@@ -531,7 +532,7 @@
 
 __device__ __forceinline__ uint32_t frame_of(const UnitMap& m, uint32_t t)
 {
-    return m.n_frames == 1u ? 0u : t / m.frame_samples;
+    return m.frame_mul ? __umulhi(t, m.frame_mul) >> m.frame_shift : t / m.frame_samples;
 }
 
 template <class Body>
@@ -586,7 +587,7 @@
         h.fog = make_float4(0.0f, 0.0f, 0.0f, 0.0f);
     }
     uint32_t px, py, a;
-    sample_pixel(m, m.frame_rot ? (t - tl) / m.frame_samples : 0u, tl, aa, W, H, &px, &py, &a);
+    sample_pixel(m, m.frame_rot ? frame_of(m, t) : 0u, tl, aa, W, H, &px, &py, &a);
     h.px = px;
     h.py = py;
     h.a = a;
@@ -704,13 +705,13 @@
 __device__ __forceinline__ void long_finish(const RtConsts* k, const UnitMap& m, const FrameRays& fr,
                                             const float4* __restrict__ fin, const float4* __restrict__ finp,
                                             float4* __restrict__ samples, uint32_t* __restrict__ aocc, uint32_t t,
-                                            uint32_t aux, const March<L, true>& st)
+                                            uint32_t aux, const March<L, true>& st, int ao_samples)
 {
     if (aux_ao(aux)) {
         if (st.d > 0.0f) {
             if (aux == kAuxAO) {
                 if (m.fit) reinterpret_cast<uint8_t*>(aocc)[late(t)] = (uint8_t)(kFinFlag | 1u);
-                else if (k->ao_samples == 1) reinterpret_cast<uint8_t*>(aocc)[late(t)] = 1u;
+                else if (ao_samples == 1) reinterpret_cast<uint8_t*>(aocc)[late(t)] = 1u;
                 else if (!(RT_DIAG_SKIP & 8)) ao_count(aocc, t);
             } else if (!(RT_DIAG_SKIP & 2)) {
                 fit_store(k, m, fr, t, aux | 0xff000000u);
@@ -730,7 +731,7 @@
             f1 = ld_rec(finp, FR * aux + FR - 1u);
         }
         const float4 v = shade_finish(k, f0, fog, f1, st.d, st.f.w);
-        if (m.fit && k->ao_samples == 0) {
+        if (m.fit && ao_samples == 0) {
             if (!(RT_DIAG_SKIP & 2)) fit_store(k, m, fr, t, fit_pixel(v, 1.0f));
         } else if (!(RT_DIAG_SKIP & 4)) {
             sample_store(k, samples, t, v);
@@ -758,6 +759,52 @@
     uint32_t done, pad;
 };
 
+__device__ __forceinline__ uint32_t ring_slot(uint32_t base, uint32_t i)
+{
+    const uint32_t s = (uint32_t)__builtin_amdgcn_readfirstlane((int)base) % kLongRing + i;
+    return s >= kLongRing ? s - kLongRing : s;
+}
+
+struct TraceLaunch {
+    UnitMap m;
+    float4 *samples, *fin, *finpool, *cpool, *hitq, *spill_long;
+    uint32_t* aocc;
+    uint32_t hit_cap, long_spill_cap;
+    uint32_t long_ring_cap, fin_slots;
+    uint32_t fit1;
+};
+typedef const __attribute__((address_space(4))) TraceLaunch* LPtr;
+__device__ __forceinline__ LPtr trace_launch()
+{
+    LPtr p = (LPtr)__builtin_amdgcn_kernarg_segment_ptr();
+    asm volatile("" : "+s"(p));
+    return p;
+}
+static_assert(sizeof(UnitMap) == 18u * sizeof(uint32_t), "trace_map copies every field of UnitMap");
+__device__ __forceinline__ UnitMap trace_map(LPtr p)
+{
+    UnitMap m;
+    m.off_x = p->m.off_x;
+    m.off_y = p->m.off_y;
+    m.ext_x = p->m.ext_x;
+    m.ext_y = p->m.ext_y;
+    m.tiles32_x = p->m.tiles32_x;
+    m.tile_first = p->m.tile_first;
+    m.tile_stride = p->m.tile_stride;
+    m.n_units = p->m.n_units;
+    m.n_frames = p->m.n_frames;
+    m.frame_samples = p->m.frame_samples;
+    m.frame_mul = p->m.frame_mul;
+    m.frame_shift = p->m.frame_shift;
+    m.frame_rot = p->m.frame_rot;
+    m.order_batch = p->m.order_batch;
+    m.cells_from_cam = p->m.cells_from_cam;
+    m.fit = p->m.fit;
+    m.fitm = p->m.fitm;
+    m.packed = p->m.packed;
+    return m;
+}
+
 struct TraceQueues {
     uint32_t lock;
     uint32_t h_top, pad0;
@@ -812,19 +859,13 @@
               "a first-unit counter per wave slot inside the zeroed work counters");
 
 template <int L, bool STATS, bool GATED = false>
-__global__ void __launch_bounds__(TraceThreads<L>::value) k_trace(const RtConsts* __restrict__ k, const FrameTable* __restrict__ ft,
+__global__ void __launch_bounds__(TraceThreads<L>::value) k_trace(TraceLaunch launch_block,
+                                                const RtConsts* __restrict__ k, const FrameTable* __restrict__ ft,
                                                 const uint32_t* __restrict__ perm2d,
                                                 const float4* __restrict__ grad,
-                                                UnitMap m, const uint32_t* __restrict__ order,
-                                                uint64_t* __restrict__ hitmask, float4* __restrict__ samples,
-                                                float4* __restrict__ fin, float4* __restrict__ finpool,
-                                                float4* __restrict__ cpool,
-                                                float4* __restrict__ hitq,
-                                                float4* __restrict__ spill_long, uint32_t hit_cap,
-                                                uint32_t long_spill_cap,
-                                                uint32_t* __restrict__ aocc, uint32_t* __restrict__ counters,
-                                                RtStats* stats, uint32_t long_batch, uint32_t refill_idle,
-                                                uint32_t compact_live, uint32_t long_ring_cap, uint32_t fin_slots,
+                                                const uint32_t* __restrict__ order,
+                                                uint64_t* __restrict__ hitmask, uint32_t* __restrict__ counters,
+                                                RtStats* stats,
                                                 FusedPrepass np, GatedPrepass gp)
 {
     __shared__ __attribute__((aligned(16))) uint32_t
@@ -833,7 +874,7 @@
     TraceQueues& q = *reinterpret_cast<TraceQueues*>(lds + kNoiseLdsWords + sizeof(FrameRays) / 4);
     BlockStats& s_st =
         *reinterpret_cast<BlockStats*>(lds + kNoiseLdsWords + (sizeof(FrameRays) + sizeof(TraceQueues)) / 4);
-    frame_rays_load(s_fr, ft, m.n_frames);
+    frame_rays_load(s_fr, ft, trace_launch()->m.n_frames);
     if (threadIdx.x == 0) {
         q.lock = 0;
         q.h_top = 0;
@@ -841,13 +882,13 @@
         q.active = 0;
         q.drained = 0;
         q.ls_top = 0;
-        q.f_top = fin_slots;
+        q.f_top = trace_launch()->fin_slots;
         q.overflow = 0;
         q.gscan = q.gate_all = q.gate_cells = 0;
         q.near_end = 0;
         if constexpr (STATS) s_st = BlockStats{};
     }
-    for (uint32_t i = threadIdx.x; i < fin_slots; i += blockDim.x) q.fin_free[i] = (uint16_t)i;
+    for (uint32_t i = threadIdx.x, n = trace_launch()->fin_slots; i < n; i += blockDim.x) q.fin_free[i] = (uint16_t)i;
     for (uint32_t i = threadIdx.x; i < kAoSlots; i += blockDim.x) {
         q.ao_free[i] = (uint8_t)i;
         if (i < kAoSlots / 2u) q.ao_ctr[i] = 0u;
@@ -860,12 +901,12 @@
     const uint32_t W = (uint32_t)k->width, H = (uint32_t)k->height, aa = (uint32_t)k->aa_samples;
     const int max_steps = k->max_steps;
     constexpr bool kSky = RT_SKY_EXIT && L == RT_NOMADPLAINS && (!STATS || RT_SKY_EXIT_STATS);
-    const uint32_t n_total = (uint32_t)__builtin_amdgcn_readfirstlane(m.n_units * m.n_frames);
+    const uint32_t n_total = trace_launch()->m.n_units * trace_launch()->m.n_frames;
     constexpr uint32_t HR = HitRec<L>::N;
-    float4* const hq = hitq + (size_t)blockIdx.x * hit_cap * HR;
-    float4* const finp = finpool + (size_t)blockIdx.x * kFinSlots * FinRec<L>::N;
-    float4* const cpl = cpool + (size_t)blockIdx.x * RT_AO_POOL_SLOTS;
-    float4* const lspill = spill_long + (size_t)blockIdx.x * long_spill_cap * kShadowRec;
+    auto hq_of = [](LPtr p) { return p->hitq + (size_t)(blockIdx.x * p->hit_cap * HR); };
+    auto finp_of = [](LPtr p) { return p->finpool + (size_t)blockIdx.x * kFinSlots * FinRec<L>::N; };
+    auto cpl_of = [](LPtr p) { return p->cpool + (size_t)blockIdx.x * RT_AO_POOL_SLOTS; };
+    auto lspill_of = [](LPtr p) { return p->spill_long + (size_t)(blockIdx.x * p->long_spill_cap * kShadowRec); };
     auto queued_long = [&]() { return vload(q.l_tail) - vload(q.l_head) + vload(q.ls_top); };
     auto queued_hits = [&]() { return vload(q.h_top); };
     auto stat = [&](int i, uint32_t v) {
@@ -880,13 +921,14 @@
         const uint32_t n = (uint32_t)__popcll(lb), rank = lane_rank(lb);
         q_lock(&q.lock, lane);
         const uint32_t lh = vload(q.l_head), lt = vload(q.l_tail);
-        if (lt - lh + n <= long_ring_cap) {
-            if (want) pack(&q.longs[((lt + rank) % kLongRing) * kShadowRec]);
+        if (lt - lh + n <= trace_launch()->long_ring_cap) {
+            if (want) pack(&q.longs[ring_slot(lt, rank) * kShadowRec]);
             if (lane == 0) q.l_tail = lt + n;
         } else {
+            const LPtr lp = trace_launch();
             const uint32_t stl = (uint32_t)__builtin_amdgcn_readfirstlane(vload(q.ls_top));
-            const bool fits = stl + n <= long_spill_cap;
-            if (want && fits) pack(lspill + (size_t)(stl + rank) * kShadowRec);
+            const bool fits = stl + n <= lp->long_spill_cap;
+            if (want && fits) pack(lspill_of(lp) + (size_t)(stl + rank) * kShadowRec);
             __builtin_amdgcn_s_waitcnt(0);
             if (lane == 0) {
                 q.ls_top = fits ? stl + n : stl;
@@ -899,7 +941,7 @@
         push_recs(want, [&](float4* r) { long_pack(st, t, aux, r); });
     };
 
-    auto free_fin_locked = [&](bool live, uint32_t& aux) {
+    auto free_fin_locked = [&](bool live, uint32_t& aux, auto fit1) {
         const bool pend = !live && aux < kFinSlots;
         const uint64_t pb = __ballot(pend);
         if (pb) {
@@ -910,7 +952,7 @@
             }
             if (lane == 0) q.f_top = top + (uint32_t)__popcll(pb);
         }
-        if constexpr (kAoSlots > 0u) {
+        if constexpr (kAoSlots > 0u && !decltype(fit1)::value) {
             const bool pa = !live && aux_slot_free(aux);
             const uint64_t ab = __ballot(pa);
             if (ab) {
@@ -924,17 +966,19 @@
         }
     };
     auto ao_slot_finish = [&](const March<L, true>& st, uint32_t t, uint32_t& aux) {
+        const LPtr lp = trace_launch();
+        const uint32_t fitm = lp->m.fitm;
         const uint32_t sl = aux & 255u, sh = (sl & 1u) * 16u;
         const uint32_t occ1 = st.d > 0.0f ? 1u : 0u;
         const uint32_t old = atomicAdd(&q.ao_ctr[sl >> 1], (1u | (occ1 << 5)) << sh) >> sh;
         if ((old & 31u) + 1u == (uint32_t)k->ao_samples) {
             const uint32_t occ = ((old >> 5) & 31u) + occ1;
-            if (m.fitm && !(old & (1u << 10))) {
-                const float4 v = ld_rec(cpl, sl);
+            if (fitm && !(old & (1u << 10))) {
+                const float4 v = ld_rec(cpl_of(lp), sl);
                 const uint32_t at = __float_as_uint(v.w);
                 if (!(RT_DIAG_SKIP & 2)) gptr(s_fr.out8[at >> 23])[at & 0x7fffffu] = fit_pixel(v, ao_factor(occ, k->ao_samples));
             } else if (occ != 0u) {
-                reinterpret_cast<uint8_t*>(aocc)[late(t)] = (uint8_t)((m.fitm ? kFinFlag : 0u) | occ);
+                reinterpret_cast<uint8_t*>(lp->aocc)[late(t)] = (uint8_t)((fitm ? kFinFlag : 0u) | occ);
             }
             atomicAnd(&q.ao_ctr[sl >> 1], ~(0xffffu << sh));
             aux = kAuxSlotFree | sl;
@@ -943,7 +987,20 @@
         }
     };
 
-    auto do_shadow = [&]() {
+    auto long_finish_at = [&](uint32_t t, uint32_t aux, const March<L, true>& st, auto fit1) {
+        const LPtr lp = trace_launch();
+        UnitMap m = trace_map(lp);
+        if constexpr (decltype(fit1)::value) {
+            m.fit = 1u;
+            m.fitm = 0u;
+        }
+        long_finish<L>(k, m, s_fr, lp->fin, finp_of(lp), lp->samples, lp->aocc, t, aux, st,
+                       decltype(fit1)::value ? 1 : k->ao_samples);
+    };
+    auto ray_frame = [&](uint32_t t) -> const float* { return s_fr.v[frame_of(trace_map(trace_launch()), t)]; };
+
+    auto do_shadow = [&](auto fit1) {
+        constexpr bool F1 = decltype(fit1)::value;
         March<L, true> st;
         st.d = 0.0f;
         st.iters = 0;
@@ -955,15 +1012,15 @@
             if (live && !march_live<L, true, true>(cl, st, aux_ao(aux) ? RT_AO_END : 100.0f, 0)) {
                 WT(wl_rays++; wl_maxit = max(wl_maxit, (uint32_t)st.iters);)
                 stat(aux_ao(aux) ? BlockStats::AO : BlockStats::SHADOW, (uint32_t)st.iters);
-                if (kAoSlots > 0u && aux_ao_slot(aux)) ao_slot_finish(st, t, aux);
-                else long_finish<L>(k, m, s_fr, fin, finp, samples, aocc, t, aux, st);
+                if (!F1 && kAoSlots > 0u && aux_ao_slot(aux)) ao_slot_finish(st, t, aux);
+                else long_finish_at(t, aux, st, fit1);
                 live = false;
             }
             const uint64_t idle = __ballot(!live);
             const uint32_t nidle = (uint32_t)__popcll(idle);
-            if (nidle >= refill_idle && queued_long() != 0u) {
+            if (nidle >= kRefillIdle && queued_long() != 0u) {
                 q_lock(&q.lock, lane);
-                free_fin_locked(live, aux);
+                free_fin_locked(live, aux, fit1);
                 const uint32_t head = vload(q.l_head), tail = vload(q.l_tail);
                 const uint32_t take = (tail - head) < nidle ? (tail - head) : nidle;
                 const uint32_t sl = vload(q.ls_top);
@@ -972,16 +1029,17 @@
                 const bool mine = ((idle >> lane) & 1ull) && rank < take + more;
                 auto take_ray = [&](float4 r0, float4 r1, float4 r2) {
                     t = long_unpack(r0, r1, r2, rtm::mk(0.0f, 0.0f, 0.0f), st, &aux);
-                    const float* fr = s_fr.v[frame_of(m, t)];
+                    const float* fr = ray_frame(t);
                     cl.eye = rtm::mk(fr[0], fr[1], fr[2]);
                     if (!aux_ao(aux)) st.dir = rtm::mk(fr[3], fr[4], fr[5]);
                     live = true;
                 };
                 if (mine && rank < take) {
-                    const float4* r = &q.longs[((head + rank) % kLongRing) * kShadowRec];
+                    const float4* r = &q.longs[ring_slot(head, rank) * kShadowRec];
                     take_ray(r[0], r[1], r[2]);
                 } else if (mine) {
                     const uint32_t ri = (sl - more + rank - take) * kShadowRec;
+                    const float4* lspill = lspill_of(trace_launch());
                     take_ray(ld_rec(lspill, ri), ld_rec(lspill, ri + 1u), ld_rec(lspill, ri + 2u));
                 }
                 if (more) __builtin_amdgcn_s_waitcnt(0);
@@ -993,14 +1051,14 @@
             }
             const uint64_t lv = __ballot(live);
             const bool drained_now = vload(q.drained) != 0u;
-            bool hand_back = lv != 0ull && (uint32_t)__popcll(lv) < compact_live && queued_long() == 0u && !drained_now;
+            bool hand_back = lv != 0ull && (uint32_t)__popcll(lv) < kCompactLive && queued_long() == 0u && !drained_now;
             if constexpr (L == RT_NOMADPLAINS && kSegLanes > 0u)
                 hand_back = hand_back || (drained_now && lv != 0ull && (uint32_t)__popcll(lv) <= kSegHandBack &&
                                           queued_long() == 0u);
             if (lv == 0ull || hand_back) {
-                if (__ballot(!live && (aux < kFinSlots || aux_slot_free(aux)))) {
+                if (__ballot(!live && (aux < kFinSlots || (!F1 && aux_slot_free(aux))))) {
                     q_lock(&q.lock, lane);
-                    free_fin_locked(live, aux);
+                    free_fin_locked(live, aux, fit1);
                     q_unlock(&q.lock, lane);
                 }
                 if (hand_back) push_long(live, st, t, aux);
@@ -1035,18 +1093,19 @@
             if (const uint32_t grp = late(lane) / LPR; grp < take + more) {
                 float4 r0, r1, r2;
                 if (grp < take) {
-                    const float4* r = &q.longs[((head + grp) % kLongRing) * kShadowRec];
+                    const float4* r = &q.longs[ring_slot(head, grp) * kShadowRec];
                     r0 = r[0];
                     r1 = r[1];
                     r2 = r[2];
                 } else {
                     const uint32_t ri = (sl - more + grp - take) * kShadowRec;
+                    const float4* lspill = lspill_of(trace_launch());
                     r0 = ld_rec(lspill, ri);
                     r1 = ld_rec(lspill, ri + 1u);
                     r2 = ld_rec(lspill, ri + 2u);
                 }
                 t = long_unpack(r0, r1, r2, rtm::mk(0.0f, 0.0f, 0.0f), st, &aux);
-                const float* fr = s_fr.v[frame_of(m, t)];
+                const float* fr = ray_frame(t);
                 cl.eye = rtm::mk(fr[0], fr[1], fr[2]);
                 if (!aux_ao(aux)) st.dir = rtm::mk(fr[3], fr[4], fr[5]);
                 live = true;
@@ -1065,7 +1124,7 @@
                     if (j == 0u) {
                         stat(aux_ao(aux) ? BlockStats::AO : BlockStats::SHADOW, (uint32_t)st.iters);
                         if (kAoSlots > 0u && aux_ao_slot(aux)) ao_slot_finish(st, t, aux);
-                        else long_finish<L>(k, m, s_fr, fin, finp, samples, aocc, t, aux, st);
+                        else long_finish_at(t, aux, st, std::false_type{});
                     }
                     live = false;
                 }
@@ -1088,7 +1147,7 @@
             uint32_t fa = j == 0u ? aux : kAuxAO;
             if (__ballot(fa < kFinSlots || aux_slot_free(fa))) {
                 q_lock(&q.lock, lane);
-                free_fin_locked(false, fa);
+                free_fin_locked(false, fa, std::false_type{});
                 q_unlock(&q.lock, lane);
             }
         }
@@ -1160,6 +1219,14 @@
     };
 
     auto do_shade = [&]() {
+        const LPtr lp = trace_launch();
+        const UnitMap m = trace_map(lp);
+        float4* const hq = hq_of(lp);
+        float4* const finp = finp_of(lp);
+        float4* const cpl = cpl_of(lp);
+        float4* const fin = lp->fin;
+        float4* const samples = lp->samples;
+        uint32_t* const aocc = lp->aocc;
         q_lock(&q.lock, lane);
         const uint32_t top = vload(q.h_top);
         const uint32_t take = top < 64u ? top : 64u;
@@ -1333,6 +1400,7 @@
         return __hip_atomic_load((gcuint*)p, __ATOMIC_RELAXED, __HIP_MEMORY_SCOPE_AGENT);
     };
     auto tile_ready = [&](uint32_t e, uint32_t w0, uint32_t w1, uint32_t w2, uint32_t w3) -> bool {
+        const UnitMap m = trace_map(trace_launch());
         const uint32_t f = e >> 24, first = m.frame_rot ? (m.tile_first + f) % m.tile_stride : m.tile_first;
         const uint32_t T = (e & 0xffffffu) * m.tile_stride + first;
         const uint32_t gx = (T % m.tiles32_x) * 32u, gy = (T / m.tiles32_x) * 32u;
@@ -1357,7 +1425,7 @@
         const uint32_t nt = n_total >> 4;
         bool gate_all = vload(q.gate_all) != 0u;
         if (!gate_all) {
-            const uint32_t gw = lane < m.n_frames ? ld_u32(gp.gate, late(lane * RT_GATE_WORDS + RT_GATE_CTR))
+            const uint32_t gw = lane < trace_launch()->m.n_frames ? ld_u32(gp.gate, late(lane * RT_GATE_WORDS + RT_GATE_CTR))
                                                   : (uint32_t)(RT_CAMERA_RES * RT_CAMERA_RES);
             gate_all = __ballot(gw < (uint32_t)(RT_CAMERA_RES * RT_CAMERA_RES)) == 0ull;
             if (gate_all && lane == 0) q.gate_all = 1u;
@@ -1425,6 +1493,9 @@
     };
 
     auto do_unit = [&](uint32_t f, uint32_t u) {
+        const LPtr lp = trace_launch();
+        const UnitMap m = trace_map(lp);
+        float4* const samples = lp->samples;
         bool cells_in = true;
         if constexpr (GATED) {
             cells_in = (vload(q.gate_cells) >> f) & 1u;
@@ -1525,8 +1596,9 @@
                 if (hit) stat(BlockStats::HITS, 1u);
                 q_lock(&q.lock, lane);
                 const uint32_t top = vload(q.h_top);
-                const bool fits = (uint32_t)__builtin_amdgcn_readfirstlane(top) + n <= hit_cap;
-                if (hit && fits) hit_store<L>(hq + (size_t)(top + rank) * HR, t, rr);
+                const LPtr lq = trace_launch();
+                const bool fits = (uint32_t)__builtin_amdgcn_readfirstlane(top) + n <= lq->hit_cap;
+                if (hit && fits) hit_store<L>(hq_of(lq) + (size_t)(top + rank) * HR, t, rr);
                 __builtin_amdgcn_s_waitcnt(0);
                 if (lane == 0) {
                     if (fits) q.h_top = top + n;
@@ -1546,7 +1618,7 @@
     if constexpr (GATED) {
         if (gp.debug & 1u) {
             float acc = 0.0f;
-            for (uint32_t f = 0; f < m.n_frames; ++f)
+            for (uint32_t f = 0; f < trace_launch()->m.n_frames; ++f)
                 for (uint32_t i = lane; i < RT_CAMERA_RES * RT_CAMERA_RES; i += 64u) acc += ft->cells[f][i].x;
             asm volatile("" : : "v"(acc));
         }
@@ -1578,7 +1650,7 @@
         const bool drained = vload(q.drained) != 0u;
         WT(const unsigned long long t0 = __builtin_amdgcn_s_memrealtime(); wt[12]++;
            wt[15] = t0; if (drained && wt[18] == 0) { wt[18] = t0; wt[19] = lp; wt[20] = hp; })
-        const uint32_t lb_now = (RT_NEAR_UNITS > 0 && vload(q.near_end) != 0u) ? (uint32_t)RT_NEAR_LONG_BATCH : long_batch;
+        const uint32_t lb_now = (RT_NEAR_UNITS > 0 && vload(q.near_end) != 0u) ? (uint32_t)RT_NEAR_LONG_BATCH : kLongBatch;
         if (lp >= lb_now || (drained && lp > 0u)) {
             if constexpr (L == RT_NOMADPLAINS && kSegLanes > 0u) {
                 if (drained && lp <= kSegQueue) {
@@ -1588,7 +1660,8 @@
                     continue;
                 }
             }
-            do_shadow();
+            if (trace_launch()->fit1) do_shadow(std::true_type{});
+            else do_shadow(std::false_type{});
             WT(const unsigned long long dl = __builtin_amdgcn_s_memrealtime() - t0; wt[4] += dl; wt[7]++; wt[27] += dl;)
             continue;
         }
@@ -1836,6 +1909,9 @@
     m.frame_rot = rot;
     m.n_frames = a.n_frames;
     m.frame_samples = m.n_units * 64u * (uint32_t)a.aa;
+    const RtFrameRcp rcp = rt_frame_rcp(m.frame_samples, m.n_frames);
+    m.frame_mul = rcp.mul;
+    m.frame_shift = rcp.shift;
     uint32_t blocks = (uint32_t)(a.num_cus > 0 ? a.num_cus : 256);
     uint32_t need = (m.n_units * m.n_frames + 15u) / 16u;
     uint32_t pblocks = need < blocks ? need : blocks;
@@ -1857,11 +1933,22 @@
         const RtConsts* k0 = a.frames_host.k[0];
         constexpr bool kCanGate = L == RT_NOMADPLAINS && !S;
         auto* kern = (kCanGate && a.gated.tasks) ? k_trace<L, S, kCanGate> : k_trace<L, S, false>;
-        hipLaunchKernelGGL(kern, dim3(pblocks), dim3(TraceThreads<L>::value), 0, a.stream, k0, a.frames,
-                           a.perm2d, a.grad, m,
-                           a.order, a.hitmask, a.samples, a.fin, a.finpool, a.cpool, a.hitq, a.spill_long, a.hit_cap,
-                           a.long_spill_cap, a.aocc, a.queue, a.stats, kLongBatch, kRefillIdle, kCompactLive,
-                           a.small_rings ? 64u : kLongRing, a.small_rings ? 8u : kFinSlots, a.fuse_next, a.gated);
+        TraceLaunch tl;
+        tl.m = m;
+        tl.samples = a.samples;
+        tl.fin = a.fin;
+        tl.finpool = a.finpool;
+        tl.cpool = a.cpool;
+        tl.hitq = a.hitq;
+        tl.spill_long = a.spill_long;
+        tl.aocc = a.aocc;
+        tl.hit_cap = a.hit_cap;
+        tl.long_spill_cap = a.long_spill_cap;
+        tl.long_ring_cap = a.small_rings ? 64u : kLongRing;
+        tl.fin_slots = a.small_rings ? 8u : kFinSlots;
+        tl.fit1 = m.fit && a.ao_samples == 1 ? 1u : 0u;
+        hipLaunchKernelGGL(kern, dim3(pblocks), dim3(TraceThreads<L>::value), 0, a.stream, tl, k0, a.frames,
+                           a.perm2d, a.grad, a.order, a.hitmask, a.queue, a.stats, a.fuse_next, a.gated);
         if (!(m.fit && a.ao_samples == 0))
             hipLaunchKernelGGL(k_finish, dim3(fblocks), blk, 0, a.stream, k0, a.frames, m, a.hitmask, a.samples, a.aocc);
     };
diff --git a/gpgpuraytrace_amd/csrc/rt_runtime.cpp b/gpgpuraytrace_amd/csrc/rt_runtime.cpp
--- a/gpgpuraytrace_amd/csrc/rt_runtime.cpp
+++ b/gpgpuraytrace_amd/csrc/rt_runtime.cpp
@@ -2454,6 +2454,18 @@
     return sky_ceiling(np_rcp, n_oct, expo, grad, n_grad, ceiling);
 }
 
+extern "C" int rt_debug_frame_index(unsigned frame_samples, unsigned n_frames, const unsigned* t, unsigned* frame, int n,
+                                    unsigned* mul, unsigned* shift)
+{
+    if (frame_samples == 0u || n_frames == 0u || n < 0 || (n > 0 && (!t || !frame)))
+        return fail(RT_ERR_INVALID, "bad arguments");
+    const RtFrameRcp r = rt_frame_rcp(frame_samples, n_frames);
+    if (mul) *mul = r.mul;
+    if (shift) *shift = r.shift;
+    for (int i = 0; i < n; ++i) frame[i] = rt_frame_index_host(r, frame_samples, t[i]);
+    return r.mul ? 1 : 0;
+}
+
 extern "C" int rt_debug_math(rt_device d, int op, const float* a, const float* b, float* y, int n)
 {
     if (!d || !a || !y || n <= 0) return fail(RT_ERR_INVALID, "bad arguments");
diff --git a/gpgpuraytrace_amd/csrc/rt_types.h b/gpgpuraytrace_amd/csrc/rt_types.h
--- a/gpgpuraytrace_amd/csrc/rt_types.h
+++ b/gpgpuraytrace_amd/csrc/rt_types.h
@@ -41,6 +41,32 @@
     int32_t pad[2];
 };
 
+struct RtFrameRcp {
+    uint32_t mul, shift;
+};
+static inline RtFrameRcp rt_frame_rcp(uint32_t frame_samples, uint32_t n_frames)
+{
+    const RtFrameRcp none = {0u, 0u};
+    const uint64_t total = (uint64_t)frame_samples * n_frames;
+    if (frame_samples < 2u || n_frames == 0u || total > (1ull << 32)) return none;
+    uint32_t s = 31u;
+    while (!((frame_samples >> s) & 1u)) --s;
+    if ((frame_samples & (frame_samples - 1u)) == 0u) {
+        const RtFrameRcp p2 = {1u << 31, s - 1u};
+        return p2;
+    }
+    const uint64_t two_k = 1ull << (32u + s);
+    const uint64_t mul = two_k / frame_samples + 1u;
+    const uint64_t e = mul * frame_samples - two_k;
+    if (mul >> 32 || (total - 1u) * e >= two_k) return none;
+    const RtFrameRcp r = {(uint32_t)mul, s};
+    return r;
+}
+static inline uint32_t rt_frame_index_host(RtFrameRcp r, uint32_t frame_samples, uint32_t t)
+{
+    return r.mul ? (uint32_t)(((uint64_t)t * r.mul) >> 32) >> r.shift : t / frame_samples;
+}
+
 struct RtStats {
     unsigned long long primary_steps;
     unsigned long long shadow_steps;
diff --git a/include/frosttrace.h b/include/frosttrace.h
--- a/include/frosttrace.h
+++ b/include/frosttrace.h
@@ -231,6 +231,8 @@
 int rt_debug_math(rt_device dev, int op, const float* a, const float* b, float* out, int n);
 int rt_debug_sky_ceiling(const float* np_rcp, int n_oct, float expo, const float* grad, int n_grad, double* ceiling);
 int rt_debug_noise(rt_compute cs, const float* xyz, float* out, int n, int density);
+int rt_debug_frame_index(unsigned frame_samples, unsigned n_frames, const unsigned* t, unsigned* frame, int n,
+                         unsigned* mul, unsigned* shift);
 int rt_debug_sky(rt_compute cs, const float* dirs, float* out, int n);
 int rt_debug_spin(void* hip_stream, const unsigned long long* base_device, unsigned long long until_ticks,
                   unsigned long long ticks, unsigned long long* stamp_device);
```

Measured after the change: 1614, median of 6. Within noise of the previous version (+0.7%).
